# algbio/SBWT

Measured on AMD Instinct MI355X. Metric: k-mers/sec (whole node), plain-matrix k=30 streaming search, higher is better.
Workload: dtype u64

## Files before the change

### include/sbwtgpu.h

```cpp
#ifndef SBWTGPU_H
#define SBWTGPU_H

#include <stdint.h>
#include <stddef.h>

#ifdef __cplusplus
extern "C" {
#endif

#define SBWTGPU_OK                      0
#define SBWTGPU_ERR_INVALID_ARG        -1
#define SBWTGPU_ERR_NO_DEVICE          -2
#define SBWTGPU_ERR_HIP                -3
#define SBWTGPU_ERR_NO_STREAMING       -4
#define SBWTGPU_ERR_PRECALC_TOO_LONG   -5
#define SBWTGPU_ERR_PRECALC_GT_K       -6
#define SBWTGPU_ERR_NOT_SINGLETON      -7
#define SBWTGPU_ERR_OOM                -8
#define SBWTGPU_ERR_READ_TOO_LONG      -9
#define SBWTGPU_ERR_STALLED           -10

typedef struct sbwtgpu_index sbwtgpu_index;

typedef struct {
    int64_t         n_nodes;
    const uint64_t *A_bits;
    const uint64_t *C_bits;
    const uint64_t *G_bits;
    const uint64_t *T_bits;
    const uint64_t *suffix_group_starts;
    int64_t         k;
    int64_t         n_kmers;
    int64_t         precalc_k;
    const int64_t  *precalc;
} sbwtgpu_index_desc;

typedef struct {
    int64_t n_nodes, n_kmers, k, precalc_k;
    int64_t C[4];
    int32_t has_streaming_support;
    int32_t device;
    int64_t device_precalc_k;
    int64_t blob_bytes;
    int64_t image_level;
    int64_t n_paths;
    int64_t n_branch;
    int64_t default_search_variant;
} sbwtgpu_index_info;

const char *sbwtgpu_version(void);
const char *sbwtgpu_last_error(void);
int         sbwtgpu_device_count(int *count);
int         sbwtgpu_set_tuning(const char *key, int64_t value);

int  sbwtgpu_index_create(const sbwtgpu_index_desc *desc, int device, sbwtgpu_index **out);
void sbwtgpu_index_destroy(sbwtgpu_index *idx);
int  sbwtgpu_index_get_info(const sbwtgpu_index *idx, sbwtgpu_index_info *info);
int  sbwtgpu_index_get_precalc(const sbwtgpu_index *idx, int64_t *out_pairs);

typedef struct {
    int64_t   n_nodes, n_kmers, k;
    uint64_t *A_bits, *C_bits, *G_bits, *T_bits;
    uint64_t *suffix_group_starts;
} sbwtgpu_plain_matrix_bits;
int  sbwtgpu_build_plain_matrix(const char *const *seqs, const int64_t *seq_len, int64_t n_seqs, int64_t k,
                                int add_revcomp, int build_streaming_support, int device,
                                sbwtgpu_plain_matrix_bits *out);
void sbwtgpu_free_plain_matrix(sbwtgpu_plain_matrix_bits *bits);

int  sbwtgpu_index_export_header(const sbwtgpu_index *idx, void *header_out, int64_t header_cap,
                                 int64_t *header_bytes);
int  sbwtgpu_index_blob(const sbwtgpu_index *idx, void **dev_ptr, int64_t *bytes);
int  sbwtgpu_index_copy_blob(const sbwtgpu_index *idx, void *dst_dev, int64_t bytes, void *stream);
int  sbwtgpu_index_adopt(const void *header, int64_t header_bytes, void *dev_blob, int64_t blob_bytes,
                         int device, sbwtgpu_index **out);
int  sbwtgpu_index_bcast(sbwtgpu_index *root, int n_dev, const int *devs, sbwtgpu_index **out);

int  sbwtgpu_rank_batch(const sbwtgpu_index *idx, const int64_t *pos, const char *sym, int64_t n,
                        int64_t *out);
int  sbwtgpu_streaming_search_batch(const sbwtgpu_index *idx, const char *bases, const int64_t *read_off,
                                    int64_t n_reads, int64_t *out, const int64_t *out_off);
int  sbwtgpu_search_batch(const sbwtgpu_index *idx, const char *bases, const int64_t *read_off,
                          int64_t n_reads, int64_t *out, const int64_t *out_off);
int  sbwtgpu_streaming_search_batch_i32(const sbwtgpu_index *idx, const char *bases, const int64_t *read_off,
                                        int64_t n_reads, int32_t *out, const int64_t *out_off);
int  sbwtgpu_search_batch_i32(const sbwtgpu_index *idx, const char *bases, const int64_t *read_off,
                              int64_t n_reads, int32_t *out, const int64_t *out_off);
int  sbwtgpu_update_interval_batch(const sbwtgpu_index *idx, const char *bases, const int64_t *off,
                                   int64_t n, int64_t *first, int64_t *second);
int  sbwtgpu_forward_batch(const sbwtgpu_index *idx, const int64_t *node, const char *sym, int64_t n,
                           int64_t *out);
int  sbwtgpu_partial_search_batch(const sbwtgpu_index *idx, const char *bases, const int64_t *off, int64_t n,
                                  int64_t *first, int64_t *second, int64_t *matched);
int  sbwtgpu_get_kmer_batch(const sbwtgpu_index *idx, const int64_t *colex_rank, int64_t n, char *out);
int  sbwtgpu_select_batch(const sbwtgpu_index *idx, const int64_t *j, const char *sym, int64_t n, int64_t *out);

int64_t sbwtgpu_search_workspace_bytes(int64_t total_bases);
int  sbwtgpu_streaming_search_dev(const sbwtgpu_index *idx, const char *d_bases, int64_t total_bases,
                                  const int64_t *d_read_off, int64_t n_reads, int64_t *d_out,
                                  const int64_t *d_out_off, void *d_workspace, int64_t workspace_bytes,
                                  void *stream);
int  sbwtgpu_search_dev(const sbwtgpu_index *idx, const char *d_bases, int64_t total_bases,
                        const int64_t *d_read_off, int64_t n_reads, int64_t *d_out,
                        const int64_t *d_out_off, void *d_workspace, int64_t workspace_bytes,
                        void *stream);
int  sbwtgpu_streaming_search_dev_i32(const sbwtgpu_index *idx, const char *d_bases, int64_t total_bases,
                                      const int64_t *d_read_off, int64_t n_reads, int32_t *d_out,
                                      const int64_t *d_out_off, void *d_workspace, int64_t workspace_bytes,
                                      void *stream);
int  sbwtgpu_search_dev_i32(const sbwtgpu_index *idx, const char *d_bases, int64_t total_bases,
                            const int64_t *d_read_off, int64_t n_reads, int32_t *d_out,
                            const int64_t *d_out_off, void *d_workspace, int64_t workspace_bytes,
                            void *stream);
int  sbwtgpu_rank_dev(const sbwtgpu_index *idx, const int64_t *d_pos, const char *d_sym, int64_t n,
                      int64_t *d_out, void *stream);
int  sbwtgpu_encode_bases_dev(const sbwtgpu_index *idx, const char *d_bases, int64_t total_bases,
                              void *d_workspace, int64_t workspace_bytes, void *stream);
int  sbwtgpu_search_encoded_dev(const sbwtgpu_index *idx, int64_t total_bases, const int64_t *d_read_off,
                                int64_t n_reads, int64_t *d_out, const int64_t *d_out_off,
                                void *d_workspace, int64_t workspace_bytes, int streaming, void *stream);
int  sbwtgpu_workspace_status(const void *d_workspace, void *stream, int *status);
int  sbwtgpu_workspace_stats(const void *d_workspace, void *stream, int64_t stats[8]);
int  sbwtgpu_kernel_times(double *ms, int64_t cap, int64_t *n);

int64_t sbwtgpu_format_text_bound(const sbwtgpu_index *idx, int64_t n_values, int64_t n_reads);
int64_t sbwtgpu_format_scratch_bytes(int64_t n_reads);
int  sbwtgpu_format_results_dev(const sbwtgpu_index *idx, const int64_t *d_values, const int64_t *d_out_off,
                                int64_t n_reads, int64_t n_values, char *d_text, int64_t text_cap,
                                int64_t *d_line_off, void *d_scratch, int64_t scratch_bytes, void *stream);
int  sbwtgpu_search_text_batch(const sbwtgpu_index *idx, const char *bases, const int64_t *read_off,
                               int64_t n_reads, int streaming, char **text, int64_t *text_bytes,
                               int64_t *n_queries);
typedef int (*sbwtgpu_text_sink)(void *ctx, const char *text, int64_t bytes);
int  sbwtgpu_search_text_stream(const sbwtgpu_index *idx, const char *bases, const int64_t *read_off,
                                int64_t n_reads, int streaming, sbwtgpu_text_sink sink, void *sink_ctx,
                                int64_t *n_queries);
void sbwtgpu_free_host(void *p);
void sbwtgpu_release_cached_buffers(void);

int  sbwtgpu_index_build_lcs(sbwtgpu_index *idx);
int  sbwtgpu_index_get_lcs(const sbwtgpu_index *idx, uint8_t *out);
int  sbwtgpu_matching_statistics_batch(const sbwtgpu_index *idx, const char *bases, const int64_t *read_off,
                                       int64_t n_reads, uint8_t *len, int64_t *first, int64_t *second);
int64_t sbwtgpu_ms_workspace_bytes(int64_t total_bases);
int  sbwtgpu_matching_statistics_dev(const sbwtgpu_index *idx, const char *d_bases, int64_t total_bases,
                                     const int64_t *d_read_off, int64_t n_reads, uint8_t *d_len, int64_t *d_first,
                                     int64_t *d_second, void *d_workspace, int64_t workspace_bytes, void *stream);
int  sbwtgpu_ms_workspace_stats(const void *d_workspace, void *stream, int64_t stats[5]);

typedef struct sbwtgpu_unitigs sbwtgpu_unitigs;
int  sbwtgpu_unitigs_create(const sbwtgpu_index *idx, sbwtgpu_unitigs **out);
int  sbwtgpu_unitigs_info(const sbwtgpu_unitigs *u, int64_t *n_unitigs, int64_t *total_bases, int64_t *n_kmers);
int  sbwtgpu_unitigs_dev(const sbwtgpu_unitigs *u, const char **d_bases, const int64_t **d_off ,
                         const int64_t **d_first_col );
int  sbwtgpu_unitigs_copy(const sbwtgpu_unitigs *u, char *bases, int64_t *off, int64_t *first_col );
int  sbwtgpu_unitigs_stats(const sbwtgpu_unitigs *u, double pass_ms[6], int64_t *jump_rounds);
void sbwtgpu_unitigs_destroy(sbwtgpu_unitigs *u);

#define SBWTGPU_SETOP_UNION 0
#define SBWTGPU_SETOP_INTERSECTION 1
#define SBWTGPU_SETOP_DIFFERENCE 2
#define SBWTGPU_SETOP_SYMMETRIC_DIFFERENCE 3
typedef struct {
    int64_t n_a, n_b, n_both, n_either;
    int64_t n_result, n_nopred;
    double  pass_ms[4];
} sbwtgpu_setop_info;
int  sbwtgpu_index_setop(const sbwtgpu_index *a, const sbwtgpu_index *b, int op, int build_streaming_support,
                         sbwtgpu_plain_matrix_bits *out, sbwtgpu_setop_info *info );
int  sbwtgpu_index_setop_counts(const sbwtgpu_index *a, const sbwtgpu_index *b, sbwtgpu_setop_info *info);
int  sbwtgpu_index_kmer_keys(const sbwtgpu_index *idx, void *out_keys, int64_t cap_bytes, int64_t *n_keys, int *key_bytes);

typedef struct { int32_t n_kmers, n_found, covered_bases, longest_run; } sbwtgpu_read_hits;
int     sbwtgpu_read_hits_batch(const sbwtgpu_index *idx, const char *bases, const int64_t *read_off, int64_t n_reads,
                                int strands, sbwtgpu_read_hits *out);
int64_t sbwtgpu_read_hits_workspace_bytes(int64_t total_bases, int64_t n_reads, int strands);
int     sbwtgpu_read_hits_dev(const sbwtgpu_index *idx, const char *d_bases, int64_t total_bases, const int64_t *d_read_off,
                              int64_t n_reads, int strands, sbwtgpu_read_hits *d_out, void *d_workspace,
                              int64_t workspace_bytes, void *stream);

#ifdef __cplusplus
}
#endif
#endif
```

### sbwt_amd/capi.py

```python
from __future__ import annotations

import ctypes as C
import os
from typing import Optional, Sequence

import numpy as np

_HERE = os.path.dirname(os.path.abspath(__file__))
LIB_PATH = os.environ.get("SBWTGPU_LIB", os.path.join(_HERE, "lib", "libsbwtgpu.so"))

OK = 0
ERR_INVALID_ARG = -1
ERR_NO_DEVICE = -2
ERR_HIP = -3
ERR_NO_STREAMING = -4
ERR_PRECALC_TOO_LONG = -5
ERR_PRECALC_GT_K = -6
ERR_NOT_SINGLETON = -7
ERR_OOM = -8
ERR_READ_TOO_LONG = -9
ERR_STALLED = -10

EXPORTED_SYMBOLS = [
    "sbwtgpu_version", "sbwtgpu_last_error", "sbwtgpu_device_count", "sbwtgpu_set_tuning",
    "sbwtgpu_index_create", "sbwtgpu_index_destroy", "sbwtgpu_index_get_info", "sbwtgpu_index_get_precalc",
    "sbwtgpu_index_export_header", "sbwtgpu_index_blob", "sbwtgpu_index_copy_blob", "sbwtgpu_index_adopt", "sbwtgpu_index_bcast",
    "sbwtgpu_rank_batch", "sbwtgpu_streaming_search_batch", "sbwtgpu_search_batch",
    "sbwtgpu_streaming_search_batch_i32", "sbwtgpu_search_batch_i32",
    "sbwtgpu_update_interval_batch", "sbwtgpu_forward_batch",
    "sbwtgpu_build_plain_matrix", "sbwtgpu_free_plain_matrix",
    "sbwtgpu_partial_search_batch", "sbwtgpu_get_kmer_batch", "sbwtgpu_select_batch",
    "sbwtgpu_search_workspace_bytes", "sbwtgpu_streaming_search_dev", "sbwtgpu_search_dev",
    "sbwtgpu_streaming_search_dev_i32", "sbwtgpu_search_dev_i32",
    "sbwtgpu_rank_dev", "sbwtgpu_encode_bases_dev", "sbwtgpu_search_encoded_dev",
    "sbwtgpu_workspace_status", "sbwtgpu_workspace_stats", "sbwtgpu_kernel_times",
    "sbwtgpu_format_text_bound", "sbwtgpu_format_scratch_bytes", "sbwtgpu_format_results_dev",
    "sbwtgpu_search_text_batch", "sbwtgpu_search_text_stream", "sbwtgpu_free_host", "sbwtgpu_release_cached_buffers",
    "sbwtgpu_index_build_lcs", "sbwtgpu_index_get_lcs", "sbwtgpu_matching_statistics_batch", "sbwtgpu_ms_workspace_bytes",
    "sbwtgpu_matching_statistics_dev", "sbwtgpu_ms_workspace_stats",
    "sbwtgpu_unitigs_create", "sbwtgpu_unitigs_info", "sbwtgpu_unitigs_dev", "sbwtgpu_unitigs_copy", "sbwtgpu_unitigs_stats",
    "sbwtgpu_unitigs_destroy",
    "sbwtgpu_index_setop", "sbwtgpu_index_setop_counts", "sbwtgpu_index_kmer_keys",
    "sbwtgpu_read_hits_batch", "sbwtgpu_read_hits_workspace_bytes", "sbwtgpu_read_hits_dev",
]

SETOP_UNION, SETOP_INTERSECTION, SETOP_DIFFERENCE, SETOP_SYMMETRIC_DIFFERENCE = 0, 1, 2, 3
SETOPS = {"union": SETOP_UNION, "intersection": SETOP_INTERSECTION, "difference": SETOP_DIFFERENCE,
          "symmetric-difference": SETOP_SYMMETRIC_DIFFERENCE}


class SbwtGpuError(RuntimeError):
    def __init__(self, code: int, msg: str):
        super().__init__(f"sbwtgpu error {code}: {msg}")
        self.code = code
        self.msg = msg


class IndexDesc(C.Structure):
    _fields_ = [
        ("n_nodes", C.c_int64),
        ("A_bits", C.c_void_p), ("C_bits", C.c_void_p), ("G_bits", C.c_void_p), ("T_bits", C.c_void_p),
        ("suffix_group_starts", C.c_void_p),
        ("k", C.c_int64), ("n_kmers", C.c_int64), ("precalc_k", C.c_int64),
        ("precalc", C.c_void_p),
    ]


class IndexInfo(C.Structure):
    _fields_ = [
        ("n_nodes", C.c_int64), ("n_kmers", C.c_int64), ("k", C.c_int64), ("precalc_k", C.c_int64),
        ("C", C.c_int64 * 4),
        ("has_streaming_support", C.c_int32), ("device", C.c_int32),
        ("device_precalc_k", C.c_int64), ("blob_bytes", C.c_int64), ("image_level", C.c_int64),
        ("n_paths", C.c_int64), ("n_branch", C.c_int64), ("default_search_variant", C.c_int64),
    ]


class ImageHeader(C.Structure):
    _fields_ = [
        ("magic", C.c_uint64),
        ("n_nodes", C.c_int64), ("n_kmers", C.c_int64), ("k", C.c_int64), ("p_file", C.c_int64), ("p_dev", C.c_int64),
        ("C", C.c_int64 * 4),
        ("n_blocks", C.c_int64), ("n_mega", C.c_int64),
        ("off_blocks", C.c_int64), ("off_ptab", C.c_int64), ("off_ftab", C.c_int64), ("off_mega", C.c_int64),
        ("blob_bytes", C.c_int64),
        ("has_ssup", C.c_int32), ("rank_only", C.c_int32), ("ssup_derived", C.c_int32), ("p_sparse", C.c_int32),
        ("off_stab", C.c_int64),
        ("big_layout", C.c_int32), ("has_path", C.c_int32),
        ("off_col", C.c_int64), ("off_pos", C.c_int64), ("off_pq", C.c_int64), ("off_trans", C.c_int64),
        ("stab_pos", C.c_int32), ("p_filter", C.c_int32),
        ("off_pfil", C.c_int64),
        ("log2f", C.c_int32), ("has_safe", C.c_int32), ("force_mega", C.c_int32),
        ("n_tslots", C.c_int64), ("n_sb", C.c_int64), ("n_pos", C.c_int64), ("n_trans", C.c_int64),
        ("n_paths", C.c_int64), ("n_branch", C.c_int64), ("image_level", C.c_int64),
        ("row_ones", C.c_int64 * 4),
        ("log2b2_unused", C.c_int32),
        ("n_sb2", C.c_int64), ("off_stab2", C.c_int64), ("path_lookahead", C.c_int64),
    ]


class PlainMatrixBitsC(C.Structure):
    _fields_ = [("n_nodes", C.c_int64), ("n_kmers", C.c_int64), ("k", C.c_int64),
                ("A_bits", C.c_void_p), ("C_bits", C.c_void_p), ("G_bits", C.c_void_p), ("T_bits", C.c_void_p),
                ("suffix_group_starts", C.c_void_p)]


class SetopInfoC(C.Structure):
    _fields_ = [("n_a", C.c_int64), ("n_b", C.c_int64), ("n_both", C.c_int64), ("n_either", C.c_int64),
                ("n_result", C.c_int64), ("n_nopred", C.c_int64), ("pass_ms", C.c_double * 4)]

    def as_dict(self) -> dict:
        d = {f: int(getattr(self, f)) for f in ("n_a", "n_b", "n_both", "n_either", "n_result", "n_nopred")}
        d["pass_ms"] = dict(zip(("keys_a", "keys_b", "merge_select", "tail_columns"), (float(x) for x in self.pass_ms)))
        return d


_lib: Optional[C.CDLL] = None


def lib() -> C.CDLL:
    global _lib
    if _lib is not None:
        return _lib
    if not os.path.exists(LIB_PATH):
        raise ImportError(f"{LIB_PATH} is missing: build it with `python -m sbwt_amd.build` "
                          "(there is no CPU fallback for the GPU search path)")
    L = C.CDLL(LIB_PATH, mode=C.RTLD_GLOBAL)
    vp, i64, ci = C.c_void_p, C.c_int64, C.c_int
    L.sbwtgpu_version.restype = C.c_char_p
    L.sbwtgpu_last_error.restype = C.c_char_p
    L.sbwtgpu_device_count.argtypes = [C.POINTER(ci)]
    L.sbwtgpu_set_tuning.argtypes = [C.c_char_p, i64]
    L.sbwtgpu_index_create.argtypes = [C.POINTER(IndexDesc), ci, C.POINTER(vp)]
    L.sbwtgpu_index_destroy.argtypes = [vp]
    L.sbwtgpu_index_destroy.restype = None
    L.sbwtgpu_index_get_info.argtypes = [vp, C.POINTER(IndexInfo)]
    L.sbwtgpu_index_get_precalc.argtypes = [vp, vp]
    L.sbwtgpu_index_export_header.argtypes = [vp, vp, i64, C.POINTER(i64)]
    L.sbwtgpu_index_blob.argtypes = [vp, C.POINTER(vp), C.POINTER(i64)]
    L.sbwtgpu_index_copy_blob.argtypes = [vp, vp, i64, vp]
    L.sbwtgpu_index_adopt.argtypes = [vp, i64, vp, i64, ci, C.POINTER(vp)]
    L.sbwtgpu_index_bcast.argtypes = [vp, ci, C.POINTER(ci), C.POINTER(vp)]
    L.sbwtgpu_rank_batch.argtypes = [vp, vp, vp, i64, vp]
    L.sbwtgpu_streaming_search_batch.argtypes = [vp, vp, vp, i64, vp, vp]
    L.sbwtgpu_search_batch.argtypes = [vp, vp, vp, i64, vp, vp]
    try:
        L.sbwtgpu_streaming_search_batch_i32.argtypes = [vp, vp, vp, i64, vp, vp]
        L.sbwtgpu_search_batch_i32.argtypes = [vp, vp, vp, i64, vp, vp]
    except AttributeError:
        if "SBWTGPU_LIB" not in os.environ:
            raise
    L.sbwtgpu_update_interval_batch.argtypes = [vp, vp, vp, i64, vp, vp]
    L.sbwtgpu_forward_batch.argtypes = [vp, vp, vp, i64, vp]
    L.sbwtgpu_build_plain_matrix.argtypes = [C.POINTER(C.c_char_p), vp, i64, i64, ci, ci, ci, C.POINTER(PlainMatrixBitsC)]
    L.sbwtgpu_free_plain_matrix.argtypes = [C.POINTER(PlainMatrixBitsC)]
    L.sbwtgpu_free_plain_matrix.restype = None
    L.sbwtgpu_partial_search_batch.argtypes = [vp, vp, vp, i64, vp, vp, vp]
    L.sbwtgpu_get_kmer_batch.argtypes = [vp, vp, i64, vp]
    L.sbwtgpu_select_batch.argtypes = [vp, vp, vp, i64, vp]
    L.sbwtgpu_search_workspace_bytes.argtypes = [i64]
    L.sbwtgpu_search_workspace_bytes.restype = i64
    L.sbwtgpu_streaming_search_dev.argtypes = [vp, vp, i64, vp, i64, vp, vp, vp, i64, vp]
    L.sbwtgpu_search_dev.argtypes = [vp, vp, i64, vp, i64, vp, vp, vp, i64, vp]
    try:
        L.sbwtgpu_streaming_search_dev_i32.argtypes = [vp, vp, i64, vp, i64, vp, vp, vp, i64, vp]
        L.sbwtgpu_search_dev_i32.argtypes = [vp, vp, i64, vp, i64, vp, vp, vp, i64, vp]
    except AttributeError:
        if not os.environ.get("SBWTGPU_LIB"):
            raise
    L.sbwtgpu_rank_dev.argtypes = [vp, vp, vp, i64, vp, vp]
    L.sbwtgpu_workspace_status.argtypes = [vp, vp, C.POINTER(ci)]
    L.sbwtgpu_encode_bases_dev.argtypes = [vp, vp, i64, vp, i64, vp]
    L.sbwtgpu_search_encoded_dev.argtypes = [vp, i64, vp, i64, vp, vp, vp, i64, ci, vp]
    L.sbwtgpu_workspace_stats.argtypes = [vp, vp, C.POINTER(i64)]
    L.sbwtgpu_kernel_times.argtypes = [vp, i64, C.POINTER(i64)]
    L.sbwtgpu_format_text_bound.argtypes = [vp, i64, i64]
    L.sbwtgpu_format_text_bound.restype = i64
    L.sbwtgpu_format_scratch_bytes.argtypes = [i64]
    L.sbwtgpu_format_scratch_bytes.restype = i64
    L.sbwtgpu_format_results_dev.argtypes = [vp, vp, vp, i64, i64, vp, i64, vp, vp, i64, vp]
    L.sbwtgpu_search_text_batch.argtypes = [vp, vp, vp, i64, ci, C.POINTER(vp), C.POINTER(i64), C.POINTER(i64)]
    L.sbwtgpu_free_host.argtypes = [vp]
    L.sbwtgpu_free_host.restype = None
    L.sbwtgpu_release_cached_buffers.restype = None
    try:
        L.sbwtgpu_index_build_lcs.argtypes = [vp]
        L.sbwtgpu_index_get_lcs.argtypes = [vp, vp]
        L.sbwtgpu_matching_statistics_batch.argtypes = [vp, vp, vp, i64, vp, vp, vp]
        L.sbwtgpu_ms_workspace_bytes.argtypes = [i64]
        L.sbwtgpu_ms_workspace_bytes.restype = i64
        L.sbwtgpu_matching_statistics_dev.argtypes = [vp, vp, i64, vp, i64, vp, vp, vp, vp, i64, vp]
        L.sbwtgpu_ms_workspace_stats.argtypes = [vp, vp, C.POINTER(i64)]
        L.sbwtgpu_unitigs_create.argtypes = [vp, C.POINTER(vp)]
        L.sbwtgpu_unitigs_info.argtypes = [vp, C.POINTER(i64), C.POINTER(i64), C.POINTER(i64)]
        L.sbwtgpu_unitigs_dev.argtypes = [vp, C.POINTER(vp), C.POINTER(vp), C.POINTER(vp)]
        L.sbwtgpu_unitigs_copy.argtypes = [vp, vp, vp, vp]
        L.sbwtgpu_unitigs_stats.argtypes = [vp, C.POINTER(C.c_double), C.POINTER(i64)]
        L.sbwtgpu_unitigs_destroy.argtypes = [vp]
        L.sbwtgpu_unitigs_destroy.restype = None
        L.sbwtgpu_index_setop.argtypes = [vp, vp, ci, ci, C.POINTER(PlainMatrixBitsC), C.POINTER(SetopInfoC)]
        L.sbwtgpu_index_setop_counts.argtypes = [vp, vp, C.POINTER(SetopInfoC)]
        L.sbwtgpu_index_kmer_keys.argtypes = [vp, vp, i64, C.POINTER(i64), C.POINTER(ci)]
        L.sbwtgpu_read_hits_batch.argtypes = [vp, vp, vp, i64, ci, vp]
        L.sbwtgpu_read_hits_workspace_bytes.argtypes = [i64, i64, ci]
        L.sbwtgpu_read_hits_workspace_bytes.restype = i64
        L.sbwtgpu_read_hits_dev.argtypes = [vp, vp, i64, vp, i64, ci, vp, vp, i64, vp]
    except AttributeError:
        if not os.environ.get("SBWTGPU_LIB"):
            raise
    _lib = L
    return L


def _check(rc: int) -> None:
    if rc != OK:
        raise SbwtGpuError(rc, lib().sbwtgpu_last_error().decode(errors="replace"))


def set_tuning(key: str, value: int) -> None:
    _check(lib().sbwtgpu_set_tuning(key.encode(), value))


def device_count() -> int:
    n = C.c_int(0)
    rc = lib().sbwtgpu_device_count(C.byref(n))
    return n.value if rc == OK else 0


def _words(a) -> np.ndarray:
    a = np.ascontiguousarray(a, dtype=np.uint64)
    return a


def concat_reads(reads: Sequence[bytes]):
    lens = np.fromiter((len(r) for r in reads), dtype=np.int64, count=len(reads))
    off = np.zeros(len(reads) + 1, dtype=np.int64)
    np.cumsum(lens, out=off[1:])
    bases = np.frombuffer(b"".join(reads), dtype=np.uint8).copy() if len(reads) else np.zeros(0, np.uint8)
    return bases, off


def out_offsets(read_off: np.ndarray, k: int) -> np.ndarray:
    lens = np.diff(read_off)
    m = np.maximum(lens - k + 1, 0)
    off = np.zeros(len(read_off), dtype=np.int64)
    np.cumsum(m, out=off[1:])
    return off


class BuiltBits:

    def __init__(self, cols, ssup, n_nodes, n_kmers, k):
        self.cols, self.ssup, self.n_nodes, self.n_kmers, self.k = cols, ssup, n_nodes, n_kmers, k


def _take_bits(out: PlainMatrixBitsC) -> BuiltBits:
    try:
        nw = (out.n_nodes + 63) // 64

        def words(p):
            return np.ctypeslib.as_array(C.cast(p, C.POINTER(C.c_uint64)), shape=(nw,)).copy()
        cols = [words(out.A_bits), words(out.C_bits), words(out.G_bits), words(out.T_bits)]
        ssup = words(out.suffix_group_starts) if out.suffix_group_starts else None
        return BuiltBits(cols, ssup, out.n_nodes, out.n_kmers, out.k)
    finally:
        lib().sbwtgpu_free_plain_matrix(C.byref(out))


def build_bits_gpu(seqs: Sequence[bytes], k: int, add_revcomp: bool = False, streaming_support: bool = True,
                   device: int = 0) -> BuiltBits:
    arr = (C.c_char_p * len(seqs))(*[bytes(s) for s in seqs])
    lens = np.array([len(s) for s in seqs], dtype=np.int64)
    out = PlainMatrixBitsC()
    _check(lib().sbwtgpu_build_plain_matrix(arr, lens.ctypes.data, len(seqs), k, int(add_revcomp), int(streaming_support),
                                            device, C.byref(out)))
    return _take_bits(out)


class Index:

    def __init__(self, handle: int, keepalive=None):
        self._h = C.c_void_p(handle)
        self._keep = keepalive
        info = IndexInfo()
        _check(lib().sbwtgpu_index_get_info(self._h, C.byref(info)))
        self.n_nodes, self.n_kmers, self.k = info.n_nodes, info.n_kmers, info.k
        self.precalc_k = info.precalc_k
        self.C = [info.C[i] for i in range(4)]
        self.has_streaming_support = bool(info.has_streaming_support)
        self.device = info.device
        self.device_precalc_k = info.device_precalc_k
        self.blob_bytes = info.blob_bytes
        self.image_level = info.image_level
        self.n_paths, self.n_branch, self.default_search_variant = info.n_paths, info.n_branch, info.default_search_variant

    @property
    def handle(self) -> C.c_void_p:
        return self._h

    @classmethod
    def create(cls, A, Cb, G, T, ssup, n_nodes: int, k: int, n_kmers: int = 0, precalc_k: int = 0,
               precalc=None, device: int = 0) -> "Index":
        A, Cb, G, T = _words(A), _words(Cb), _words(G), _words(T)
        s = _words(ssup) if ssup is not None else None
        pc = np.ascontiguousarray(precalc, dtype=np.int64) if precalc is not None else None
        d = IndexDesc(n_nodes, A.ctypes.data, Cb.ctypes.data, G.ctypes.data, T.ctypes.data,
                      s.ctypes.data if s is not None else None, k, n_kmers, precalc_k,
                      pc.ctypes.data if pc is not None else None)
        h = C.c_void_p()
        _check(lib().sbwtgpu_index_create(C.byref(d), device, C.byref(h)))
        return cls(h.value)

    @classmethod
    def adopt(cls, header: bytes, dev_ptr: int, blob_bytes: int, device: int, keepalive=None) -> "Index":
        h = C.c_void_p()
        buf = C.create_string_buffer(header, len(header))
        _check(lib().sbwtgpu_index_adopt(buf, len(header), C.c_void_p(dev_ptr), blob_bytes, device, C.byref(h)))
        return cls(h.value, keepalive=keepalive)

    def close(self) -> None:
        if self._h:
            lib().sbwtgpu_index_destroy(self._h)
            self._h = C.c_void_p()

    def __del__(self):
        try:
            self.close()
        except Exception:
            pass

    def export_header(self) -> bytes:
        n = C.c_int64(0)
        _check(lib().sbwtgpu_index_export_header(self._h, None, 0, C.byref(n)))
        buf = C.create_string_buffer(n.value)
        _check(lib().sbwtgpu_index_export_header(self._h, buf, n.value, C.byref(n)))
# ... 3 lines not shown
        raw = self.export_header()
        if len(raw) != C.sizeof(ImageHeader):
            raise SbwtGpuError(ERR_INVALID_ARG, "ImageHeader has %d bytes, the library's header %d" % (C.sizeof(ImageHeader), len(raw)))
        return ImageHeader.from_buffer_copy(raw)

    def blob(self):
        p, n = C.c_void_p(), C.c_int64(0)
        _check(lib().sbwtgpu_index_blob(self._h, C.byref(p), C.byref(n)))
        return p.value, n.value

    def blob_tensor(self):
        import torch
        ptr, n = self.blob()

        class _Alias:
            __cuda_array_interface__ = {"shape": (n,), "typestr": "|u1", "data": (ptr, False), "version": 3, "strides": None}
        t = torch.as_tensor(_Alias(), device=torch.device("cuda", self.device))
        t._sbwt_owner = self
        return t

    def copy_blob(self, dst_dev_ptr: int, nbytes: int, stream: int = 0) -> None:
        _check(lib().sbwtgpu_index_copy_blob(self._h, dst_dev_ptr, nbytes, stream))

    def get_precalc(self) -> np.ndarray:
        out = np.zeros((4 ** self.precalc_k if self.precalc_k else 0, 2), dtype=np.int64)
        if self.precalc_k:
            _check(lib().sbwtgpu_index_get_precalc(self._h, out.ctypes.data))
        return out

    def rank(self, pos, sym) -> np.ndarray:
        pos = np.ascontiguousarray(pos, dtype=np.int64)
        sym = np.ascontiguousarray(sym, dtype=np.uint8)
        out = np.empty(len(pos), dtype=np.int64)
        _check(lib().sbwtgpu_rank_batch(self._h, pos.ctypes.data, sym.ctypes.data, len(pos), out.ctypes.data))
        return out

    def _search(self, fn, bases, read_off, out_off=None):
        bases = np.ascontiguousarray(bases, dtype=np.uint8)
        read_off = np.ascontiguousarray(read_off, dtype=np.int64)
        if out_off is None:
            out_off = out_offsets(read_off, self.k)
        out_off = np.ascontiguousarray(out_off, dtype=np.int64)
        out = np.full(int(out_off[-1]) if len(out_off) else 0, -12345, dtype=np.int64)
        _check(fn(self._h, bases.ctypes.data, read_off.ctypes.data, len(read_off) - 1, out.ctypes.data,
                  out_off.ctypes.data))
        return out, out_off

    def streaming_search(self, bases, read_off, out_off=None):
        return self._search(lib().sbwtgpu_streaming_search_batch, bases, read_off, out_off)

    def search(self, bases, read_off, out_off=None):
        return self._search(lib().sbwtgpu_search_batch, bases, read_off, out_off)

    def search_i32(self, bases, read_off, streaming: bool = True, out_off=None):
        bases = np.ascontiguousarray(bases, dtype=np.uint8)
        read_off = np.ascontiguousarray(read_off, dtype=np.int64)
        if out_off is None:
            out_off = out_offsets(read_off, self.k)
        out_off = np.ascontiguousarray(out_off, dtype=np.int64)
        out = np.full(int(out_off[-1]) if len(out_off) else 0, -12345, dtype=np.int32)
        fn = lib().sbwtgpu_streaming_search_batch_i32 if streaming else lib().sbwtgpu_search_batch_i32
        _check(fn(self._h, bases.ctypes.data, read_off.ctypes.data, len(read_off) - 1, out.ctypes.data, out_off.ctypes.data))
        return out, out_off

    def streaming_search_reads(self, reads: Sequence[bytes]):
        bases, off = concat_reads(reads)
        out, oo = self.streaming_search(bases, off)
        return [out[oo[i]:oo[i + 1]] for i in range(len(reads))]

    def search_reads(self, reads: Sequence[bytes]):
        bases, off = concat_reads(reads)
        out, oo = self.search(bases, off)
        return [out[oo[i]:oo[i + 1]] for i in range(len(reads))]

    def search_text(self, bases, read_off, streaming: bool = True):
        bases = np.ascontiguousarray(bases, dtype=np.uint8)
        read_off = np.ascontiguousarray(read_off, dtype=np.int64)
        p, n, q = C.c_void_p(), C.c_int64(0), C.c_int64(0)
        _check(lib().sbwtgpu_search_text_batch(self._h, bases.ctypes.data, read_off.ctypes.data, len(read_off) - 1,
                                               int(streaming), C.byref(p), C.byref(n), C.byref(q)))
        try:
            return C.string_at(p.value, n.value), q.value
        finally:
            lib().sbwtgpu_free_host(p)

    def update_interval(self, bases, off, first, second):
        bases = np.ascontiguousarray(bases, dtype=np.uint8)
        off = np.ascontiguousarray(off, dtype=np.int64)
        first = np.array(first, dtype=np.int64)
        second = np.array(second, dtype=np.int64)
        _check(lib().sbwtgpu_update_interval_batch(self._h, bases.ctypes.data, off.ctypes.data, len(first),
                                                   first.ctypes.data, second.ctypes.data))
        return first, second

    def forward(self, node, sym) -> np.ndarray:
        node = np.ascontiguousarray(node, dtype=np.int64)
        sym = np.ascontiguousarray(sym, dtype=np.uint8)
        out = np.empty(len(node), dtype=np.int64)
        _check(lib().sbwtgpu_forward_batch(self._h, node.ctypes.data, sym.ctypes.data, len(node), out.ctypes.data))
        return out

    def partial_search(self, bases, off):
        bases = np.ascontiguousarray(bases, dtype=np.uint8)
        off = np.ascontiguousarray(off, dtype=np.int64)
        n = len(off) - 1
        first, second, matched = (np.empty(n, dtype=np.int64) for _ in range(3))
        _check(lib().sbwtgpu_partial_search_batch(self._h, bases.ctypes.data, off.ctypes.data, n, first.ctypes.data,
                                                  second.ctypes.data, matched.ctypes.data))
        return first, second, matched

    def get_kmers(self, colex_ranks) -> np.ndarray:
        cr = np.ascontiguousarray(colex_ranks, dtype=np.int64)
        out = np.empty((len(cr), self.k), dtype=np.uint8)
        _check(lib().sbwtgpu_get_kmer_batch(self._h, cr.ctypes.data, len(cr), out.ctypes.data))
        return out

    def select(self, j, sym) -> np.ndarray:
        j = np.ascontiguousarray(j, dtype=np.int64)
        sym = np.ascontiguousarray(sym, dtype=np.uint8)
        out = np.empty(len(j), dtype=np.int64)
        _check(lib().sbwtgpu_select_batch(self._h, j.ctypes.data, sym.ctypes.data, len(j), out.ctypes.data))
        return out

    def streaming_search_dev(self, d_bases: int, total_bases: int, d_read_off: int, n_reads: int, d_out: int,
                             d_out_off: int, d_ws: int, ws_bytes: int, stream: int = 0, streaming: bool = True):
        fn = lib().sbwtgpu_streaming_search_dev if streaming else lib().sbwtgpu_search_dev
        _check(fn(self._h, d_bases, total_bases, d_read_off, n_reads, d_out, d_out_off, d_ws, ws_bytes, stream))

    def streaming_search_dev_i32(self, d_bases: int, total_bases: int, d_read_off: int, n_reads: int, d_out32: int,
                                 d_out_off: int, d_ws: int, ws_bytes: int, stream: int = 0, streaming: bool = True):
        fn = lib().sbwtgpu_streaming_search_dev_i32 if streaming else lib().sbwtgpu_search_dev_i32
        _check(fn(self._h, d_bases, total_bases, d_read_off, n_reads, d_out32, d_out_off, d_ws, ws_bytes, stream))

    def encode_bases_dev(self, d_bases: int, total_bases: int, d_ws: int, ws_bytes: int, stream: int = 0):
        _check(lib().sbwtgpu_encode_bases_dev(self._h, d_bases, total_bases, d_ws, ws_bytes, stream))

    def search_encoded_dev(self, total_bases: int, d_read_off: int, n_reads: int, d_out: int, d_out_off: int,
                           d_ws: int, ws_bytes: int, streaming: bool = True, stream: int = 0):
        _check(lib().sbwtgpu_search_encoded_dev(self._h, total_bases, d_read_off, n_reads, d_out, d_out_off, d_ws,
                                                ws_bytes, int(streaming), stream))

    def workspace_stats(self, d_ws: int, stream: int = 0):
        st = (C.c_int64 * 8)()
        _check(lib().sbwtgpu_workspace_stats(d_ws, stream, st))
        return tuple(int(x) for x in st[:5])

    def workspace_bridges(self, d_ws: int, stream: int = 0) -> int:
        st = (C.c_int64 * 8)()
        _check(lib().sbwtgpu_workspace_stats(d_ws, stream, st))
        return int(st[5])

    def build_lcs(self) -> None:
        _check(lib().sbwtgpu_index_build_lcs(self._h))

    def lcs(self) -> np.ndarray:
        out = np.empty(self.n_nodes, dtype=np.uint8)
        _check(lib().sbwtgpu_index_get_lcs(self._h, out.ctypes.data))
        return out

    def matching_statistics(self, bases, read_off, intervals: bool = True):
        bases = np.ascontiguousarray(bases, dtype=np.uint8)
        read_off = np.ascontiguousarray(read_off, dtype=np.int64)
        n = int(read_off[-1]) if len(read_off) else 0
        ln = np.zeros(n, dtype=np.uint8)
        first = np.full(n, -12345, dtype=np.int64) if intervals else None
        second = np.full(n, -12345, dtype=np.int64) if intervals else None
        _check(lib().sbwtgpu_matching_statistics_batch(self._h, bases.ctypes.data, read_off.ctypes.data, max(len(read_off) - 1, 0),
                                                       ln.ctypes.data, first.ctypes.data if intervals else None,
                                                       second.ctypes.data if intervals else None))
        return (ln, first, second) if intervals else ln

    def matching_statistics_reads(self, reads: Sequence[bytes], intervals: bool = True):
        bases, off = concat_reads(reads)
        res = self.matching_statistics(bases, off, intervals)
        if not intervals:
            return [res[off[i]:off[i + 1]] for i in range(len(reads))]
        return [tuple(a[off[i]:off[i + 1]] for a in res) for i in range(len(reads))]

    def matching_statistics_dev(self, d_bases: int, total_bases: int, d_read_off: int, n_reads: int, d_len: int,
                                d_first: int, d_second: int, d_ws: int, ws_bytes: int, stream: int = 0):
        _check(lib().sbwtgpu_matching_statistics_dev(self._h, d_bases, total_bases, d_read_off, n_reads, d_len,
                                                     d_first or None, d_second or None, d_ws, ws_bytes, stream))

    def ms_workspace_stats(self, d_ws: int, stream: int = 0) -> dict:
        st = (C.c_int64 * 5)()
        _check(lib().sbwtgpu_ms_workspace_stats(d_ws, stream, st))
        return dict(zip(("positions", "walked", "full", "contractions", "recomputes"), (int(x) for x in st)))

    def unitigs_dev(self) -> "Unitigs":
        h = C.c_void_p()
        _check(lib().sbwtgpu_unitigs_create(self._h, C.byref(h)))
        return Unitigs(h)

    def unitigs(self):
        with self.unitigs_dev() as u:
            return u.copy()

    def setop(self, other: "Index", op, streaming_support: bool = True):
        out, info = PlainMatrixBitsC(), SetopInfoC()
        rc = lib().sbwtgpu_index_setop(self._h, other._h, SETOPS.get(op, op), int(streaming_support), C.byref(out), C.byref(info))
        if rc != OK:
            err = SbwtGpuError(rc, lib().sbwtgpu_last_error().decode(errors="replace"))
            err.info = info.as_dict()
            raise err
        return _take_bits(out), info.as_dict()

    def setop_counts(self, other: "Index") -> dict:
        info = SetopInfoC()
        _check(lib().sbwtgpu_index_setop_counts(self._h, other._h, C.byref(info)))
        d = info.as_dict()
        d["jaccard"] = d["n_both"] / d["n_either"] if d["n_either"] else 1.0
        d["containment"] = d["n_both"] / d["n_a"] if d["n_a"] else 1.0
        return d

    def kmer_keys(self) -> np.ndarray:
        n, kb = C.c_int64(0), C.c_int(0)
        cap = max(self.n_kmers, 0) * (8 if self.k <= 32 else 16)
        out = np.empty(cap // 8, dtype=np.uint64)
        rc = lib().sbwtgpu_index_kmer_keys(self._h, out.ctypes.data if cap else None, cap, C.byref(n), C.byref(kb))
        if rc in (OK, ERR_INVALID_ARG) and n.value * kb.value > cap:
            cap = n.value * kb.value
            out = np.empty(cap // 8, dtype=np.uint64)
            rc = lib().sbwtgpu_index_kmer_keys(self._h, out.ctypes.data, cap, C.byref(n), C.byref(kb))
        _check(rc)
        out = out[: n.value * kb.value // 8]
        return out if kb.value == 8 else out.reshape(n.value, 2)

    def read_hits(self, bases, read_off, both_strands: bool = False) -> np.ndarray:
        bases = np.ascontiguousarray(bases, dtype=np.uint8)
        read_off = np.ascontiguousarray(read_off, dtype=np.int64)
        n = max(len(read_off) - 1, 0)
        out = np.full((n, 4), -12345, dtype=np.int32)
        _check(lib().sbwtgpu_read_hits_batch(self._h, bases.ctypes.data, read_off.ctypes.data, n, 2 if both_strands else 1,
                                             out.ctypes.data))
        return out

    def read_hits_reads(self, reads: Sequence[bytes], both_strands: bool = False) -> np.ndarray:
        bases, off = concat_reads(reads)
        return self.read_hits(bases, off, both_strands)

    def read_hits_dev(self, d_bases: int, total_bases: int, d_read_off: int, n_reads: int, d_out: int, d_ws: int, ws_bytes: int,
                      both_strands: bool = False, stream: int = 0):
        _check(lib().sbwtgpu_read_hits_dev(self._h, d_bases, total_bases, d_read_off, n_reads, 2 if both_strands else 1, d_out,
                                           d_ws, ws_bytes, stream))

    def workspace_status(self, d_ws: int, stream: int = 0) -> int:
        st = C.c_int(0)
        _check(lib().sbwtgpu_workspace_status(d_ws, stream, C.byref(st)))
        return st.value


class Unitigs:

    def __init__(self, handle):
        self._h = handle
        n, total, nk = C.c_int64(0), C.c_int64(0), C.c_int64(0)
        _check(lib().sbwtgpu_unitigs_info(self._h, C.byref(n), C.byref(total), C.byref(nk)))
        self.n_unitigs, self.total_bases, self.n_kmers = n.value, total.value, nk.value

    def __enter__(self):
        return self

    def __exit__(self, *exc):
        self.close()

    def close(self) -> None:
        if self._h:
            lib().sbwtgpu_unitigs_destroy(self._h)
            self._h = None

    def __del__(self):
        try:
            self.close()
        except Exception:
            pass

    def dev_ptrs(self):
        b, o, f = C.c_void_p(), C.c_void_p(), C.c_void_p()
        _check(lib().sbwtgpu_unitigs_dev(self._h, C.byref(b), C.byref(o), C.byref(f)))
        return b.value or 0, o.value or 0, f.value or 0

    def copy(self):
        bases = np.empty(self.total_bases, dtype=np.uint8)
        off = np.empty(self.n_unitigs + 1, dtype=np.int64)
        first_col = np.empty(self.n_unitigs, dtype=np.int64)
        _check(lib().sbwtgpu_unitigs_copy(self._h, bases.ctypes.data, off.ctypes.data, first_col.ctypes.data))
        return bases, off, first_col

    def stats(self) -> dict:
        ms = (C.c_double * 6)()
        r = C.c_int64(0)
        _check(lib().sbwtgpu_unitigs_stats(self._h, ms, C.byref(r)))
        names = ("pred_marks", "real_flags", "internal_edges", "pointer_jumping", "ids_offsets", "bases")
        return {"pass_ms": dict(zip(names, (float(x) for x in ms))), "jump_rounds": int(r.value)}


def kernel_times() -> list:
    buf = (C.c_double * 256)()
    n = C.c_int64(0)
    _check(lib().sbwtgpu_kernel_times(buf, 256, C.byref(n)))
    return [float(buf[i]) for i in range(n.value)]


def search_workspace_bytes(total_bases: int) -> int:
    return int(lib().sbwtgpu_search_workspace_bytes(total_bases))


def ms_workspace_bytes(total_bases: int) -> int:
    return int(lib().sbwtgpu_ms_workspace_bytes(total_bases))


def read_hits_workspace_bytes(total_bases: int, n_reads: int, both_strands: bool = False) -> int:
    return int(lib().sbwtgpu_read_hits_workspace_bytes(total_bases, n_reads, 2 if both_strands else 1))
```

### sbwt_amd/csrc/sbwt_device.h

```cpp
#pragma once
#include <stdint.h>

#ifndef SBWT_MEGA_SHIFT
#define SBWT_MEGA_SHIFT 31
#endif
static_assert(SBWT_MEGA_SHIFT >= 7 && SBWT_MEGA_SHIFT <= 31, "a mega block holds 2 .. 2^25 whole 64-column blocks, and its relative counts fit 32 bits");
#define SBWT_GROUP_BASES 32

#ifndef SBWT_FUSED_SORT_DEFAULT
#define SBWT_FUSED_SORT_DEFAULT 3632
#endif
struct SbwtIndexView {
    const uint4 *blocks;
    const longlong2 *ptab;
    const unsigned long long *mega;
    long long n_nodes;
    long long n_pos;
    long long C[4];
    int k;
    int p_dev;
    int n_mega;
    int has_ssup;
    int probe_len;
    const uint4 *stab;
    int p_sparse;
    unsigned n_sb;
    const unsigned *col, *pos;
    const uint4 *pq;
    int has_safe;
    const uint4 *stab2;
    unsigned n_sb2;
    const uint4 *pfil;
    int p_filter, log2f;
    const uint4 *trans;
    unsigned n_tslots;
    int stab_pos;
    int debug;
    int out32 = 0;
    int big = 0;
    int fused_sort = 0;
    int force_mega;
};

struct SbwtBlobHeader {
    uint64_t magic;
    int64_t n_nodes, n_kmers, k, p_file, p_dev;
    int64_t C[4];
    int64_t n_blocks, n_mega;
    int64_t off_blocks, off_ptab, off_ftab, off_mega, blob_bytes;
    int32_t has_ssup;
    int32_t rank_only;
    int32_t ssup_derived;
    int32_t p_sparse;
    int64_t off_stab;
    int32_t big_layout;
    int32_t has_path;
    int64_t off_col, off_pos, off_pq, off_trans;
    int32_t stab_pos;
    int32_t p_filter;
    int64_t off_pfil;
    int32_t log2f;
    int32_t has_safe;
    int32_t force_mega;
    int64_t n_tslots;
    int64_t n_sb;
    int64_t n_pos;
    int64_t n_trans;
    int64_t n_paths;
    int64_t n_branch;
    int64_t image_level;
    int64_t row_ones[4];
    int32_t log2b2_unused;
    int64_t n_sb2;
    int64_t off_stab2;
    int64_t path_lookahead;
};
#define SBWT_BLOB_MAGIC 0x3355504754574253ull

#define SBWT_SP_EMPTY (1ull << 63)
#define SBWT_SP_OVERFLOW (1ull << 62)
#define SBWT_SP_UNIQ 0x80000000u
#define SBWT_SP_MAX_DEPTH 31
#define SBWT_SP_HASH 0x9E3779B97F4A7C15ull
static __host__ __device__ inline unsigned long long sp2_hash(unsigned origin, unsigned long long key2) {
    unsigned long long h = (key2 ^ ((unsigned long long)origin << 17)) * SBWT_SP_HASH;
    h ^= h >> 31;
    return (h + origin) * 0xD6E8FEB86659FD93ull;
}
#define SBWT_SP2_USED 0x80000000u
#define SBWT_SP2_OVERFLOW 0x80000000u
static __host__ __device__ inline unsigned long long sbwt_pf_hash(unsigned long long key) { return key * SBWT_SP_HASH; }
static __host__ __device__ inline unsigned sbwt_pf_bits(unsigned long long h) { return (unsigned)(h >> 24) ^ (unsigned)(h >> 41); }

struct SbwtWorkHeader {
    unsigned long long ticket;
    int status;
    int rg_sample;
    unsigned long long n_stream;
    unsigned long long n_search;
    unsigned long long n_lf;
    unsigned long long n_tab_hit;
    unsigned long long n_ext;
    unsigned long long n_bridge;
    unsigned long long u_bad;
    long long u_read0, u_len, u_out0, u_stride;
    unsigned long long n_deferred;
    unsigned long long ticket2;
    unsigned long long n_pieces;
    unsigned long long pad[15];
    unsigned long long rg_long;
    unsigned long long n_ftick;
    unsigned long long ftick_over;
    unsigned long long pad2[5];
    unsigned long long hint;
};
#define SBWT_WS_CLEAR_BYTES (sizeof(SbwtWorkHeader) - 8)

#define SBWT_PIECE 1024
struct SbwtPieceTab {
    uint4 *pairs = nullptr;
    uint4 *outs = nullptr;
    long long cap = 0;
    int piece = SBWT_PIECE;
};
static_assert(sizeof(SbwtWorkHeader) == 320, "workspace header is 320 bytes");
struct SbwtTickTab {
    uint4 *tick = nullptr;
    unsigned *tick_read = nullptr;
    unsigned *defer_bits = nullptr;
    long long cap = 0;
};
#define SBWT_HINT_MAGIC 0x5B377A00u
#define SBWT_HINT_RATIO 12
#define SBWT_HINT_CALLS 2

void sbwt_launch_encode(const char *d_bases, long long total_bases, uint4 *d_packed, SbwtWorkHeader *ws,
                        hipStream_t stream);
void sbwt_launch_search(const SbwtIndexView &ix, const uint4 *d_packed, const long long *d_read_off,
                        const long long *d_out_off, long long *d_out, long long n_reads, SbwtWorkHeader *ws,
                        int streaming, hipStream_t stream, int variant, long long total_groups, void *d_sort_scratch,
                        long long sort_scratch_bytes, int sort_key_bits, SbwtPieceTab pt);
void sbwt_launch_search_fused(const SbwtIndexView &ix, const char *d_bases, long long total_bases, uint4 *d_packed,
                              const long long *d_read_off, const long long *d_out_off, long long *d_out, long long n_reads,
                              SbwtWorkHeader *ws, int streaming, hipStream_t stream, unsigned *d_defer,
                              hipEvent_t ev_begin, hipEvent_t ev_end, SbwtPieceTab pt, int ragged_ok, SbwtTickTab tt = SbwtTickTab());
void sbwt_launch_encode_chained(const char *d_bases, long long total_bases, uint4 *d_packed, SbwtWorkHeader *ws,
                                const unsigned *d_defer, const long long *d_read_off, int k, hipStream_t stream);
void sbwt_launch_search_chained(const SbwtIndexView &ix, const uint4 *d_packed, const long long *d_read_off,
                                const long long *d_out_off, long long *d_out, long long n_reads, SbwtWorkHeader *ws,
                                int streaming, hipStream_t stream, const unsigned *d_defer, SbwtPieceTab pt);
void sbwt_launch_piece_bounds_tt(const uint4 *d_packed, const long long *d_read_off, const long long *d_out_off, int k,
                                 SbwtWorkHeader *ws, SbwtPieceTab pt, int behind_fused, hipStream_t stream, const unsigned *defer_bits);
void sbwt_launch_piece_bounds(const uint4 *d_packed, const long long *d_read_off, const long long *d_out_off, int k,
                              SbwtWorkHeader *ws, SbwtPieceTab pt, int behind_fused, hipStream_t stream);
long long sbwt_sort_scratch_bytes(long long n_reads, int key_bits);
const unsigned *sbwt_launch_sort_reads(const SbwtIndexView &ix, const uint4 *d_packed, const long long *d_read_off,
                                       long long n_reads, const SbwtWorkHeader *ws, void *d_scratch, long long scratch_bytes,
                                       int key_bits, hipStream_t stream);
void sbwt_launch_rank(const SbwtIndexView &ix, const long long *d_pos, const char *d_sym, long long n,
                      long long *d_out, hipStream_t stream);
void sbwt_launch_precalc(const SbwtIndexView &ix, int p, longlong2 *d_table, hipStream_t stream);
void sbwt_launch_update_interval(const SbwtIndexView &ix, const char *d_bases, const long long *d_off, long long n,
                                 long long *d_first, long long *d_second, hipStream_t stream);
void sbwt_launch_forward(const SbwtIndexView &ix, const long long *d_node, const char *d_sym, long long n,
                         long long *d_out, hipStream_t stream);
void sbwt_launch_partial_search(const SbwtIndexView &ix, const char *d_bases, const long long *d_off, long long n,
                                long long *d_first, long long *d_second, long long *d_matched, hipStream_t stream);
void sbwt_launch_get_kmer(const SbwtIndexView &ix, const long long *d_colex, long long n, char *d_out,
                          hipStream_t stream);
void sbwt_launch_select(const SbwtIndexView &ix, const long long *d_j, const char *d_sym, long long n,
                        const long long row_ones[4], long long *d_out, hipStream_t stream);
long long sbwt_format_scratch_bytes(long long n_reads);
void sbwt_launch_format(const long long *d_vals, const long long *d_out_off, long long n_reads, char *d_text,
                        long long *d_line_off, void *d_scratch, hipStream_t stream);
long long sbwt_blocks_scratch_bytes(long long n_nodes);
int sbwt_blocks_count(const unsigned long long *d_bits, long long n_nodes, void *d_scratch, long long totals[5], hipStream_t st);
void sbwt_blocks_fill(const unsigned long long *d_bits, const unsigned long long *d_ssup, long long n_nodes, void *d_scratch,
                      const long long C[4], int use_mega, int n_mega, uint4 *d_blocks, unsigned long long *d_mega, hipStream_t st);
long long sbwt_derive_scratch_bytes(long long n_nodes);
void sbwt_launch_derive_marks(const SbwtIndexView &ix, uint4 *d_blocks, void *d_scratch, hipStream_t stream);
long long sbwt_sparse_scratch_bytes(long long n_nodes);
long long sbwt_path_scratch_bytes(long long n_nodes);
long long sbwt_path_quads(long long n_nodes);
long long sbwt_count_paths(const SbwtIndexView &ix, hipStream_t stream);
void sbwt_launch_path_safe(const SbwtIndexView &ix, uint4 *d_pq, int rule, void *d_hlab, unsigned char *d_alt_safe,
                           hipStream_t stream);
long long sbwt_path_safe_scratch_bytes(long long n_pos, int k);
long long sbwt_launch_path_oth(const SbwtIndexView &ix, uint4 *d_pq, long long *n_branch, hipStream_t stream, int count_only = 0);
void sbwt_launch_trans_insert(const SbwtIndexView &ix, uint4 *d_trans, long long n_slots, const unsigned char *d_alt_safe,
                              hipStream_t stream);
int sbwt_launch_build_path(const SbwtIndexView &ix, unsigned *d_col, unsigned *d_pos, uint4 *d_pq, long long pos_cap,
                           long long *n_pos, int stitch, int min_copy, void *d_scratch, int lookahead, hipStream_t stream);
int sbwt_launch_build_sparse(const SbwtIndexView &ix, int p_dense, int p_sparse, long long n_buckets, uint4 *d_table,
                             void *d_scratch, const unsigned *d_pos, int p_filter, int log2f, uint4 *d_filter,
                             long long n_entries2, uint4 *d_table2, hipStream_t stream);

struct SbwtBuildState {
    int k = 0, rc = 0, ssup = 0;
    int key_bytes = 8;
    long long n_text = 0, nk = 0, ng = 0, n_nopred = 0;
    void *km = nullptr;
    unsigned *edges = nullptr;
    void *nopred_keys = nullptr;
};
int sbwt_build_phase_a(const char *h_text, long long n_text, int k, int rc, SbwtBuildState *S, hipStream_t st);
int sbwt_build_from_keys(void *d_km, long long nk, int k, SbwtBuildState *S, hipStream_t st);
int sbwt_build_copy_nopred(const SbwtBuildState *S, void *h_keys);
int sbwt_build_phase_b(SbwtBuildState *S, const void *h_ddata, const unsigned *h_dedges, long long nd, int ssup,
                       unsigned long long *h_rows, hipStream_t st);
void sbwt_build_release(SbwtBuildState *S);
```

### sbwt_amd/csrc/sbwt_kernels_common.h

```cpp
#pragma once
#include <hip/hip_runtime.h>
#include <cstdio>
#include <cstdlib>
#include "sbwt_device.h"

typedef unsigned long long u64;
typedef long long i64;

#define SBWT_ERR_NOT_SINGLETON (-7)
#define SBWT_ERR_STALLED (-10)

__device__ __forceinline__ unsigned dna_code(unsigned b) { return ((b >> 1) & 3u) ^ ((b >> 2) & 1u); }
__device__ __forceinline__ bool is_ACGT(unsigned b) { return b == 'A' || b == 'C' || b == 'G' || b == 'T'; }
__device__ __forceinline__ u64 quad_bits(const uint4 &q) { return (u64)q.x | ((u64)q.y << 32); }
__device__ __forceinline__ u64 low_mask(int n) { return (1ull << n) - 1ull; }

__device__ __forceinline__ unsigned uniform32(unsigned v) { return (unsigned)__builtin_amdgcn_readfirstlane((int)v); }
__device__ __forceinline__ u64 uniform64(u64 v) {
    return (u64)(unsigned)__builtin_amdgcn_readfirstlane((int)(unsigned)v) |
           ((u64)(unsigned)__builtin_amdgcn_readfirstlane((int)(unsigned)(v >> 32)) << 32);
}

typedef unsigned u32x4 __attribute__((ext_vector_type(4)));
#ifdef SBWT_PLAIN_STORES
#define SBWT_NT_STORE(v, p) (*(p) = (v))
#else
#define SBWT_NT_STORE(v, p) __builtin_nontemporal_store(v, p)
#endif
__device__ __forceinline__ void st_stream(i64 *p, i64 v) { SBWT_NT_STORE(v, p); }
typedef i64 i64x2_a8 __attribute__((ext_vector_type(2), aligned(8)));
typedef unsigned u32x2_a4 __attribute__((ext_vector_type(2), aligned(4)));
__device__ __forceinline__ void st_stream2(i64 *p, i64 a, i64 b) {
    i64x2_a8 v = {a, b};
    SBWT_NT_STORE(v, reinterpret_cast<i64x2_a8 *>(p));
}
typedef int i32x2_a4 __attribute__((ext_vector_type(2), aligned(4)));
__device__ __forceinline__ void st_res(i64 *out, i64 at, i64 v, int o32) {
    if (o32) SBWT_NT_STORE((int)v, reinterpret_cast<int *>(out) + at);
    else st_stream(out + at, v);
}
__device__ __forceinline__ void st_res2(i64 *out, i64 at, i64 a, i64 b, int o32) {
    if (o32) {
        i32x2_a4 v = {(int)a, (int)b};
        SBWT_NT_STORE(v, reinterpret_cast<i32x2_a4 *>(reinterpret_cast<int *>(out) + at));
    } else {
        st_stream2(out + at, a, b);
    }
}
__device__ __forceinline__ uint4 ld_stream(const uint4 *p) {
    u32x4 v = __builtin_nontemporal_load(reinterpret_cast<const u32x4 *>(p));
    return make_uint4(v.x, v.y, v.z, v.w);
}

template <bool MEGA>
__device__ __forceinline__ u64 quad_rank(const SbwtIndexView &ix, const uint4 &q, i64 pos, int c) {
    u64 v = (u64)q.z + (u64)__popcll(quad_bits(q) & low_mask((int)(pos & 63)));
    if (MEGA) v += ix.mega[(i64)c * ix.n_mega + (pos >> SBWT_MEGA_SHIFT)];
    return v;
}

template <bool MEGA>
__device__ __forceinline__ u64 block_count(const SbwtIndexView &ix, i64 blk, int c, uint4 *q) {
    *q = ix.blocks[(blk << 2) + c];
    u64 v = (u64)q->z;
    if (MEGA) v += ix.mega[(i64)c * ix.n_mega + (blk >> (SBWT_MEGA_SHIFT - 6))];
    return v;
}

template <bool MEGA>
__device__ __forceinline__ i64 select_in_row(const SbwtIndexView &ix, int c, i64 target_i, i64 row_ones) {
    const u64 target = (u64)target_i;
    const i64 n_blocks = ix.n_nodes / 64 + 1;
    i64 g = row_ones > 0 ? (i64)((double)(target_i - ix.C[c]) / (double)row_ones * (double)n_blocks) : 0;
    if (g < 0) g = 0;
    if (g > n_blocks - 1) g = n_blocks - 1;
    uint4 q;
    i64 lo, hi;
    if (block_count<MEGA>(ix, g, c, &q) <= target) {
        lo = g;
        i64 step = 1;
        hi = g + step;
        while (hi < n_blocks && block_count<MEGA>(ix, hi, c, &q) <= target) { lo = hi; step <<= 1; hi = lo + step; }
        if (hi > n_blocks) hi = n_blocks;
    } else {
        hi = g;
        i64 step = 1;
        lo = g - step;
        while (lo > 0 && block_count<MEGA>(ix, lo, c, &q) > target) { hi = lo; step <<= 1; lo = hi - step; }
        if (lo < 0) lo = 0;
    }
    while (hi - lo > 1) {
        const i64 mid = lo + ((hi - lo) >> 1);
        if (block_count<MEGA>(ix, mid, c, &q) <= target) lo = mid; else hi = mid;
    }
    const u64 cnt = block_count<MEGA>(ix, lo, c, &q);
    u64 bits = quad_bits(q);
    const int skip = (int)(target - cnt);
    for (int s = 0; s < skip; s++) bits &= bits - 1;
    return (lo << 6) + (bits ? (__ffsll((i64)bits) - 1) : 0);
}


#define PS_NONE 0
#define PS_TRANS 1
#define PS_BRIDGE 2
#define PS_ABSENT 3
__device__ __forceinline__ int path_stop_kind(bool mismatch, unsigned sA, unsigned sB, bool has_safe) {
    if (!mismatch || !sB) return PS_TRANS;
    return (sA && has_safe) ? PS_BRIDGE : PS_ABSENT;
}
#define SBWT_TRANS_NEG 0x100u
#define SBWT_TRANS_NEG_SAFE 0x200u
__device__ __forceinline__ unsigned sbwt_sp_bucket(u64 key, unsigned n_buckets, unsigned j) {
    unsigned b = (unsigned)__umul64hi(key * SBWT_SP_HASH, (u64)n_buckets) + j;
    while (b >= n_buckets) b -= n_buckets;
    return b;
}
__device__ __forceinline__ unsigned sbwt_sp2_entry(unsigned origin, u64 key2, unsigned n_entries, unsigned j) {
    unsigned e = (unsigned)__umul64hi(sp2_hash(origin, key2), (u64)n_entries) + j;
    while (e >= n_entries) e -= n_entries;
    return e;
}
__device__ __forceinline__ unsigned sbwt_trans_slot(unsigned t, unsigned c, unsigned n_slots, unsigned j) {
    const u64 h = ((u64)t * 4ull + c) * SBWT_SP_HASH;
    unsigned s = (unsigned)__umul64hi(h, (u64)n_slots) + j;
    while (s >= n_slots) s -= n_slots;
    return s;
}

#define SBWT_FUSED_MAXG 5
#define SBWT_FUSED_MAXLEN (32 * SBWT_FUSED_MAXG)
#define SBWT_FUSED_MAXP 3
__device__ __forceinline__ long long sbwt_fused_limit(int P, int k) {
    const int kpp = SBWT_FUSED_MAXLEN - k + 1;
    return (P <= 1 || kpp < 64) ? (long long)SBWT_FUSED_MAXLEN : (long long)P * kpp + k - 1;
}
__device__ __forceinline__ int sbwt_fused_pieces(const SbwtWorkHeader *ws, int k) {
    const int sample = ws->rg_sample & 0xFFFF;
    int maxp = ws->rg_sample >> 16;
    if (maxp < 1) maxp = 1;
    if (maxp > SBWT_FUSED_MAXP) maxp = SBWT_FUSED_MAXP;
    if (ws->u_bad == 0) {
        for (int P = 1; P <= maxp; P++)
            if (ws->u_len <= sbwt_fused_limit(P, k)) return P;
        return 0;
    }
    if (sample <= 0) return 0;
    for (int P = 1; P <= maxp; P++) {
        const unsigned long long longer = (ws->rg_long >> (20 * (P - 1))) & 0xFFFFFull;
        if (longer * 8ull <= (unsigned long long)sample && (P == 1 || sbwt_fused_limit(P, k) > SBWT_FUSED_MAXLEN)) return P;
    }
    return 0;
}
__device__ __forceinline__ int sbwt_fused_mode(const SbwtWorkHeader *ws, int k) {
    const long long len = ws->u_len;
    const int pieces = sbwt_fused_pieces(ws, k);
    if (ws->u_bad == 0 && pieces > 0) return (len >= 32 && len >= k) ? 1 : 0;
    if (ws->u_bad != 0 && pieces > 0) return 2;
    return (ws->n_ftick > 0 && ws->ftick_over == 0) ? 3 : 0;
}
__device__ __forceinline__ bool sbwt_fused_wants_table(const SbwtWorkHeader *ws, int k) {
    return (ws->rg_sample & 0xFFFF) > 0 && sbwt_fused_pieces(ws, k) == 0;
}
#define SBWT_RG_SAMPLE 4096
__device__ __forceinline__ void fused_sample_of_wave(i64 t, i64 len, bool valid, i64 n_reads, int rg_enable, int k, SbwtWorkHeader *ws) {
    if (t == 0) ws->rg_sample = ((rg_enable & 1) ? (int)(n_reads < SBWT_RG_SAMPLE ? n_reads : SBWT_RG_SAMPLE) : 0) | ((rg_enable >> 8) << 16);
    if (t - (threadIdx.x & 63) >= SBWT_RG_SAMPLE) return;
    const bool in = valid && t < SBWT_RG_SAMPLE;
    const u64 l1 = __ballot(in && len > sbwt_fused_limit(1, k)), l2 = __ballot(in && len > sbwt_fused_limit(2, k)),
              l3 = __ballot(in && len > sbwt_fused_limit(3, k));
    if (l1 && (threadIdx.x & 63) == 0)
        atomicAdd(&ws->rg_long, (unsigned long long)__popcll(l1) | ((unsigned long long)__popcll(l2) << 20) |
                                    ((unsigned long long)__popcll(l3) << 40));
}

__device__ __forceinline__ bool piece_read_is_cut(i64 m, int piece) {
    return m > 2 * (i64)piece && m > (i64)SBWT_FUSED_MAXP * SBWT_FUSED_MAXLEN;
}
__device__ __forceinline__ void piece_zones_of_wave(i64 r, i64 len, bool valid, int k, SbwtWorkHeader *ws, const SbwtPieceTab &pt) {
    const i64 m = len - k + 1;
    const bool isl = valid && pt.pairs != nullptr && piece_read_is_cut(m, pt.piece);
    u64 mask = __ballot(isl);
    if (!mask) return;
    const i64 nz = isl ? m / pt.piece : 0;
    const i64 base = isl ? (i64)atomicAdd(&ws->n_pieces, (unsigned long long)nz) : 0;
    const int lane = threadIdx.x & 63;
    while (mask) {
        const int src = __ffsll((i64)mask) - 1;
        mask &= mask - 1;
        const i64 rr = __shfl(r, src), bb = __shfl(base, src), nn = __shfl(nz, src);
        for (i64 j = lane; j < nn && bb + j < pt.cap; j += 64)
            pt.outs[bb + j] = make_uint4((unsigned)rr, (unsigned)((u64)rr >> 32), (unsigned)j, (unsigned)nn);
    }
}

static inline unsigned grid_for(i64 n) {
    if (n + 255 >= ((i64)1 << 32)) {
        fprintf(stderr, "sbwtgpu: internal error: a launch of %lld threads exceeds the 2^32 work-items of one dispatch\n", (long long)n);
        abort();
    }
    return (unsigned)((n + 255) / 256);
}
```

### sbwt_amd/csrc/sbwt_search.hip

```cpp
#include "sbwt_kernels_common.h"

__device__ __forceinline__ uint4 encode_group(const unsigned char *__restrict__ bases, i64 total, i64 g, int aligned16) {
    i64 base = g * SBWT_GROUP_BASES;
    u64 codes = 0;
    unsigned vu = 0, vr = 0;
    if (aligned16 && base + SBWT_GROUP_BASES <= total) {
        const uint4 *src = reinterpret_cast<const uint4 *>(bases + base);
        uint4 x0 = ld_stream(src), x1 = ld_stream(src + 1);
        unsigned w[8] = {x0.x, x0.y, x0.z, x0.w, x1.x, x1.y, x1.z, x1.w};
#pragma unroll
        for (int d = 0; d < 8; d++) {
            const unsigned up = w[d] & 0xDFDFDFDFu;
            const unsigned t = ((up >> 1) & 0x03030303u) ^ ((up >> 2) & 0x01010101u);
            const unsigned c8 = (t * 0x01041040u) >> 24;
            auto nz = [](unsigned v) { return ((v & 0x7F7F7F7Fu) + 0x7F7F7F7Fu) | v; };
            const unsigned none = nz(up ^ 0x41414141u) & nz(up ^ 0x43434343u) & nz(up ^ 0x47474747u) & nz(up ^ 0x54545454u);
            const unsigned isl = (~none >> 7) & 0x01010101u;
            const unsigned u4 = (isl * 0x10204080u) >> 28;
            const unsigned low4 = (((w[d] >> 5) & 0x01010101u) * 0x10204080u) >> 28;
            codes |= (u64)c8 << (8 * d);
            vu |= u4 << (4 * d);
            vr |= (u4 & ~low4) << (4 * d);
        }
    } else {
        for (int pos = 0; pos < SBWT_GROUP_BASES; pos++) {
            if (base + pos < total) {
                unsigned b = bases[base + pos];
                unsigned up = b & 0xDFu;
                codes |= (u64)dna_code(up) << (2 * pos);
                vu |= (unsigned)is_ACGT(up) << pos;
                vr |= (unsigned)is_ACGT(b) << pos;
            }
        }
    }
    return make_uint4((unsigned)codes, (unsigned)(codes >> 32), vu, vr);
}

__global__ void __launch_bounds__(256) k_encode(const unsigned char *__restrict__ bases, i64 total,
                                                uint4 *__restrict__ packed, i64 n_groups,
                                                SbwtWorkHeader *ws, int aligned16) {
    i64 g = (i64)blockIdx.x * 256 + threadIdx.x;
    if (g == 0) { ws->ticket = 0; ws->status = 0; ws->n_stream = 0; ws->n_search = 0; ws->n_lf = 0; ws->n_tab_hit = 0; ws->n_ext = 0; ws->n_bridge = 0; }
    if (g >= n_groups) return;
    packed[g] = encode_group(bases, total, g, aligned16);
}

__global__ void __launch_bounds__(256) k_encode_chained(const unsigned char *__restrict__ bases, i64 total,
                                                        uint4 *__restrict__ packed, i64 n_groups, const SbwtWorkHeader *ws,
                                                        const unsigned *__restrict__ defer_list,
                                                        const i64 *__restrict__ read_off, int k, int aligned16) {
    const i64 t0 = (i64)blockIdx.x * 256 + threadIdx.x, stride = (i64)gridDim.x * 256;
    const int fmode = sbwt_fused_mode(ws, k);
    if (fmode == 0) {
        for (i64 g = t0; g < n_groups; g += stride) packed[g] = encode_group(bases, total, g, aligned16);
        return;
    }
    if (fmode >= 2) {
        const i64 nd = (i64)ws->n_deferred, nw = stride >> 6;
        const int lane = threadIdx.x & 63;
        for (i64 d = t0 >> 6; d < nd; d += nw) {
            const i64 r = (i64)defer_list[d], P0 = read_off[r], P1 = read_off[r + 1];
            if (P1 <= P0) continue;
            for (i64 g = (P0 >> 5) + lane; g <= ((P1 - 1) >> 5) && g < n_groups; g += 64)
                packed[g] = encode_group(bases, total, g, aligned16);
        }
        return;
    }
    const i64 nd = (i64)ws->n_deferred, len = ws->u_len, r0 = ws->u_read0;
    const i64 GP = (len + 31) / 32 + 1;
    for (i64 t = t0; t < nd * GP; t += stride) {
        const i64 P0 = r0 + (i64)defer_list[t / GP] * len;
        const i64 g = (P0 >> 5) + (t % GP);
        if (g <= ((P0 + len - 1) >> 5) && g < n_groups) packed[g] = encode_group(bases, total, g, aligned16);
    }
}

#define M_IDLE 0
#define M_STREAM 1
#define M_INIT 2
#define M_STEP 3
#define M_DEAD 4

template <bool MEGA>
__global__ void __launch_bounds__(256) k_search(SbwtIndexView ix, const uint4 *__restrict__ packed,
                                                const i64 *__restrict__ read_off,
                                                const i64 *__restrict__ out_off, i64 *__restrict__ out,
                                                i64 n_reads, SbwtWorkHeader *ws, int streaming) {
    const int lane = threadIdx.x & 63;
    const int k = ix.k, p = ix.p_dev;
    const i64 last_node = ix.n_nodes - 1;

    int mode = M_IDLE;
    bool dead = false;
    i64 P0 = 0, obase = 0;
    int m = 0, i = 0, j = 0;
    i64 a = -1, l = 0, r = 0;
    i64 tag = -1;
    uint4 g0 = make_uint4(0, 0, 0, 0), g1 = make_uint4(0, 0, 0, 0);
    unsigned c_stream = 0, c_search = 0, c_lf = 0, c_tab = 0;

    for (;;) {
        bool want = (mode == M_IDLE) && !dead;
        u64 need = __ballot(want);
        if (need) {
            int leader = __ffsll((i64)need) - 1;
            u64 first = 0;
            if (lane == leader) first = atomicAdd(&ws->ticket, (u64)__popcll(need));
            first = __shfl(first, leader);
            if (want) {
                u64 rd = first + (u64)__popcll(need & low_mask(lane));
                if (rd < (u64)n_reads) {
                    i64 s = read_off[rd], e = read_off[rd + 1];
                    P0 = s;
                    obase = out_off[rd];
                    m = (int)(e - s) - k + 1;
                    i = 0;
                    if (m > 0) {
                        if (p > 0) mode = M_INIT;
                        else { mode = M_STEP; l = 0; r = last_node; j = 0; c_search++; }
                    }
                } else {
                    dead = true;
                }
            }
        }
        if (__ballot(!dead) == 0) break;

        const bool act = (mode != M_IDLE);
        const int q = (mode == M_STREAM) ? (i + k - 1) : ((mode == M_INIT) ? i : (i + j));
        const i64 P = P0 + q;
        if (act && (P >> 5) != tag) {
            tag = P >> 5;
            g0 = packed[tag];
            g1 = packed[tag + 1];
        }
        const int s = (int)(P & 31);
        const u64 codes0 = quad_bits(g0);
        const int c = (int)((codes0 >> (2 * s)) & 3ull);

        const uint4 *a1 = nullptr, *a2 = nullptr;
        bool emit = false;
        i64 res = -1;
        if (mode == M_STREAM) {
            c_stream++;
            if ((g0.z >> s) & 1u) {
                a1 = ix.blocks + (((a >> 6) << 2) + (c & 2));
                a2 = a1 + 1;
            } else {
                emit = true;
            }
        } else if (mode == M_INIT) {
            c_search++;
            u64 w = codes0 >> (2 * s);
            if (s) w |= quad_bits(g1) << (64 - 2 * s);
            u64 vr = (((u64)g1.w << 32) | (u64)g0.w) >> s;
            u64 vm = low_mask(p);
            if ((vr & vm) == vm) a1 = reinterpret_cast<const uint4 *>(ix.ptab + (w & low_mask(2 * p)));
            else emit = true;
        } else if (mode == M_STEP) {
            if ((g0.w >> s) & 1u) {
                a1 = ix.blocks + (((l >> 6) << 2) + c);
                const uint4 *t = ix.blocks + ((((r + 1) >> 6) << 2) + c);
                if (t != a1) a2 = t;
            } else {
                emit = true;
            }
        }

        uint4 v1 = make_uint4(0, 0, 0, 0), v2 = make_uint4(0, 0, 0, 0);
        if (a1) v1 = *a1;
        if (a2) v2 = *a2;

        if (a1) {
            if (mode == M_STREAM) {
                u64 ss = (u64)v1.w | ((u64)v2.w << 32);
                uint4 mine = (c & 1) ? v2 : v1;
                const int b = (int)(a & 63);
                u64 msk = ss & ((2ull << b) - 1ull);
                i64 blk = a >> 6;
                while (msk == 0) {
                    if (blk == 0) { msk = 1; break; }
                    blk--;
                    const uint4 *pa = ix.blocks + ((blk << 2) + (c & 2));
                    uint4 e = pa[0], o = pa[1];
                    msk = (u64)e.w | ((u64)o.w << 32);
                    mine = (c & 1) ? o : e;
                }
                const int gb = 63 - __clzll((i64)msk);
                const u64 bits = quad_bits(mine);
                u64 val = (u64)mine.z + (u64)__popcll(bits & low_mask(gb));
                if (MEGA) val += ix.mega[(i64)c * ix.n_mega + (((blk << 6) | gb) >> SBWT_MEGA_SHIFT)];
                res = ((bits >> gb) & 1ull) ? (i64)val : -1;
                emit = true;
            } else if (mode == M_INIT) {
                l = (i64)quad_bits(v1);
                r = (i64)((u64)v1.z | ((u64)v1.w << 32));
                c_tab += (l != -1);
                if (l == -1) {
                    emit = true;
                } else if (p == k) {
                    emit = true;
                    res = l;
                    if (l != r) ws->status = SBWT_ERR_NOT_SINGLETON;
                } else {
                    j = p;
                    mode = M_STEP;
                }
            } else {
                if (!a2) v2 = v1;
                c_lf++;
                u64 va = quad_rank<MEGA>(ix, v1, l, c);
                u64 vb = quad_rank<MEGA>(ix, v2, r + 1, c);
                l = (i64)va;
                r = (i64)vb - 1;
                if (l > r) {
                    emit = true;
                } else if (++j == k) {
                    emit = true;
                    res = l;
                    if (l != r) ws->status = SBWT_ERR_NOT_SINGLETON;
                }
            }
        }

        if (emit) {
            if (ix.out32) reinterpret_cast<int *>(out)[obase + i] = (int)res;
            else out[obase + i] = res;
            i++;
            if (i == m) {
                mode = M_IDLE;
            } else if (streaming && res != -1) {
                mode = M_STREAM;
                a = res;
            } else if (p > 0) {
                mode = M_INIT;
            } else {
                mode = M_STEP; l = 0; r = last_node; j = 0;
                c_search++;
            }
        }
    }

    u64 t0 = c_stream, t1 = c_search, t2 = c_lf, t3 = c_tab;
#pragma unroll
    for (int off = 32; off > 0; off >>= 1) {
        t0 += __shfl_down(t0, off);
        t1 += __shfl_down(t1, off);
        t2 += __shfl_down(t2, off);
        t3 += __shfl_down(t3, off);
    }
    if (lane == 0) {
        atomicAdd(&ws->n_stream, t0);
        atomicAdd(&ws->n_search, t1);
        atomicAdd(&ws->n_lf, t2);
        atomicAdd(&ws->n_tab_hit, t3);
    }
}

#define M_FETCH 5
#define M_BACK 6
#define M_EXT 7
#define M_TRANS 8
#define M_POS 9
#define M_BRIDGE 10
#define EV_NONE 0
#define EV_EMIT1 1
#define EV_FAIL 2
#define EV_END 3
#define EV_PRES 4
#define K_NONE 0
#define K_FETCH 1
#define K_RELOAD 2
#define K_MODE 3
#define STAGE_DEPTH 8
#ifndef SBWT_COPY_PIPE
#define SBWT_COPY_PIPE 4
#endif

template <bool WIDE> struct SearchTypes;
template <> struct SearchTypes<false> { typedef int pos_t; typedef unsigned stage_t; static constexpr int DEPTH = 16; };
template <> struct SearchTypes<true> { typedef i64 pos_t; typedef u64 stage_t; static constexpr int DEPTH = 8; };

template <bool WIDE>
__device__ __forceinline__ typename SearchTypes<WIDE>::pos_t quad_rank_t(const SbwtIndexView &ix, const uint4 &q,
                                                                        typename SearchTypes<WIDE>::pos_t pos, int c) {
    typedef typename SearchTypes<WIDE>::pos_t pos_t;
    pos_t v = (pos_t)q.z + (pos_t)__popcll(quad_bits(q) & low_mask((int)(pos & 63)));
    if (WIDE) v += (pos_t)ix.mega[(i64)c * ix.n_mega + ((i64)pos >> SBWT_MEGA_SHIFT)];
    return v;
}

#define SBWT_NSEG 12
template <bool WIDE, int WPS, bool PATH>
__global__ void __launch_bounds__(256, WPS) k_search_cert(SbwtIndexView ix, const uint4 *__restrict__ packed,
                                                        const i64 *__restrict__ read_off,
                                                        const i64 *__restrict__ out_off, i64 *__restrict__ out,
                                                        i64 n_reads, SbwtWorkHeader *ws, int streaming,
                                                        const unsigned *__restrict__ perm,
                                                        const unsigned *__restrict__ defer_list, SbwtPieceTab pt) {
    unsigned long long *const ticket = defer_list ? &ws->ticket2 : &ws->ticket;
    if (defer_list && sbwt_fused_mode(ws, ix.k)) {
        n_reads = (i64)ws->n_deferred;
        perm = defer_list;
        if (n_reads == 0) return;
    }
    const bool cut = pt.pairs != nullptr;
    i64 n_tickets = n_reads;
    if (cut) {
        const i64 np = (i64)ws->n_pieces;
        n_tickets += np < pt.cap ? np : pt.cap;
    }
    typedef typename SearchTypes<WIDE>::pos_t pos_t;
    typedef typename SearchTypes<WIDE>::stage_t stage_t;
    constexpr int DEPTH = SearchTypes<WIDE>::DEPTH;
    constexpr bool SEG = PATH;
    static_assert(!PATH || !WIDE, "path order: 32-bit indexes only");
    constexpr bool G3 = SEG;
    __shared__ stage_t stage[SEG ? 1 : DEPTH][SEG ? 1 : 256];
    __shared__ uint2 segs[SEG ? SBWT_NSEG : 1][SEG ? 256 : 1];
    const int tid = threadIdx.x, lane = tid & 63;
    int nseg = 0, i0 = 0, last_start = 0;
    unsigned last_src = 0, emit_pos = 0;
    const int k = ix.k, p = ix.p_dev, L0 = ix.probe_len;
    const int ps = WIDE ? 0 : ix.p_sparse;
    const bool pfon = ix.pfil && ix.p_filter == L0 && L0 > p;
    const u64 m2 = (k - ps >= 32) ? ~0ull : low_mask(2 * ((k - ps) & 31));
    const int pw = pfon ? L0 : p;
    const pos_t last_node = (pos_t)(ix.n_nodes - 1);

    int wk = 0;
    u64 hk = 0;
    int blo = -1;
    unsigned mz = 0;
    int mode = M_IDLE;
    i64 obase = 0;
    int pgrp = 0, poff = 0;
    int m = 0, i = 0, j = 0, b = -1, wstart = 0, cnt = 0;
    pos_t l = 0, r = 0;
    i64 rd = 0;
    bool rdok = true;
    int tag = -2;
    bool g1ok = false, g2ok = false;
    const bool uni = PATH && ws->u_bad == 0 && ws->u_len > 0;
    const i64 u_read0 = ws->u_read0, u_len = ws->u_len, u_out0 = ws->u_out0, u_stride = ws->u_stride;
    unsigned c_ext = 0;
    unsigned c_brg = 0;
    uint4 g0 = make_uint4(0, 0, 0, 0), g1 = make_uint4(0, 0, 0, 0), g2 = make_uint4(0, 0, 0, 0);
    u64 pool_next = 0, pool_end = 0;
    unsigned c_stream = 0, c_search = 0, c_lf = 0, c_tab = 0;

    for (;;) {
        const u64 need = __ballot(mode == M_IDLE);
        if (need) {
            if (pool_next == pool_end) {
// ... 452 lines not shown
                }
            } else {
                l = quad_rank_t<WIDE>(ix, v1, l, c);
                r = quad_rank_t<WIDE>(ix, v2, r + 1, c) - 1;
                if (l > r) {
                    ev = EV_FAIL;
                    tfail = wstart + j;
                } else if (wstart + (++j) == i + k) {
                    ev = EV_END;
                }
            }
        }
        c_tab = uniform32(c_tab + (unsigned)__popcll(__ballot(tabhit)));
        c_stream = uniform32(c_stream + (unsigned)__popcll(__ballot(ev == EV_EMIT1 && (strm || trn))));

        int burst_hi = -1;
        if (ev == EV_END) {
            if (wstart == i) {
                res = l;
                if (l != r) ws->status = SBWT_ERR_NOT_SINGLETON;
                if (PATH && tpos >= 0) { r = tpos; rknown = true; emit_pos = (unsigned)tpos; }
                ev = EV_EMIT1;
                b = -1;
                mz = 0;
            } else {
                do_plan = true;
                force = true;
            }
        } else if (ev == EV_FAIL) {
            burst_hi = (wstart < m - 1) ? wstart : (m - 1);
            if (burst_to >= 0) {
                burst_hi = burst_to;
                b = -1;
            } else if (wk == 3) {
                if (wstart >= b) b = -1;
                else if (blo < wstart + 1) blo = wstart + 1;
            } else if (imprecise && !(wstart == b && blo >= b)) {
                blo = wstart;
                b = tfail;
            } else {
                if (wstart == b) b = -1;
                else if (!(b > wstart && b <= tfail)) b = tfail;
                blo = b;
            }
            if (burst_hi > i || wk == 2 || wk == 3) mz = 0;
            else if (wstart == i && (mz & 3u) < 2u) mz = (mz & 4u) ? (mz & 3u) + 1u : 0u;
            mz &= ~4u;
            if (burst_hi == i) { ev = EV_EMIT1; burst_hi = -1; }
        }
        if (ev == EV_PRES) {
            const int lo = blo > i ? blo : i;
            if (wstart > lo) b = wstart - 1;
            else blo = wstart + pw;
            if (blo > b) b = -1;
            do_plan = true;
        }
        if (ev == EV_EMIT1 && !SEG) {
            stage[cnt][tid] = (stage_t)res;
            cnt++;
            i++;
        }
        if (SEG) {
            auto append = [&](int at, unsigned src) {
                const bool merge = nseg > 0 && ((src == 0xFFFFFFFFu && last_src == 0xFFFFFFFFu) ||
                                                (!(src >> 31) && !(last_src >> 31) && last_src + (unsigned)(at - last_start) == src));
                if (!merge) {
                    segs[nseg][tid] = make_uint2(src, (unsigned)at);
                    nseg++;
                    last_src = src;
                    last_start = at;
                }
            };
            if (ev == EV_EMIT1) {
                append(i, res == -1 ? 0xFFFFFFFFu : (rknown ? emit_pos : (0x80000000u | (unsigned)res)));
                i++;
            }
            {
                const int nleft = (burst_hi >= 0) ? (burst_hi - i + 1) : seg_n;
                if (nleft > 0) {
                    append(i, (burst_hi >= 0) ? 0xFFFFFFFFu : seg_src);
                    i += nleft;
                }
                if (ext_absent) {
                    append(i, 0xFFFFFFFFu);
                    b = blo = i + k - 1;
                    i++;
                    if (i == m) mode = M_IDLE;
                    else do_plan = true;
                }
            }
            u64 fm = __ballot(nseg > 0 && (i == m || nseg > SBWT_NSEG - 2));
            while (fm) {
                constexpr int FP = 4;
                int fL[FP], fe[FP], fj[FP], w0[FP], w1[FP];
                i64 fob[FP];
                unsigned x0[FP], x1[FP];
                bool long_read = false;
#pragma unroll
                for (int u = 0; u < FP; u++) {
                    fL[u] = -1; fe[u] = 0; fj[u] = 0; fob[u] = 0; x0[u] = x1[u] = 0xFFFFFFFFu; w0[u] = w1[u] = 0;
                    if (fm == 0) continue;
                    const int L = __ffsll((i64)fm) - 1;
                    fm &= fm - 1;
                    const int ns = __builtin_amdgcn_readlane(nseg, L), a = __builtin_amdgcn_readlane(i0, L), e = __builtin_amdgcn_readlane(i, L);
                    fL[u] = L;
                    fe[u] = e;
                    fob[u] = (i64)((u64)(unsigned)__builtin_amdgcn_readlane((int)(unsigned)(u64)obase, L) |
                                   ((u64)(unsigned)__builtin_amdgcn_readlane((int)(unsigned)((u64)obase >> 32), L) << 32));
                    long_read = long_read || (e - a > 128);
                    const int tl = (tid & ~63) + L;
                    const int j0 = a + 2 * lane, j1 = j0 + 1;
                    fj[u] = j0;
                    const int my_at = (int)segs[lane < SBWT_NSEG ? lane : SBWT_NSEG - 1][tl].y;
                    int idx = 0;
                    for (int t = 1; t < ns; t++) idx += (__builtin_amdgcn_readlane(my_at, t) <= j0) ? 1 : 0;
                    const uint2 c0 = segs[idx][tl];
                    const uint2 nx = segs[idx + 1 < SBWT_NSEG ? idx + 1 : SBWT_NSEG - 1][tl];
                    const uint2 c1 = (idx + 1 < ns && (int)nx.y <= j1) ? nx : c0;
                    x0[u] = c0.x;
                    x1[u] = c1.x;
                    const unsigned p0 = (j0 < e && !(c0.x >> 31)) ? c0.x + (unsigned)(j0 - (int)c0.y) : 0u;
                    const unsigned p1 = (j1 < e && !(c1.x >> 31)) ? c1.x + (unsigned)(j1 - (int)c1.y) : 0u;
                    w0[u] = (int)ix.col[p0];
                    w1[u] = (int)ix.col[p1];
                }
                int v0[FP], v1[FP];
#pragma unroll
                for (int u = 0; u < FP; u++) {
                    v0[u] = (x0[u] >> 31) ? ((x0[u] == 0xFFFFFFFFu) ? -1 : (int)(x0[u] & 0x7FFFFFFFu)) : w0[u];
                    v1[u] = (x1[u] >> 31) ? ((x1[u] == 0xFFFFFFFFu) ? -1 : (int)(x1[u] & 0x7FFFFFFFu)) : w1[u];
                }
#pragma unroll
                for (int u = 0; u < FP; u++) asm volatile("" : "+v"(v0[u]), "+v"(v1[u]));
                if (!(ix.debug & 1)) {
#pragma unroll
                    for (int u = 0; u < FP; u++) {
                        if (fj[u] + 1 < fe[u]) st_res2(out, fob[u] + fj[u], (i64)v0[u], (i64)v1[u], ix.out32);
                        else if (fj[u] < fe[u]) st_res(out, fob[u] + fj[u], (i64)v0[u], ix.out32);
                    }
                }
                if (long_read) {
#pragma unroll
                    for (int u = 0; u < FP; u++) {
                        if (fL[u] < 0) continue;
                        const int L = fL[u], ns = __shfl(nseg, L), a = __shfl(i0, L), e = fe[u];
                        const int tl = (tid & ~63) + L;
                        for (int base = a + 128; base < e; base += 128) {
                            const int j0 = base + 2 * lane, j1 = j0 + 1;
                            uint2 c0 = segs[0][tl], c1 = c0;
                            for (int sx = 1; sx < ns; sx++) {
                                const uint2 sg = segs[sx][tl];
                                if ((int)sg.y <= j0) c0 = sg;
                                if ((int)sg.y <= j1) c1 = sg;
                            }
                            const unsigned p0 = (j0 < e && !(c0.x >> 31)) ? c0.x + (unsigned)(j0 - (int)c0.y) : 0u;
                            const unsigned p1 = (j1 < e && !(c1.x >> 31)) ? c1.x + (unsigned)(j1 - (int)c1.y) : 0u;
                            const int q0 = (int)ix.col[p0], q1 = (int)ix.col[p1];
                            const int v0 = (c0.x >> 31) ? ((c0.x == 0xFFFFFFFFu) ? -1 : (int)(c0.x & 0x7FFFFFFFu)) : q0;
                            const int v1 = (c1.x >> 31) ? ((c1.x == 0xFFFFFFFFu) ? -1 : (int)(c1.x & 0x7FFFFFFFu)) : q1;
                            if (!(ix.debug & 1)) {
                                if (j1 < e) st_res2(out, fob[u] + j0, (i64)v0, (i64)v1, ix.out32);
                                else if (j0 < e) st_res(out, fob[u] + j0, (i64)v0, ix.out32);
                            }
                        }
                    }
                }
#pragma unroll
                for (int u = 0; u < FP; u++)
                    if (lane == fL[u]) { nseg = 0; i0 = i; }
            }
        } else
        {
            const bool fl = (cnt > 0) && (burst_hi >= 0 || seg_n > 0 || i == m || (((unsigned)obase + (unsigned)i) & (DEPTH - 1)) == 0);
            i64 dst = obase + (i - cnt);
            int nrun = fl ? cnt : 0;
            u64 fm = __ballot(fl);
            const int sub = lane & (DEPTH - 1), grpl = lane / DEPTH;
            constexpr int NG = 64 / DEPTH;
            while (fm) {
                int src = -1;
#pragma unroll
                for (int g = 0; g < NG; g++) {
                    int f = fm ? (__ffsll((i64)fm) - 1) : -1;
                    fm &= fm - 1;
                    src = (grpl == g) ? f : src;
                }
                const int srcl = src < 0 ? 0 : src;
                const i64 d = __shfl(dst, srcl);
                const int nn = __shfl(nrun, srcl);
                if (src >= 0 && sub < nn && !(ix.debug & 1)) {
                    const i64 val = (i64)(pos_t)stage[sub][(tid & ~63) + src];
                    if ((ix.debug & 2) && !ix.out32) out[d + sub] = val;
                    else st_res(out, d + sub, val, ix.out32);
                }
            }
            if (fl) cnt = 0;
            dst = obase + i;
            nrun = (burst_hi >= 0) ? (burst_hi - i + 1) : 0;
            fm = __ballot(nrun > 0);
            while (fm) {
                int src = -1;
                u64 served = 0;
#pragma unroll
                for (int g = 0; g < NG; g++) {
                    int f = fm ? (__ffsll((i64)fm) - 1) : -1;
                    if (f >= 0) served |= 1ull << f;
                    fm &= fm - 1;
                    src = (grpl == g) ? f : src;
                }
                const int srcl = src < 0 ? 0 : src;
                const i64 d = __shfl(dst, srcl);
                const int nn = __shfl(nrun, srcl);
                if (src >= 0 && sub < nn && !(ix.debug & 1)) {
                    if ((ix.debug & 2) && !ix.out32) out[d + sub] = -1;
                    else st_res(out, d + sub, -1, ix.out32);
                }
                if ((served >> lane) & 1ull) { dst += DEPTH; nrun -= DEPTH; }
                fm = __ballot(nrun > 0);
            }
            if (burst_hi >= 0) i = burst_hi + 1;
        }
        if (ev == EV_EMIT1 || burst_hi >= 0) {
            if (i == m) {
                mode = M_IDLE;
            } else if (ev == EV_EMIT1 && res != -1 && streaming) {
                mode = PATH ? (rknown ? tnext : M_POS) : M_STREAM;
                l = res;
                if (PATH) j = 0;
            } else if (PATH && bridged) {
                mode = M_EXT;
                r += (pos_t)k;
            } else {
                do_plan = true;
            }
        }
        if (do_plan) {
            int s0 = i, nwk = (ps > 0) ? 1 : 0;
            if ((mz & 3u) >= 2u) force = true;
            if (!force && L0 > 0 && b >= i && b <= i + k - 1) {
                const int lo = blo > i ? blo : i;
                if (lo < b && p > 0 && k - pw >= 1) {
                    int x = lo + ((b - lo + 1) >> 1);
                    if (x > i + k - pw) x = i + k - pw;
                    if (x <= i) x = i + 1;
                    s0 = x;
                    nwk = 3;
                } else {
                    s0 = (b - i >= L0 - 1) ? (b - L0 + 1) : b;
                    if (pfon && s0 == b && b + L0 - 1 > i + k - 1 && k > L0) s0 = i + k - L0;
                    if (s0 + p - 1 > i + k - 1) s0 = i;
                    if (s0 != i) nwk = (pfon && s0 + L0 - 1 <= i + k - 1) ? 2 : 0;
                }
            }
            wstart = s0;
            j = 0;
            wk = nwk;
            if (p > 0) mode = M_INIT;
            else { mode = M_STEP; l = 0; r = last_node; }
        }
    }

    if (PATH) {
        u64 e = c_ext, eb = c_brg;
#pragma unroll
        for (int off = 32; off > 0; off >>= 1) { e += __shfl_down(e, off); eb += __shfl_down(eb, off); }
        if (lane == 0) { if (e) atomicAdd(&ws->n_ext, e); if (eb) atomicAdd(&ws->n_bridge, eb); }
    }
    if (lane == 0) {
        if (c_stream) atomicAdd(&ws->n_stream, (u64)c_stream);
        if (c_search) atomicAdd(&ws->n_search, (u64)c_search);
        if (c_lf) atomicAdd(&ws->n_lf, (u64)c_lf);
        if (c_tab) atomicAdd(&ws->n_tab_hit, (u64)c_tab);
    }
}

__global__ void __launch_bounds__(256) k_check_uniform(const i64 *__restrict__ read_off, const i64 *__restrict__ out_off,
                                                       i64 n_reads, SbwtWorkHeader *ws, int k, SbwtPieceTab pt) {
    const i64 t = (i64)blockIdx.x * 256 + threadIdx.x;
    const i64 len = read_off[1] - read_off[0], stride = (n_reads > 1) ? out_off[1] - out_off[0] : 0;
    if (t == 0) { ws->u_read0 = read_off[0]; ws->u_len = len; ws->u_out0 = out_off[0]; ws->u_stride = stride; }
    const bool valid = t < n_reads;
    const i64 mylen = valid ? read_off[t + 1] - read_off[t] : 0;
    piece_zones_of_wave(t, mylen, valid, k, ws, pt);
    if (!valid) return;
    const bool bad = (mylen != len) || (t + 1 < n_reads && out_off[t + 1] - out_off[t] != stride);
    if (__ballot(bad) != 0 && (threadIdx.x & 63) == 0) ws->u_bad = 1ull;
}

__device__ static i64 piece_adjust(const uint4 *__restrict__ packed, i64 P0, i64 x, i64 m, int k) {
    i64 cand = x, gi = -1;
    unsigned low = 0;
    for (i64 t = x; cand < m; t++) {
        if (t - cand >= k) return cand;
        const i64 g = (P0 + t) >> 5;
        if (g != gi) { const uint4 q = packed[g]; low = q.z & ~q.w; gi = g; }
        if ((low >> ((P0 + t) & 31)) & 1u) cand = t + 1;
    }
    return m;
}
__global__ void __launch_bounds__(256) k_piece_bounds(const uint4 *__restrict__ packed, const i64 *__restrict__ read_off,
                                                      const i64 *__restrict__ out_off, int k, const SbwtWorkHeader *ws,
                                                      SbwtPieceTab pt, int behind_fused, const unsigned *__restrict__ defer_bits) {
    if (behind_fused && sbwt_fused_mode(ws, k) == 1 && !piece_read_is_cut(ws->u_len - k + 1, pt.piece)) return;
    const i64 z = (i64)blockIdx.x * 256 + threadIdx.x;
    const i64 np = (i64)ws->n_pieces < pt.cap ? (i64)ws->n_pieces : pt.cap;
    if (z >= np) return;
    const uint4 d = pt.outs[z];
    const i64 r = (i64)(((u64)d.y << 32) | (u64)d.x), j = (i64)d.z, nz = (i64)d.w;
    if (behind_fused && defer_bits && sbwt_fused_mode(ws, k) == 3 && !((defer_bits[r >> 5] >> (r & 31)) & 1u)) {
        const i64 P0e = read_off[r];
        pt.pairs[z] = make_uint4((unsigned)P0e, (unsigned)((u64)P0e >> 32), (unsigned)P0e, (unsigned)((u64)P0e >> 32));
        pt.outs[z] = make_uint4(0u, 0u, 0u, 0u);
        return;
    }
    const i64 P0 = read_off[r], m = read_off[r + 1] - P0 - k + 1, ob = out_off[r];
    const i64 s = j ? piece_adjust(packed, P0, j * pt.piece, m, k) : 0;
    const i64 e = (j + 1 == nz) ? m : piece_adjust(packed, P0, (j + 1) * pt.piece, m, k);
    const i64 b0 = P0 + (e > s ? s : 0), b1 = e > s ? P0 + e + k - 1 : P0;
    const i64 o0 = ob + (e > s ? s : 0);
    pt.pairs[z] = make_uint4((unsigned)b0, (unsigned)((u64)b0 >> 32), (unsigned)b1, (unsigned)((u64)b1 >> 32));
    pt.outs[z] = make_uint4((unsigned)o0, (unsigned)((u64)o0 >> 32), 0u, 0u);
}

void sbwt_launch_encode(const char *d_bases, long long total_bases, uint4 *d_packed, SbwtWorkHeader *ws,
                        hipStream_t stream) {
    i64 n_groups = (total_bases + SBWT_GROUP_BASES - 1) / SBWT_GROUP_BASES + 2;
    int aligned = ((uintptr_t)d_bases & 15) == 0;
    hipLaunchKernelGGL(k_encode, dim3(grid_for(n_groups)), dim3(256), 0, stream,
                       reinterpret_cast<const unsigned char *>(d_bases), (i64)total_bases, d_packed, n_groups, ws,
                       aligned);
}

void sbwt_launch_encode_chained(const char *d_bases, long long total_bases, uint4 *d_packed, SbwtWorkHeader *ws,
                                const unsigned *d_defer, const long long *d_read_off, int k, hipStream_t stream) {
    i64 n_groups = (total_bases + SBWT_GROUP_BASES - 1) / SBWT_GROUP_BASES + 2;
    int aligned = ((uintptr_t)d_bases & 15) == 0;
    const i64 want = (n_groups + 255) / 256;
    hipLaunchKernelGGL(k_encode_chained, dim3((unsigned)(want < 4096 ? want : 4096)), dim3(256), 0, stream,
                       reinterpret_cast<const unsigned char *>(d_bases), (i64)total_bases, d_packed, n_groups, ws, d_defer, d_read_off, k,
                       aligned);
}

static inline bool view_is_big(const SbwtIndexView &ix) { return ix.big || ix.n_mega > 1 || ix.n_nodes >= ((1ll << 31) - 128); }
static inline SbwtIndexView general_view(const SbwtIndexView &ix) {
    SbwtIndexView v = ix;
    if (v.k > 32) v.has_safe = 0;
    if (view_is_big(v)) {
        v.stab = nullptr; v.p_sparse = 0; v.n_sb = 0; v.stab_pos = 0;
        v.stab2 = nullptr; v.n_sb2 = 0;
        v.pfil = nullptr; v.p_filter = 0; v.log2f = 0;
        v.col = v.pos = nullptr; v.pq = nullptr; v.trans = nullptr; v.n_tslots = 0; v.has_safe = 0;
        v.n_pos = v.n_nodes;
    }
    return v;
}

void sbwt_launch_search_chained(const SbwtIndexView &ix_in, const uint4 *d_packed, const long long *d_read_off,
                                const long long *d_out_off, long long *d_out, long long n_reads, SbwtWorkHeader *ws,
                                int streaming, hipStream_t stream, const unsigned *d_defer, SbwtPieceTab pt) {
    const i64 want1 = (n_reads + pt.cap + 255) / 256;
    const SbwtIndexView ix = general_view(ix_in);
    const unsigned cap = (ix.debug >> 8) ? (unsigned)(ix.debug >> 8) : 1280u;
    const unsigned g = (unsigned)(want1 < (i64)cap ? want1 : (i64)cap);
    if (view_is_big(ix))
        hipLaunchKernelGGL((k_search_cert<true, 4, false>), dim3(g), dim3(256), 0, stream, ix, d_packed, d_read_off,
                           d_out_off, d_out, (i64)n_reads, ws, streaming, (const unsigned *)nullptr, d_defer, pt);
    else
        hipLaunchKernelGGL((k_search_cert<false, 4, true>), dim3(g), dim3(256), 0, stream, ix, d_packed, d_read_off,
                           d_out_off, d_out, (i64)n_reads, ws, streaming, (const unsigned *)nullptr, d_defer, pt);
}

void sbwt_launch_piece_bounds_tt(const uint4 *d_packed, const long long *d_read_off, const long long *d_out_off, int k,
                                 SbwtWorkHeader *ws, SbwtPieceTab pt, int behind_fused, hipStream_t stream, const unsigned *defer_bits) {
    if (!pt.pairs || pt.cap <= 0) return;
    hipLaunchKernelGGL(k_piece_bounds, dim3(grid_for(pt.cap)), dim3(256), 0, stream, d_packed, d_read_off, d_out_off, k, ws, pt,
                       behind_fused, defer_bits);
}
void sbwt_launch_piece_bounds(const uint4 *d_packed, const long long *d_read_off, const long long *d_out_off, int k,
                              SbwtWorkHeader *ws, SbwtPieceTab pt, int behind_fused, hipStream_t stream) {
    sbwt_launch_piece_bounds_tt(d_packed, d_read_off, d_out_off, k, ws, pt, behind_fused, stream, nullptr);
}

void sbwt_launch_search(const SbwtIndexView &ix_in, const uint4 *d_packed, const long long *d_read_off,
                        const long long *d_out_off, long long *d_out, long long n_reads, SbwtWorkHeader *ws,
                        int streaming, hipStream_t stream, int variant, long long total_groups, void *d_sort_scratch,
                        long long sort_scratch_bytes, int sort_key_bits, SbwtPieceTab pt) {
    if (n_reads <= 0) return;
    const SbwtIndexView ix = general_view(ix_in);
    const unsigned *d_perm = nullptr;
    if (variant >= 1) {
        if (d_sort_scratch) pt = SbwtPieceTab();
        i64 want1 = (n_reads + pt.cap + 255) / 256;
        if (!(ix.debug & 8) || pt.pairs)
            hipLaunchKernelGGL(k_check_uniform, dim3(grid_for(n_reads)), dim3(256), 0, stream, d_read_off, d_out_off,
                               (i64)n_reads, ws, ix.k, pt);
        if (ix.debug & 8) (void)hipMemsetAsync(&ws->u_bad, 0xFF, 8, stream);
        sbwt_launch_piece_bounds(d_packed, d_read_off, d_out_off, ix.k, ws, pt, 0, stream);
        unsigned grid1 = (unsigned)(want1 < 2048 ? want1 : 2048);
        const bool wide = view_is_big(ix) || total_groups >= (1ll << 31) - 4 || (ix.debug & 16);
        unsigned cap = (ix.debug >> 8) ? (unsigned)(ix.debug >> 8) : (variant >= 2 ? 1280u : 1024u);
        unsigned g = grid1 < cap ? grid1 : cap;
        if (wide)
            hipLaunchKernelGGL((k_search_cert<true, 4, false>), dim3(g), dim3(256), 0, stream, ix, d_packed, d_read_off,
                               d_out_off, d_out, (i64)n_reads, ws, streaming, d_perm, (const unsigned *)nullptr, pt);
        else if (variant >= 2 && ix.col && streaming) {
            if (d_sort_scratch)
                d_perm = sbwt_launch_sort_reads(ix, d_packed, d_read_off, n_reads, ws, d_sort_scratch, sort_scratch_bytes,
                                                sort_key_bits, stream);
            hipLaunchKernelGGL((k_search_cert<false, 4, true>), dim3(g), dim3(256), 0, stream, ix, d_packed, d_read_off,
                               d_out_off, d_out, (i64)n_reads, ws, streaming, d_perm, (const unsigned *)nullptr, pt);
        } else
            hipLaunchKernelGGL((k_search_cert<false, 4, false>), dim3(g), dim3(256), 0, stream, ix, d_packed, d_read_off,
                               d_out_off, d_out, (i64)n_reads, ws, streaming, d_perm, (const unsigned *)nullptr, pt);
        return;
    }
    i64 want = (n_reads + 255) / 256;
    unsigned grid = (unsigned)(want < 2048 ? want : 2048);
    if (ix.n_mega > 1)
        hipLaunchKernelGGL(k_search<true>, dim3(grid), dim3(256), 0, stream, ix, d_packed, d_read_off, d_out_off,
                           d_out, (i64)n_reads, ws, streaming == 1 ? 1 : 0);
    else
        hipLaunchKernelGGL(k_search<false>, dim3(grid), dim3(256), 0, stream, ix, d_packed, d_read_off, d_out_off,
                           d_out, (i64)n_reads, ws, streaming == 1 ? 1 : 0);
}
```

### sbwt_amd/csrc/sbwt_search_fused.hip

```cpp
#include "sbwt_kernels_common.h"

#define F_IDLE 0
#define F_INIT 2
#define F_STEP 3
#define F_DEAD 4
#define F_EXT 7
#define F_TRANS 8
#define F_POS 9
#define F_BRIDGE 10
#define F_CMP 11
#define F_PLAN 12
#define FE_NONE 0
#define FE_EMIT1 1
#define FE_FAIL 2
#define FE_END 3
#define FE_PRES 4
#define FE_ANCH 5
#ifndef FZ_ANCHORS
#define FZ_ANCHORS 3
#endif
#ifndef FZ_ALIGNS
#define FZ_ALIGNS 7
#endif
#define CF_S1 1u
#define CF_A1 2u
#define CF_B1 4u
#define CF_S2 8u
#define CF_A2 16u
#define CF_B2 32u
#define CF_ONP 64u
#define CF_ALIGNED 128u
#define CF_ANCH 256u
#define CF_SEED 512u
#define CA_GOON 0
#define CA_DONE 1
#define CA_CERT 2
#define CA_TRANS 3
#define CA_ABSENT 4
#define CA_LOST 5
#define CF_MISS 1024u
#define CF_MISS_MASK 3072u
#define CF_WIN31 8192u
#define CF_SEED2 16384u
#define CF_NOCERT 4096u
#define CF_FORCE (1u << 30)
#define CF_ANC_LEFT(f) (((f) >> 16) & 3u)
#define CF_CMP_LEFT(f) (((f) >> 18) & 7u)
#define CF_ANC_TRIED(f) ((int)(((f) >> 21) & 511u) - 1)
#define CF_SET_TRIED(f, a) ((f) = ((f) & ~(511u << 21)) | ((((unsigned)((a) + 1)) & 511u) << 21))
#define CF_BUDGETS (((unsigned)FZ_ANCHORS << 16) | ((unsigned)FZ_ALIGNS << 18))
#define CF_M1 (CF_S1 | CF_A1 | CF_B1)
#define CF_M2 (CF_S2 | CF_A2 | CF_B2)

#ifndef FZ_SPLIT_MIN
#define FZ_SPLIT_MIN 16
#endif
#define FZ_NSEG 9

typedef unsigned fz_u32x4 __attribute__((ext_vector_type(4)));

#ifdef SBWT_STATS
#ifndef SBWT_SLOW_LO
#define SBWT_SLOW_LO 100
#define SBWT_SLOW_HI 100000
#endif
__device__ unsigned long long g_iter_hist[64];
__device__ unsigned long long g_tail_prof[192];
extern "C" int sbwtgpu_debug_tail_prof(unsigned long long *out, int reset) {
    if (out && hipMemcpyFromSymbol(out, HIP_SYMBOL(g_tail_prof), sizeof(g_tail_prof)) != hipSuccess) return -1;
    if (reset) {
        unsigned long long z[192] = {0};
        if (hipMemcpyToSymbol(HIP_SYMBOL(g_tail_prof), z, sizeof(z)) != hipSuccess) return -1;
    }
    return 0;
}
__device__ unsigned long long g_iter_max[8];
extern "C" int sbwtgpu_debug_iter_hist(unsigned long long *out, int reset) {
    if (out && hipMemcpyFromSymbol(out, HIP_SYMBOL(g_iter_hist), sizeof(g_iter_hist)) != hipSuccess) return -1;
    if (reset) {
        unsigned long long z[64] = {0};
        if (hipMemcpyToSymbol(HIP_SYMBOL(g_iter_hist), z, sizeof(z)) != hipSuccess) return -1;
    }
    return 0;
}
extern "C" int sbwtgpu_debug_iter_max(unsigned long long *out, int reset) {
    if (out && hipMemcpyFromSymbol(out, HIP_SYMBOL(g_iter_max), sizeof(g_iter_max)) != hipSuccess) return -1;
    if (reset) {
        unsigned long long z[8] = {0};
        if (hipMemcpyToSymbol(HIP_SYMBOL(g_iter_max), z, sizeof(z)) != hipSuccess) return -1;
    }
    return 0;
}
__device__ unsigned long long g_fz_why[24];
extern "C" int sbwtgpu_debug_why(unsigned long long *out, int reset) {
    if (out && hipMemcpyFromSymbol(out, HIP_SYMBOL(g_fz_why), sizeof(g_fz_why)) != hipSuccess) return -1;
    if (reset) {
        unsigned long long z[24] = {0};
        if (hipMemcpyToSymbol(HIP_SYMBOL(g_fz_why), z, sizeof(z)) != hipSuccess) return -1;
    }
    return 0;
}
__device__ unsigned long long g_sort_stats[16];
extern "C" int sbwtgpu_debug_sort_stats(unsigned long long *out, int reset) {
    if (out && hipMemcpyFromSymbol(out, HIP_SYMBOL(g_sort_stats), sizeof(g_sort_stats)) != hipSuccess) return -1;
    if (reset) {
        unsigned long long z[16] = {0};
        if (hipMemcpyToSymbol(HIP_SYMBOL(g_sort_stats), z, sizeof(z)) != hipSuccess) return -1;
    }
    return 0;
}
#define FZ_SORT_STAT(q, val) do { const unsigned long long v_ = (unsigned long long)(val); if (lane == 0 && v_) atomicAdd(&g_sort_stats[q], v_); } while (0)
#define FZ_WHY(q, cond) do { const unsigned long long n_ = __popcll(__ballot(cond)); if (lane == 0 && n_) atomicAdd(&g_fz_why[q], n_); } while (0)
__device__ unsigned long long g_fz_plan[48];
extern "C" int sbwtgpu_debug_plan(unsigned long long *out, int reset) {
    if (out && hipMemcpyFromSymbol(out, HIP_SYMBOL(g_fz_plan), sizeof(g_fz_plan)) != hipSuccess) return -1;
    if (reset) {
        unsigned long long z[48] = {0};
        if (hipMemcpyToSymbol(HIP_SYMBOL(g_fz_plan), z, sizeof(z)) != hipSuccess) return -1;
    }
    return 0;
}
#define FZ_PLAN(q, cond) do { const unsigned long long n_ = __popcll(__ballot(cond)); if (lane == 0 && n_) atomicAdd(&g_fz_plan[q], n_); } while (0)
#define FZ_PLAN_SUM(q, val) do { unsigned long long v_ = (unsigned long long)(val); for (int o_ = 32; o_ > 0; o_ >>= 1) v_ += __shfl_down(v_, o_); if (lane == 0 && v_) atomicAdd(&g_fz_plan[q], v_); } while (0)
#define FZ_HIST_FLUSH() do { if (it_cnt) { atomicAdd(&g_iter_hist[(it_cnt >> 1) < 63 ? (it_cnt >> 1) : 63], 1ull); \
    if (it_cnt >= SBWT_SLOW_LO && it_cnt < SBWT_SLOW_HI) atomicMax(&g_iter_max[it_cnt & 7u], ((unsigned long long)it_cnt << 32) | rd); it_cnt = 0; } } while (0)
#else
#define FZ_SORT_STAT(q, val) do { } while (0)
#define FZ_HIST_FLUSH() do { } while (0)
#define FZ_WHY(q, cond) do { } while (0)
#define FZ_PLAN(q, cond) do { } while (0)
#define FZ_PLAN_SUM(q, val) do { } while (0)
#endif

#ifdef SBWT_TIMELINE
__device__ unsigned long long g_fz_tl[8];
__device__ unsigned long long g_fz_tl_hist[1024];
extern "C" int sbwtgpu_debug_timeline(unsigned long long *out, int reset) {
    if (out && (hipMemcpyFromSymbol(out, HIP_SYMBOL(g_fz_tl), sizeof(g_fz_tl)) != hipSuccess ||
                hipMemcpyFromSymbol(out + 8, HIP_SYMBOL(g_fz_tl_hist), sizeof(g_fz_tl_hist)) != hipSuccess)) return -1;
    if (reset) {
        static unsigned long long z[1024];
        unsigned long long t0[8] = {~0ull, ~0ull, 0, 0, 0, 0, 0, 0};
        if (hipMemcpyToSymbol(HIP_SYMBOL(g_fz_tl), t0, sizeof(t0)) != hipSuccess ||
            hipMemcpyToSymbol(HIP_SYMBOL(g_fz_tl_hist), z, sizeof(g_fz_tl_hist)) != hipSuccess) return -1;
    }
    return 0;
}
#endif

__device__ __forceinline__ u64 fz_encode32(const unsigned w[8], const unsigned tm[8], unsigned &bad) {
    u64 codes = 0;
#pragma unroll
    for (int d = 0; d < 8; d++) {
        const unsigned x = w[d];
        const unsigned t = ((x >> 1) & 0x03030303u) ^ ((x >> 2) & 0x01010101u);
        const unsigned c8 = (t * 0x01041040u) >> 24;
        const unsigned letters = __builtin_amdgcn_perm(0x54474341u, 0x54474341u, t);
        bad |= (letters ^ x) & tm[d];
        codes |= (u64)c8 << (8 * d);
    }
    return codes;
}

#ifdef FZ_SORT_WG5
#define FZ_SLOTS 256
#define FZ_RING 256
#define FZ_SORT_WGS 5
#else
#define FZ_SLOTS 320
#define FZ_RING 512
#define FZ_SORT_WGS 4
#endif
template <bool WIDE, bool O32, bool BIG = false, bool UNI = false, bool SORT = false, bool TAB = false>
__global__ void __launch_bounds__(256, SORT ? FZ_SORT_WGS : 5) k_search_fused(SbwtIndexView ix, const unsigned char *__restrict__ bases,
                                                          i64 total_bases, i64 *__restrict__ out, i64 n_reads,
                                                          SbwtWorkHeader *ws, unsigned *__restrict__ defer_list,
                                                          const i64 *__restrict__ read_off, const i64 *__restrict__ out_off,
                                                          SbwtTickTab tt) {
    static_assert(!SORT || (!WIDE && !BIG), "lanes sorted by state: k <= 31, fewer than 2^31 columns (so far)");
    __shared__ u64 pool_codes[SBWT_FUSED_MAXG][SORT ? 128 : 256];
    constexpr int NSLOT = SORT ? FZ_SLOTS : 256;
    __shared__ u64 cur_codes[SBWT_FUSED_MAXG][NSLOT];
    __shared__ unsigned seg_src[FZ_NSEG][NSLOT];
    __shared__ unsigned char seg_at[FZ_NSEG][NSLOT];
    __shared__ unsigned st_w[SORT ? 4 : 1][SORT ? FZ_SLOTS : 1];
    __shared__ unsigned short q_ring[SORT ? 2 : 1][SORT ? FZ_RING : 1];
    __shared__ unsigned q_ctl[8];
    const int fmode = sbwt_fused_mode(ws, ix.k);
    if (fmode == 0) return;
    const int P_batch = sbwt_fused_pieces(ws, ix.k);
    if (UNI != (fmode == 1 && P_batch == 1 && !(ix.debug & 128))) return;
    const bool ragged = !UNI && fmode == 2;
    static_assert(!TAB || !UNI, "the ticket table's instantiation is a general one");
    const bool table = TAB && fmode == 3 && tt.tick != nullptr;
    if (TAB != (fmode == 3)) return;
    if (!WIDE && !BIG && ix.fused_sort > 0) {
        const bool sorted_call = (ix.fused_sort & 4096) ||
                                 (ws->hint == (unsigned long long)(SBWT_HINT_MAGIC | (unsigned)SBWT_HINT_CALLS) && (UNI || TAB || P_batch == 1));
        if (SORT != sorted_call) return;
    } else if (SORT) return;
    const int tid = threadIdx.x, lane = tid & 63, wbase = tid & ~63;
    const bool follower_wave = SORT && __builtin_amdgcn_readfirstlane(tid) >= 128;
    int slot = SORT ? (follower_wave ? -1 : tid) : tid;
    if (SORT) {
        if (tid < 8) q_ctl[tid] = (tid == 2) ? (unsigned)(FZ_SLOTS - 128) : 0u;
        for (int q = tid; q < (SORT ? FZ_RING : 0); q += 256) {
            q_ring[0][SORT ? q : 0] = q < FZ_SLOTS - 128 ? (unsigned short)(128 + q + 1) : (unsigned short)0;
            q_ring[SORT ? 1 : 0][SORT ? q : 0] = 0;
        }
        for (int q = 128 + tid; q < (SORT ? FZ_SLOTS : 0); q += 256) st_w[SORT ? 2 : 0][SORT ? q : 0] = 0u;
        __syncthreads();
    }
#define FZ_LDS32(p) (*(__attribute__((address_space(3))) volatile unsigned *)(p))
#define FZ_LDS16(p) (*(__attribute__((address_space(3))) volatile unsigned short *)(p))
    auto ring_push = [&](const u64 mask, const int ring, const int s) {
        unsigned base = 0;
        if (lane == 0) base = __hip_atomic_fetch_add(&q_ctl[2 + ring], (unsigned)__popcll(mask), __ATOMIC_RELAXED, __HIP_MEMORY_SCOPE_WORKGROUP);
        base = uniform32(base);
        if ((mask >> lane) & 1ull) {
            const unsigned at = (base + (unsigned)__popcll(mask & low_mask(lane))) & (unsigned)(FZ_RING - 1);
            asm volatile("s_waitcnt lgkmcnt(0)" ::: "memory");
            FZ_LDS16(&q_ring[SORT ? ring : 0][SORT ? at : 0]) = (unsigned short)(s + 1);
        }
    };
    const int k = ix.k, p = ix.p_dev, L0 = ix.probe_len, ps = ix.p_sparse;
    const int P = (UNI || table) ? 1 : P_batch, kpp = SBWT_FUSED_MAXLEN - k + 1;
    const bool varlen = ragged || table || P > 1;
    const i64 n_tickets = table ? (i64)ws->n_ftick : n_reads * P;
    const int ulen = (ragged || table) ? SBWT_FUSED_MAXLEN : (int)ws->u_len, m = ulen - k + 1, G = varlen ? SBWT_FUSED_MAXG : ((ulen + 31) >> 5);
    const i64 u_read0 = ws->u_read0, u_out0 = ws->u_out0, u_stride = ws->u_stride;
    const bool pfon = ix.pfil && ix.p_filter == L0 && L0 > p;
    const u64 mk2 = (k - ps >= 32) ? ~0ull : low_mask(2 * ((k - ps) & 31));
    const int pw = pfon ? L0 : p;
    const int last_node = (int)(ix.n_nodes - 1);
    static_assert(!BIG || !O32, "2^31 columns and more: int64 results");
    auto zx = [](int v) -> i64 { return BIG ? (i64)(unsigned)v : (i64)v; };
    auto is_run = [](unsigned src) -> bool { return BIG ? src != 0xFFFFFFFFu : !(src >> 31); };

    int nseg = 0, i0 = 0, last_start = 0;
    unsigned sort_spins = 0;
    unsigned sort_seen = 0;
    unsigned sort_waits = 0;
#ifdef SBWT_SORT_COUNTERS
    unsigned c_iter = 0;
    unsigned long long c_busy = 0;
    unsigned c_lists = 0, c_part = 0;
#endif
    const int sort_thr = (SORT && (ix.fused_sort & 255) > 1) ? ((ix.fused_sort & 255) < 64 ? (ix.fused_sort & 255) : 64) : 0;
    const int sort_ship = SORT ? ((ix.fused_sort >> 8) & 15) : 0;
    u64 fm_pend = 0;
    int pend = 0;
    unsigned pend_rd = 0;
    unsigned last_src = 0, emit_pos = 0;
    int wk = 0;
    u64 hk = 0;
    int blo = -1;
    int co = 0, cP = 0, m1 = -1;
    unsigned fl = 0;
    const bool wide_k = WIDE && ((ix.stab2 != nullptr && ps < k) || (ix.stab_pos && ps == k)) && !(ix.debug & 32);
    const bool anch_ok = wide_k;
    const bool seed_ok = wide_k && ps < k && !BIG;
    int bnext = -1;
    int mode = F_IDLE;
    unsigned rd = 0;
    int i = 0, j = 0, b = -1, wstart = 0;
    int mend = 0;
    bool drained = false;
    int l = 0, r = 0;
    unsigned c_ext = 0;
    constexpr bool LSEG_LDS = SORT || !UNI;
    u64 pool_next = 0, pool_end = 0, pool_bad = 0;
    int pool_len = 0;
    unsigned c_stream = 0, c_search = 0, c_lf = 0, c_tab = 0;
#ifdef SBWT_STATS
    unsigned it_cnt = 0, tail_it = 0;
#endif
#ifdef SBWT_TIMELINE
    const u64 tl_start = wall_clock64();
    u64 tl_drain = 0;
    unsigned tl_n = 0;
    if (lane == 0) atomicMin(&g_fz_tl[0], tl_start);
#endif

    if (SORT && follower_wave) {
        constexpr bool isP = true;
        constexpr bool runS = !SORT || !isP, runP = !SORT || isP;
        constexpr int qc = isP ? 1 : 0;
#include "sbwt_search_fused_loop.inc"
    } else {
        constexpr bool isP = false;
        constexpr bool runS = !SORT || !isP, runP = !SORT || isP;
        constexpr int qc = isP ? 1 : 0;
#include "sbwt_search_fused_loop.inc"
    }

    FZ_HIST_FLUSH();
#ifdef SBWT_TIMELINE
    if (lane == 0) {
        const u64 tl_exit = wall_clock64(), t0 = g_fz_tl[0];
        atomicMin(&g_fz_tl[1], tl_drain); atomicMax(&g_fz_tl[2], tl_drain); atomicMax(&g_fz_tl[3], tl_exit);
        atomicAdd(&g_fz_tl[4], 1ull); atomicAdd(&g_fz_tl[5], tl_exit - tl_drain); atomicAdd(&g_fz_tl[6], tl_exit - tl_start);
        atomicAdd(&g_fz_tl[7], (unsigned long long)tl_n);
        const u64 bk = (tl_exit - t0) / 1000ull;
        atomicAdd(&g_fz_tl_hist[bk < 1023 ? bk : 1023], 1ull);
    }
#endif
    {
        u64 e = c_ext & 0xFFFFFu, eb = c_ext >> 20;
#pragma unroll
        for (int off = 32; off > 0; off >>= 1) { e += __shfl_down(e, off); eb += __shfl_down(eb, off); }
        if (lane == 0) { if (e) atomicAdd(&ws->n_ext, e); if (eb) atomicAdd(&ws->n_bridge, eb); }
    }
#if defined(SBWT_SORT_COUNTERS) && !defined(SBWT_STATS)
    if (SORT && lane == 0) {
        atomicAdd(&ws->pad[follower_wave ? 13 : 11], (unsigned long long)c_iter);
        atomicAdd(&ws->pad[follower_wave ? 14 : 12], c_busy);
        atomicAdd(&ws->pad[9], (unsigned long long)c_lists);
        atomicAdd(&ws->pad[10], (unsigned long long)c_part);
    }
#endif
    if (lane == 0) {
        if (c_stream) atomicAdd(&ws->n_stream, (u64)c_stream);
        if (c_search) atomicAdd(&ws->n_search, (u64)c_search);
        if (c_lf) atomicAdd(&ws->n_lf, (u64)c_lf);
        if (c_tab) atomicAdd(&ws->n_tab_hit, (u64)c_tab);
    }
}

__global__ void __launch_bounds__(256) k_fused_tickets(const i64 *__restrict__ read_off, const i64 *__restrict__ out_off, i64 n_reads,
                                                       SbwtWorkHeader *ws, int k, SbwtTickTab tt) {
    if (!sbwt_fused_wants_table(ws, k)) return;
    const int lane = threadIdx.x & 63;
    const int kpp = SBWT_FUSED_MAXLEN - k + 1;
    const i64 stride = (i64)gridDim.x * 256;
    for (i64 r0 = (i64)blockIdx.x * 256 + (threadIdx.x & ~63); r0 < n_reads; r0 += stride) {
        const i64 r = r0 + lane;
        const bool valid = r < n_reads;
        const i64 P0 = valid ? read_off[r] : 0, len = valid ? read_off[r + 1] - P0 : 0, ob = valid ? out_off[r] : 0;
        const i64 m = len - k + 1;
        const u64 np = m > 0 ? (u64)((m + kpp - 1) / kpp) : 0ull;
        u64 incl = np;
#pragma unroll
        for (int o = 1; o < 64; o <<= 1) { const u64 v = __shfl_up(incl, o); if (lane >= o) incl += v; }
        const u64 total = __shfl(incl, 63);
        if (total == 0) continue;
        u64 base = 0;
        if (lane == 0) base = atomicAdd(&ws->n_ftick, (unsigned long long)total);
        base = uniform64(base);
        if (base + total > (u64)tt.cap) {
            if (lane == 0) ws->ftick_over = 1ull;
            continue;
        }
        const u64 first = base + incl - np;
        auto entry = [&](i64 rr, i64 p0, i64 ln, i64 o0, u64 t0, u64 j) {
            const i64 b = p0 + (i64)j * kpp, left = ln - (i64)j * kpp;
            const unsigned nb = (unsigned)(left > SBWT_FUSED_MAXLEN ? SBWT_FUSED_MAXLEN : left);
            const i64 o = o0 + (i64)j * kpp;
            tt.tick[t0 + j] = make_uint4((unsigned)b, ((unsigned)((u64)b >> 32) & 0xFFFFu) | (nb << 16), (unsigned)o, (unsigned)((u64)o >> 32));
            tt.tick_read[t0 + j] = (unsigned)rr;
        };
        for (u64 j = 0; j < np && j < 4; j++) entry(r, P0, len, ob, first, j);
        u64 big = __ballot(np > 4);
        while (big) {
            const int src = __ffsll((i64)big) - 1;
            big &= big - 1;
            const i64 rr = __shfl(r, src), p0 = __shfl(P0, src), ln = __shfl(len, src), o0 = __shfl(ob, src);
            const u64 t0 = __shfl(first, src), nn = __shfl(np, src);
            for (u64 j = 4 + (u64)lane; j < nn; j += 64) entry(rr, p0, ln, o0, t0, j);
        }
    }
}

__global__ void k_fused_hint(SbwtWorkHeader *ws, int k) {
    if (threadIdx.x != 0 || sbwt_fused_mode(ws, k) == 0) return;
    const unsigned long long ext = ws->n_ext, walks = ws->n_search, prev = ws->hint;
    const bool fits = walks > 0 && ext >= (unsigned long long)SBWT_HINT_RATIO * walks;
    const unsigned run = ((prev & ~0xFFull) == (unsigned long long)SBWT_HINT_MAGIC) ? (unsigned)(prev & 0xFFull) : 0u;
    ws->hint = (unsigned long long)(SBWT_HINT_MAGIC | (fits ? (run < SBWT_HINT_CALLS ? run + 1u : (unsigned)SBWT_HINT_CALLS) : 0u));
}

__global__ void __launch_bounds__(256) k_check_uniform2(const i64 *__restrict__ read_off, const i64 *__restrict__ out_off,
                                                        i64 n_reads, SbwtWorkHeader *ws, int k, SbwtPieceTab pt,
                                                        int rg_enable) {
    const i64 t = (i64)blockIdx.x * 256 + threadIdx.x;
    const i64 len = read_off[1] - read_off[0], stride = (n_reads > 1) ? out_off[1] - out_off[0] : 0;
    if (t == 0) { ws->u_read0 = read_off[0]; ws->u_len = len; ws->u_out0 = out_off[0]; ws->u_stride = stride; }
    const bool valid = t < n_reads;
    const i64 mylen = valid ? read_off[t + 1] - read_off[t] : 0;
    fused_sample_of_wave(t, mylen, valid, n_reads, rg_enable, k, ws);
    piece_zones_of_wave(t, mylen, valid, k, ws, pt);
    if (!valid) return;
    const bool bad = (mylen != len) || (t + 1 < n_reads && out_off[t + 1] - out_off[t] != stride);
    if (__ballot(bad) != 0 && (threadIdx.x & 63) == 0) ws->u_bad = 1ull;
}

void sbwt_launch_search_fused(const SbwtIndexView &ix, const char *d_bases, long long total_bases, uint4 *d_packed,
                              const long long *d_read_off, const long long *d_out_off, long long *d_out, long long n_reads,
                              SbwtWorkHeader *ws, int streaming, hipStream_t stream, unsigned *d_defer,
                              hipEvent_t ev_begin, hipEvent_t ev_end, SbwtPieceTab pt, int ragged_ok, SbwtTickTab tt) {
    if (n_reads <= 0) return;
    hipLaunchKernelGGL(k_check_uniform2, dim3(grid_for(n_reads)), dim3(256), 0, stream, d_read_off, d_out_off, (i64)n_reads, ws,
                       ix.k, pt, ragged_ok);
    if (tt.tick && n_reads < ((i64)1 << 32)) {
        const i64 wantt = (n_reads + 255) / 256;
        hipLaunchKernelGGL(k_fused_tickets, dim3((unsigned)(wantt < 1024 ? wantt : 1024)), dim3(256), 0, stream, d_read_off, d_out_off,
                           (i64)n_reads, ws, ix.k, tt);
    }
    const i64 want_r = (n_reads + 255) / 256, want_t = tt.tick ? (total_bases / SBWT_FUSED_MAXLEN + 255) / 256 : 0;
    const i64 want = want_r > want_t ? want_r : want_t;
    unsigned cap = 1280u;
    if (ix.debug >> 8) cap = (unsigned)(ix.debug >> 8);
    else if (total_bases < 8000000ll) cap = 256u;
    else if (total_bases < 20000000ll) cap = 384u;
    else if (total_bases < 60000000ll) cap = 512u;
    else if (total_bases < 110000000ll) cap = 640u;
    else if (total_bases < 170000000ll) cap = 768u;
    else if (total_bases < 250000000ll) cap = 896u;
    else if (total_bases < 500000000ll) cap = 1024u;
    const bool sorted = !ix.big && !(ix.n_nodes >= ((i64)1 << 31) - 64) && !((ix.stab2 != nullptr && ix.p_sparse < ix.k) || (ix.debug & 64)) && ix.fused_sort > 0;
    const unsigned cap_s = cap > 256u * FZ_SORT_WGS ? 256u * FZ_SORT_WGS : cap;
    const unsigned g = (unsigned)(want < (i64)cap ? want : (i64)cap), g_s = (unsigned)(want < (i64)cap_s ? want : (i64)cap_s);
    if (ev_begin) (void)hipEventRecord(ev_begin, stream);
    const bool wide = (ix.stab2 != nullptr && ix.p_sparse < ix.k) || (ix.debug & 64);
#define FZ_LAUNCH1(W, O, B, U) hipLaunchKernelGGL((k_search_fused<W, O, B, U>), dim3(g), dim3(256), 0, stream, ix, \
                                           reinterpret_cast<const unsigned char *>(d_bases), (i64)total_bases, d_out, (i64)n_reads, ws, d_defer, \
                                           d_read_off, d_out_off, tt)
#define FZ_LAUNCH(W, O, B) do { FZ_LAUNCH1(W, O, B, true); FZ_LAUNCH1(W, O, B, false); \
                                if (tt.tick) hipLaunchKernelGGL((k_search_fused<W, O, B, false, false, true>), dim3(g), dim3(256), 0, stream, ix, \
                                           reinterpret_cast<const unsigned char *>(d_bases), (i64)total_bases, d_out, (i64)n_reads, ws, d_defer, \
                                           d_read_off, d_out_off, tt); } while (0)
#define FZ_LAUNCH_S(O) do { hipLaunchKernelGGL((k_search_fused<false, O, false, true, true>), dim3(g_s), dim3(256), 0, stream, ix, \
                                           reinterpret_cast<const unsigned char *>(d_bases), (i64)total_bases, d_out, (i64)n_reads, ws, d_defer, \
                                           d_read_off, d_out_off, tt); \
                            hipLaunchKernelGGL((k_search_fused<false, O, false, false, true>), dim3(g_s), dim3(256), 0, stream, ix, \
                                           reinterpret_cast<const unsigned char *>(d_bases), (i64)total_bases, d_out, (i64)n_reads, ws, d_defer, \
                                           d_read_off, d_out_off, tt); \
                            if (tt.tick) hipLaunchKernelGGL((k_search_fused<false, O, false, false, true, true>), dim3(g_s), dim3(256), 0, stream, ix, \
                                           reinterpret_cast<const unsigned char *>(d_bases), (i64)total_bases, d_out, (i64)n_reads, ws, d_defer, \
                                           d_read_off, d_out_off, tt); } while (0)
    const bool big = ix.big || ix.n_nodes >= ((i64)1 << 31) - 64;
    if (big) { if (wide) FZ_LAUNCH(true, false, true); else FZ_LAUNCH(false, false, true); }
    else if (wide) { if (ix.out32) FZ_LAUNCH(true, true, false); else FZ_LAUNCH(true, false, false); }
    else {
        if (ix.out32) FZ_LAUNCH(false, true, false); else FZ_LAUNCH(false, false, false);
        if (sorted) { if (ix.out32) FZ_LAUNCH_S(true); else FZ_LAUNCH_S(false); }
    }
#undef FZ_LAUNCH_S
#undef FZ_LAUNCH
#undef FZ_LAUNCH1
    if (ev_end) (void)hipEventRecord(ev_end, stream);
    if (sorted) hipLaunchKernelGGL(k_fused_hint, dim3(1), dim3(64), 0, stream, ws, ix.k);
    sbwt_launch_encode_chained(d_bases, total_bases, d_packed, ws, d_defer, d_read_off, ix.k, stream);
    sbwt_launch_piece_bounds_tt(d_packed, d_read_off, d_out_off, ix.k, ws, pt, 1, stream, tt.defer_bits);
    sbwt_launch_search_chained(ix, d_packed, d_read_off, d_out_off, d_out, n_reads, ws, streaming, stream, d_defer, pt);
}
```

### sbwt_amd/csrc/sbwtgpu_capi.cpp

```cpp
#include <hip/hip_runtime.h>

#include <dlfcn.h>
#include <cstdarg>
#include <chrono>
#include <cstdio>
#include <cstdlib>
#include <algorithm>
#include <mutex>
#include <cstddef>
#include <cstring>
#include <new>
#include <vector>
#include <thread>

#include "../../include/sbwtgpu.h"
#include "sbwt_device.h"
#include "sbwt_ms.h"
#include "sbwt_unitigs.h"
#include "sbwt_setops.h"
#include "sbwt_readhits.h"

namespace {

thread_local char g_err[512] = "";
// ... 576 lines not shown
                                               h.p_filter > 0 ? reinterpret_cast<uint4 *>(idx->blob + h.off_pfil) : nullptr,
                                               (long long)h.n_sb2,
                                               h.n_sb2 > 0 ? reinterpret_cast<uint4 *>(idx->blob + h.off_stab2) : nullptr, 0);
            e = hipDeviceSynchronize();
            if (g_verbose >= 2) plog("  (sparse tables: built)");
            if (!use_arena) arena_drop();
            if (src == -3) { h.n_sb2 = 0; src = 0; }
            if (src < 0 && e == hipSuccess) e = hipErrorUnknown;
            if (e != hipSuccess) break;
            h.stab_pos = src > 0 ? 1 : 0;
            plog("sparse table, second level, filter");
            if (big_path && h.has_path && !(h.stab_pos || (h.n_sb2 > 0 && d->k > h.p_sparse))) { e = hipErrorOutOfMemory; break; }
            const bool whole_kmers = h.p_sparse == d->k || (h.n_sb2 > 0 && d->k > h.p_sparse);
            if (h.has_path && whole_kmers && g_path_safe) {
                SbwtIndexView v2 = idx->view();
                void *hscr = nullptr;
                const bool wide_safe = d->k > h.p_sparse;
                const size_t safe_bytes = (size_t)sbwt_path_safe_scratch_bytes(h.n_pos, (int)d->k);
                const bool hscr_in_arena = arena && arena_bytes >= safe_bytes;
                if (!hscr_in_arena) arena_drop();
                if (g_path_safe >= 2 || wide_safe) {
                    if (hscr_in_arena) hscr = arena;
                    else if (hipMalloc(&hscr, safe_bytes) != hipSuccess) {
                        (void)hipGetLastError();
                        hscr = nullptr;
                    }
                }
                if (hscr && hipMalloc((void **)&alt_safe, (size_t)h.n_pos) != hipSuccess) {
                    (void)hipGetLastError();
                    alt_safe = nullptr;
                }
                sbwt_launch_path_safe(v2, reinterpret_cast<uint4 *>(idx->blob + h.off_pq), hscr ? (wide_safe ? 2 : g_path_safe) : 1, hscr, alt_safe, 0);
                e = hipDeviceSynchronize();
                const bool had_scratch = hscr != nullptr;
                if (hscr && !hscr_in_arena) (void)hipFree(hscr);
                if (e != hipSuccess) break;
                h.has_safe = (wide_safe && !had_scratch) ? 0 : 1;
            }
        }
        plog("substitution-safe bits");
        if (h.has_path) {
            SbwtIndexView v3 = idx->view();
            long long nb = 0;
            const long long n_ent = sbwt_launch_path_oth(v3, reinterpret_cast<uint4 *>(idx->blob + h.off_pq), &nb, 0);
            if (n_ent != h.n_trans) { e = hipErrorUnknown; break; }
            const int64_t n_slots = h.n_tslots;
            plog("only-successor bits");
            sbwt_launch_trans_insert(idx->view(), reinterpret_cast<uint4 *>(idx->blob + h.off_trans), n_slots, alt_safe, 0);
            if ((e = hipDeviceSynchronize()) != hipSuccess) break;
            h.n_paths = sbwt_count_paths(idx->view(), 0);
            if (h.n_paths < 0) { e = hipErrorUnknown; break; }
            plog("transition table");
        }
        if ((e = hipGetLastError()) != hipSuccess) break;
        e = hipDeviceSynchronize();
    } while (0);
    arena_drop();
    if (alt_safe) (void)hipFree(alt_safe);
    if (e == hipErrorOutOfMemory && level < 2 && (h.has_path || h.p_sparse > 0)) {
        (void)hipGetLastError();
        (void)hipFree(idx->blob);
        delete idx;
        return retry_next_level();
    }
    if (e != hipSuccess) {
        rc = fail(SBWTGPU_ERR_HIP, "building the index image: %s", hipGetErrorString(e));
        (void)hipFree(idx->blob);
        delete idx;
        return rc;
    }
    *out = idx;
    return SBWTGPU_OK;
}

void sbwtgpu_index_destroy(sbwtgpu_index *idx) {
    if (!idx) return;
    if (idx->blob && idx->owns_blob) {
        DeviceGuard guard(idx->device);
        (void)hipFree(idx->blob);
    }
    if (idx->lcs) {
        DeviceGuard guard(idx->device);
        (void)hipFree(idx->lcs);
    }
    delete idx;
}

int sbwtgpu_index_get_info(const sbwtgpu_index *idx, sbwtgpu_index_info *info) {
    if (!idx || !info) return fail(SBWTGPU_ERR_INVALID_ARG, "idx/info is NULL");
    info->n_nodes = idx->h.n_nodes;
    info->n_kmers = idx->h.n_kmers;
    info->k = idx->h.k;
    info->precalc_k = idx->h.p_file;
    for (int i = 0; i < 4; i++) info->C[i] = idx->h.C[i];
    info->has_streaming_support = idx->h.has_ssup;
    info->device = idx->device;
    info->device_precalc_k = idx->h.p_dev;
    info->blob_bytes = idx->h.blob_bytes;
    info->image_level = idx->h.image_level;
    info->n_paths = idx->h.n_paths;
    info->n_branch = idx->h.n_branch;
    info->default_search_variant = !idx->h.has_path ? 1 : auto_variant(idx->h);
    return SBWTGPU_OK;
}

int sbwtgpu_index_get_precalc(const sbwtgpu_index *idx, int64_t *out_pairs) {
    if (!idx || !out_pairs) return fail(SBWTGPU_ERR_INVALID_ARG, "idx/out is NULL");
    if (idx->h.p_file == 0) return SBWTGPU_OK;
    DeviceGuard guard(idx->device);
    HIP_TRY(hipMemcpy(out_pairs, idx->blob + idx->h.off_ftab, (size_t)16 << (2 * idx->h.p_file),
                      hipMemcpyDeviceToHost));
    return SBWTGPU_OK;
}

int sbwtgpu_index_export_header(const sbwtgpu_index *idx, void *header_out, int64_t cap, int64_t *bytes) {
    if (!idx || !bytes) return fail(SBWTGPU_ERR_INVALID_ARG, "idx/bytes is NULL");
    *bytes = (int64_t)sizeof(SbwtBlobHeader);
    if (!header_out) return SBWTGPU_OK;
    if (cap < (int64_t)sizeof(SbwtBlobHeader)) return fail(SBWTGPU_ERR_INVALID_ARG, "header buffer too small");
    memcpy(header_out, &idx->h, sizeof(SbwtBlobHeader));
    return SBWTGPU_OK;
}

int sbwtgpu_index_blob(const sbwtgpu_index *idx, void **dev_ptr, int64_t *bytes) {
    if (!idx || !dev_ptr || !bytes) return fail(SBWTGPU_ERR_INVALID_ARG, "NULL argument");
    *dev_ptr = idx->blob;
    *bytes = idx->h.blob_bytes;
    return SBWTGPU_OK;
}

int sbwtgpu_index_copy_blob(const sbwtgpu_index *idx, void *dst_dev, int64_t bytes, void *stream) {
    if (!idx || !dst_dev) return fail(SBWTGPU_ERR_INVALID_ARG, "NULL argument");
    if (bytes != idx->h.blob_bytes) return fail(SBWTGPU_ERR_INVALID_ARG, "bytes must equal blob_bytes");
    DeviceGuard guard(idx->device);
    HIP_TRY(hipMemcpyAsync(dst_dev, idx->blob, (size_t)bytes, hipMemcpyDeviceToDevice, static_cast<hipStream_t>(stream)));
    return SBWTGPU_OK;
}

int sbwtgpu_index_adopt(const void *header, int64_t header_bytes, void *dev_blob, int64_t blob_bytes, int device,
                        sbwtgpu_index **out) {
    if (!header || !dev_blob || !out) return fail(SBWTGPU_ERR_INVALID_ARG, "NULL argument");
    if (header_bytes != (int64_t)sizeof(SbwtBlobHeader)) return fail(SBWTGPU_ERR_INVALID_ARG, "bad header size");
    SbwtBlobHeader h;
    memcpy(&h, header, sizeof(h));
    if (h.magic != SBWT_BLOB_MAGIC) return fail(SBWTGPU_ERR_INVALID_ARG, "bad header magic");
    if (h.blob_bytes != blob_bytes) return fail(SBWTGPU_ERR_INVALID_ARG, "blob size does not match its header");
    if (((uintptr_t)dev_blob & 255) != 0) return fail(SBWTGPU_ERR_INVALID_ARG, "the device image must be 256-byte aligned");
    sbwtgpu_index *idx = new (std::nothrow) sbwtgpu_index();
    if (!idx) return fail(SBWTGPU_ERR_OOM, "out of host memory");
    idx->h = h;
    idx->device = device;
    idx->blob = static_cast<char *>(dev_blob);
    idx->owns_blob = false;
    *out = idx;
    return SBWTGPU_OK;
}

int sbwtgpu_debug_bcast_plan(int n_dev, const int *devs, int root_device, int n_visible, int *uniq_out, int *slot_out, int *n_uniq,
                             int *root_rank) {
    if (n_dev <= 0 || !devs || !uniq_out || !slot_out || !n_uniq || !root_rank) return fail(SBWTGPU_ERR_INVALID_ARG, "NULL/empty argument");
    int nu = 0;
    for (int i = 0; i < n_dev; i++) {
        if (devs[i] < 0 || devs[i] >= n_visible) return fail(SBWTGPU_ERR_NO_DEVICE, "device %d out of range", devs[i]);
        int u = 0;
        while (u < nu && uniq_out[u] != devs[i]) u++;
        if (u == nu) uniq_out[nu++] = devs[i];
        slot_out[i] = u;
    }
    *n_uniq = nu;
    *root_rank = -1;
    for (int u = 0; u < nu; u++)
        if (uniq_out[u] == root_device) *root_rank = u;
    if (*root_rank < 0) return fail(SBWTGPU_ERR_INVALID_ARG, "the root's device must be in devs[]");
    return SBWTGPU_OK;
}

int sbwtgpu_index_bcast(sbwtgpu_index *root, int n_dev, const int *devs, sbwtgpu_index **out) {
    if (!root || n_dev <= 0 || !devs || !out) return fail(SBWTGPU_ERR_INVALID_ARG, "NULL/empty argument");
    int ndev = 0;
    if (hipGetDeviceCount(&ndev) != hipSuccess) ndev = 0;
    std::vector<int> uniq((size_t)n_dev, 0);
    std::vector<int> slot((size_t)n_dev, 0);
    int n_uniq = 0, root_rank = -1;
    {
        const int prc = sbwtgpu_debug_bcast_plan(n_dev, devs, root->device, ndev, uniq.data(), slot.data(), &n_uniq, &root_rank);
        if (prc != SBWTGPU_OK) return prc;
    }
    const char *nd_env = getenv("SBWTGPU_BCAST_NO_DEDUP");
    if (nd_env && *nd_env == '1' && n_dev > 1) {
        n_uniq = n_dev;
        root_rank = -1;
        for (int i = 0; i < n_dev; i++) {
            uniq[(size_t)i] = devs[i];
            slot[(size_t)i] = i;
            if (root_rank < 0 && devs[i] == root->device) root_rank = i;
        }
    }
    uniq.resize((size_t)n_uniq);
    if (uniq.size() == 1) {
        for (int i = 0; i < n_dev; i++) out[i] = root;
        return SBWTGPU_OK;
    }
    typedef void *comm_t;
    typedef int (*init_all_t)(comm_t *, int, const int *);
    typedef int (*bcast_t)(const void *, void *, size_t, int, int, comm_t, hipStream_t);
    typedef int (*grp_t)(void);
    typedef int (*destroy_t)(comm_t);
    const char *rccl_name = getenv("SBWTGPU_RCCL_LIB");
    void *lib = (rccl_name && *rccl_name) ? dlopen(rccl_name, RTLD_NOW | RTLD_GLOBAL) : dlopen("librccl.so.1", RTLD_NOW | RTLD_GLOBAL);
    if (!lib && !(rccl_name && *rccl_name)) lib = dlopen("librccl.so", RTLD_NOW | RTLD_GLOBAL);
    if (!lib) return fail(SBWTGPU_ERR_HIP, "cannot load librccl.so: %s", dlerror());
    init_all_t init_all = (init_all_t)dlsym(lib, "ncclCommInitAll");
    bcast_t bcast = (bcast_t)dlsym(lib, "ncclBroadcast");
    grp_t gstart = (grp_t)dlsym(lib, "ncclGroupStart"), gend = (grp_t)dlsym(lib, "ncclGroupEnd");
    destroy_t destroy = (destroy_t)dlsym(lib, "ncclCommDestroy");
    if (!init_all || !bcast || !gstart || !gend || !destroy) {
        dlclose(lib);
        return fail(SBWTGPU_ERR_HIP, "RCCL symbols missing");
    }
    const int nu = (int)uniq.size();
    std::vector<comm_t> comms((size_t)nu, nullptr);
    std::vector<hipStream_t> streams((size_t)nu, nullptr);
    std::vector<char> have_stream((size_t)nu, 0);
    std::vector<sbwtgpu_index *> made((size_t)nu, nullptr);
    bool have_comms = false;
    int rc = SBWTGPU_OK;
    for (int u = 0; u < nu && rc == SBWTGPU_OK; u++) {
        if (hipSetDevice(uniq[u]) != hipSuccess || hipStreamCreate(&streams[u]) != hipSuccess) {
            rc = fail(SBWTGPU_ERR_HIP, "cannot set up device %d", uniq[u]);
            break;
        }
        have_stream[u] = 1;
        if (u != root_rank) {
            sbwtgpu_index *c = new (std::nothrow) sbwtgpu_index();
            if (!c || hipMalloc((void **)&c->blob, (size_t)root->h.blob_bytes) != hipSuccess) {
                delete c;
                rc = fail(SBWTGPU_ERR_OOM, "hipMalloc on device %d", uniq[u]);
                break;
            }
            c->h = root->h;
            c->device = uniq[u];
            made[u] = c;
        }
    }
    if (rc == SBWTGPU_OK) {
        if (init_all(comms.data(), nu, uniq.data()) != 0) rc = fail(SBWTGPU_ERR_HIP, "ncclCommInitAll failed");
        else have_comms = true;
    }
    if (rc == SBWTGPU_OK) {
        gstart();
        for (int u = 0; u < nu; u++) {
            (void)hipSetDevice(uniq[u]);
            void *buf = (u == root_rank) ? (void *)root->blob : (void *)made[u]->blob;
            if (bcast(buf, buf, (size_t)root->h.blob_bytes,  0, root_rank, comms[u], streams[u]) != 0)
                rc = fail(SBWTGPU_ERR_HIP, "ncclBroadcast failed");
        }
        if (gend() != 0 && rc == SBWTGPU_OK) rc = fail(SBWTGPU_ERR_HIP, "ncclGroupEnd failed");
        for (int u = 0; u < nu; u++) {
            (void)hipSetDevice(uniq[u]);
            if (hipStreamSynchronize(streams[u]) != hipSuccess && rc == SBWTGPU_OK)
                rc = fail(SBWTGPU_ERR_HIP, "broadcast to device %d failed", uniq[u]);
        }
    }
    for (int u = 0; u < nu; u++) {
        if (!have_stream[u] && !have_comms) continue;
        (void)hipSetDevice(uniq[u]);
        if (have_comms) destroy(comms[u]);
        if (have_stream[u]) (void)hipStreamDestroy(streams[u]);
    }
    (void)hipSetDevice(root->device);
    if (rc != SBWTGPU_OK) {
        for (auto *c : made) sbwtgpu_index_destroy(c);
        dlclose(lib);
        return rc;
    }
    for (int i = 0; i < n_dev; i++) out[i] = (slot[(size_t)i] == root_rank) ? root : made[(size_t)slot[(size_t)i]];
    return SBWTGPU_OK;
}

static inline int64_t ws_packed_bytes(int64_t total_bases) {
    const int64_t groups = (total_bases + SBWT_GROUP_BASES - 1) / SBWT_GROUP_BASES + 4;
    return (int64_t)sizeof(SbwtWorkHeader) + groups * 16;
}
static inline int64_t ws_sort_capacity(int64_t total_bases) {
    return g_sort_reads > 0 ? total_bases / 32 + 4096 : 0;
}
static inline int64_t ws_defer_bytes(int64_t total_bases) { return align256(total_bases / 8 + 256); }
static inline int ws_piece_len(int64_t total_bases) {
    int piece = 128;
    while (piece < SBWT_PIECE && total_bases / piece > ((int64_t)1 << 18)) piece *= 2;
    return piece;
}
static inline int64_t ws_piece_cap(int64_t total_bases) {
    return std::max<int64_t>(total_bases / SBWT_PIECE, std::min<int64_t>(total_bases / 128, (int64_t)1 << 18)) + 2;
}
static inline int64_t ws_piece_bytes(int64_t total_bases) { return align256(ws_piece_cap(total_bases) * 32); }
static inline int64_t ws_tick_cap(int64_t total_bases) { return total_bases / 64 + 64; }
static inline int64_t ws_tick_bytes(int64_t total_bases) {
    return align256(ws_tick_cap(total_bases) * 16) + align256(ws_tick_cap(total_bases) * 4) + align256(total_bases / 256 + 64);
}
static inline int64_t ws_fixed_bytes(int64_t total_bases) {
    return align256(ws_packed_bytes(total_bases)) + ws_defer_bytes(total_bases) + ws_piece_bytes(total_bases) + ws_tick_bytes(total_bases);
}
int64_t sbwtgpu_search_workspace_bytes(int64_t total_bases) {
    if (total_bases < 0) total_bases = 0;
    const int64_t n_cap = ws_sort_capacity(total_bases);
    return ws_fixed_bytes(total_bases) + (n_cap ? 32 * n_cap + ((int64_t)16 << 20) : 0);
}
static SbwtPieceTab ws_piece_tab(void *d_ws, int64_t total_bases) {
    SbwtPieceTab pt;
    if (!g_split_long) return pt;
    char *base = static_cast<char *>(d_ws) + align256(ws_packed_bytes(total_bases)) + ws_defer_bytes(total_bases);
    pt.cap = ws_piece_cap(total_bases);
    pt.piece = ws_piece_len(total_bases);
    pt.pairs = reinterpret_cast<uint4 *>(base);
    pt.outs = pt.pairs + pt.cap;
    return pt;
}

static SbwtTickTab ws_tick_tab(void *d_ws, int64_t total_bases) {
    SbwtTickTab tt;
    char *base = static_cast<char *>(d_ws) + align256(ws_packed_bytes(total_bases)) + ws_defer_bytes(total_bases) + ws_piece_bytes(total_bases);
    tt.cap = ws_tick_cap(total_bases);
    tt.tick = reinterpret_cast<uint4 *>(base);
    tt.tick_read = reinterpret_cast<unsigned *>(base + align256(tt.cap * 16));
    tt.defer_bits = reinterpret_cast<unsigned *>(base + align256(tt.cap * 16) + align256(tt.cap * 4));
    return tt;
}

static const char *RANK_ONLY_MSG =
    "the index columns are not a valid SBWT (set bits != n_nodes - 1): only rank() is available";

static bool internal_streaming_ok(const SbwtBlobHeader &h) {
    return (h.has_ssup || h.ssup_derived) && g_derive_ssup && h.k >= 2;
}

static int search_dev_check(const sbwtgpu_index *idx, int64_t total_bases, int64_t n_reads, const void *d_ws,
                            int64_t ws_bytes, int streaming) {
    if (!idx) return fail(SBWTGPU_ERR_INVALID_ARG, "idx is NULL");
    if (idx->h.rank_only) return fail(SBWTGPU_ERR_INVALID_ARG, "%s", RANK_ONLY_MSG);
    if (streaming && !idx->h.has_ssup)
        return fail(SBWTGPU_ERR_NO_STREAMING, "Error: streaming search support not built");
    if (n_reads < 0 || total_bases < 0) return fail(SBWTGPU_ERR_INVALID_ARG, "negative size");
    if (total_bases >= ((int64_t)1 << 36))
        return fail(SBWTGPU_ERR_INVALID_ARG, "more than 2^36 bases in one call: split the batch");
    if (!d_ws) return fail(SBWTGPU_ERR_INVALID_ARG, "NULL workspace");
    if (ws_bytes < sbwtgpu_search_workspace_bytes(total_bases))
        return fail(SBWTGPU_ERR_INVALID_ARG, "workspace too small (%lld < %lld)", (long long)ws_bytes,
                    (long long)sbwtgpu_search_workspace_bytes(total_bases));
    if (((uintptr_t)d_ws & 15) != 0) return fail(SBWTGPU_ERR_INVALID_ARG, "workspace must be 16-byte aligned");
    return SBWTGPU_OK;
}

int sbwtgpu_encode_bases_dev(const sbwtgpu_index *idx, const char *d_bases, int64_t total_bases, void *d_ws,
                             int64_t ws_bytes, void *stream) {
    int rc = search_dev_check(idx, total_bases, 0, d_ws, ws_bytes, 0);
    if (rc != SBWTGPU_OK) return rc;
    if (total_bases > 0 && !d_bases) return fail(SBWTGPU_ERR_INVALID_ARG, "NULL device pointer");
    DeviceGuard guard(idx->device);
    SbwtWorkHeader *ws = static_cast<SbwtWorkHeader *>(d_ws);
    uint4 *packed = reinterpret_cast<uint4 *>(static_cast<char *>(d_ws) + sizeof(SbwtWorkHeader));
    sbwt_launch_encode(d_bases, total_bases, packed, ws, static_cast<hipStream_t>(stream));
    hipError_t e = hipGetLastError();
    if (e != hipSuccess) return fail(SBWTGPU_ERR_HIP, "kernel launch: %s", hipGetErrorString(e));
    return SBWTGPU_OK;
}

int sbwtgpu_search_encoded_dev(const sbwtgpu_index *idx, int64_t total_bases, const int64_t *d_read_off,
                               int64_t n_reads, int64_t *d_out, const int64_t *d_out_off, void *d_ws,
                               int64_t ws_bytes, int streaming, void *stream) {
    int rc = search_dev_check(idx, total_bases, n_reads, d_ws, ws_bytes, streaming);
    if (rc != SBWTGPU_OK) return rc;
    if (n_reads == 0) return SBWTGPU_OK;
    if (!d_read_off || !d_out_off) return fail(SBWTGPU_ERR_INVALID_ARG, "NULL device pointer");
    DeviceGuard guard(idx->device);
    hipStream_t st = static_cast<hipStream_t>(stream);
    SbwtWorkHeader *ws = static_cast<SbwtWorkHeader *>(d_ws);
    hipError_t e = hipMemsetAsync(ws, 0, sizeof(SbwtWorkHeader), st);
    if (e != hipSuccess) return fail(SBWTGPU_ERR_HIP, "hipMemsetAsync: %s", hipGetErrorString(e));
    const uint4 *packed = reinterpret_cast<const uint4 *>(static_cast<char *>(d_ws) + sizeof(SbwtWorkHeader));
    if (g_poison && n_reads > 0) {
        int64_t ends[2] = {0, 0};
        HIP_TRY(hipMemcpyAsync(&ends[0], d_out_off, 8, hipMemcpyDeviceToHost, st));
        HIP_TRY(hipMemcpyAsync(&ends[1], d_out_off + n_reads, 8, hipMemcpyDeviceToHost, st));
        HIP_TRY(hipStreamSynchronize(st));
        if (ends[1] > ends[0]) {
                    const size_t vb = t_out32 ? 4 : 8;
                    HIP_TRY(hipMemsetAsync(reinterpret_cast<char *>(d_out) + (size_t)ends[0] * vb, 0xA5, (size_t)(ends[1] - ends[0]) * vb, st));
                }
    }
    int variant = g_variant_override >= 0 ? g_variant_override : tuning_variant();
    if (variant < 0) variant = idx->h.has_path ? auto_variant(idx->h) : 2;
    if (variant == 5 || variant == 2 || variant == 3) variant = 4;
    const int eff_streaming = (!streaming && internal_streaming_ok(idx->h)) ? 2 : streaming;
    void *sort_scratch = nullptr;
    long long sort_bytes = 0;
    int key_bits = 1;
    while (key_bits < 32 && ((int64_t)1 << key_bits) <= idx->h.n_nodes) key_bits++;
    const bool path_kernel = variant == 4 && idx->h.has_path && eff_streaming && idx->h.stab_pos &&
                             idx->h.n_nodes < ((int64_t)1 << 31) - 128 && n_reads < ((int64_t)1 << 31);
    const bool want_sort = path_kernel && g_sort_reads > 0;
    if (want_sort) {
        const int64_t off = ws_fixed_bytes(total_bases);
        sort_bytes = sbwt_sort_scratch_bytes(n_reads, key_bits);
        if (n_reads <= ws_sort_capacity(total_bases) && off + sort_bytes <= ws_bytes) sort_scratch = static_cast<char *>(d_ws) + off;
    }
    sbwt_launch_search(idx->view(), packed, reinterpret_cast<const long long *>(d_read_off),
                       reinterpret_cast<const long long *>(d_out_off), reinterpret_cast<long long *>(d_out), n_reads,
                       ws, eff_streaming, st, variant, total_bases / SBWT_GROUP_BASES + 2, sort_scratch, sort_bytes, key_bits,
                       ws_piece_tab(d_ws, total_bases));
    e = hipGetLastError();
    if (e != hipSuccess) return fail(SBWTGPU_ERR_HIP, "kernel launch: %s", hipGetErrorString(e));
    return SBWTGPU_OK;
}

static const int EV_RING = 256;
static hipEvent_t g_ev[EV_RING][2];
static int g_ev_made = 0;

int sbwtgpu_kernel_times(double *ms, int64_t cap, int64_t *n) {
    if (!n || (cap > 0 && !ms)) return fail(SBWTGPU_ERR_INVALID_ARG, "NULL argument");
    const int64_t have = g_ev_count < EV_RING ? g_ev_count : EV_RING;
    const int64_t first = g_ev_count - have;
    int64_t w = 0;
    for (int64_t q = first; q < g_ev_count && w < cap; q++, w++) {
        hipEvent_t *e = g_ev[q % EV_RING];
        HIP_TRY(hipEventSynchronize(e[1]));
        float f = 0;
        HIP_TRY(hipEventElapsedTime(&f, e[0], e[1]));
        ms[w] = (double)f;
    }
    *n = w;
    return SBWTGPU_OK;
}

static int search_dev_common(const sbwtgpu_index *idx, const char *d_bases, int64_t total_bases,
                             const int64_t *d_read_off, int64_t n_reads, int64_t *d_out, const int64_t *d_out_off,
                             void *d_ws, int64_t ws_bytes, void *stream, int streaming) {
    int rc = search_dev_check(idx, total_bases, n_reads, d_ws, ws_bytes, streaming);
    if (rc != SBWTGPU_OK) return rc;
    if (n_reads == 0) return SBWTGPU_OK;
    {
        int variant = g_variant_override >= 0 ? g_variant_override : tuning_variant();
        if (variant < 0) variant = idx->h.has_path ? auto_variant(idx->h) : 2;
        const int eff_streaming = (!streaming && internal_streaming_ok(idx->h)) ? 2 : streaming;
        const bool big_image = idx->h.big_layout && idx->h.has_path && !t_out32 &&
                               ((idx->h.stab_pos && idx->h.p_sparse == idx->h.k) || (idx->h.n_sb2 > 0 && idx->h.k > idx->h.p_sparse));
        const bool path_kernel = idx->h.has_path && eff_streaming &&
                                 ((idx->h.n_nodes < ((int64_t)1 << 31) - 128 && !idx->h.big_layout) || big_image) && n_reads < ((int64_t)1 << 31) &&
                                 total_bases / SBWT_GROUP_BASES + 2 < ((int64_t)1 << 31) - 4;
        if (variant == 5 && path_kernel && g_sort_reads <= 0 && !(g_debug & 16)) {
            if (!d_read_off || !d_out_off) return fail(SBWTGPU_ERR_INVALID_ARG, "NULL device pointer");
            if (total_bases > 0 && !d_bases) return fail(SBWTGPU_ERR_INVALID_ARG, "NULL device pointer");
            DeviceGuard guard(idx->device);
            hipStream_t st = static_cast<hipStream_t>(stream);
            SbwtWorkHeader *ws = static_cast<SbwtWorkHeader *>(d_ws);
            HIP_TRY(hipMemsetAsync(ws, 0, SBWT_WS_CLEAR_BYTES, st));
            if (g_poison) {
                int64_t ends[2] = {0, 0};
                HIP_TRY(hipMemcpyAsync(&ends[0], d_out_off, 8, hipMemcpyDeviceToHost, st));
                HIP_TRY(hipMemcpyAsync(&ends[1], d_out_off + n_reads, 8, hipMemcpyDeviceToHost, st));
                HIP_TRY(hipStreamSynchronize(st));
                if (ends[1] > ends[0]) {
                    const size_t vb = t_out32 ? 4 : 8;
                    HIP_TRY(hipMemsetAsync(reinterpret_cast<char *>(d_out) + (size_t)ends[0] * vb, 0xA5, (size_t)(ends[1] - ends[0]) * vb, st));
                }
            }
            uint4 *packed = reinterpret_cast<uint4 *>(static_cast<char *>(d_ws) + sizeof(SbwtWorkHeader));
            unsigned *defer = reinterpret_cast<unsigned *>(static_cast<char *>(d_ws) + align256(ws_packed_bytes(total_bases)));
            const SbwtTickTab tt_of_call = ws_tick_tab(d_ws, total_bases);
            HIP_TRY(hipMemsetAsync(tt_of_call.defer_bits, 0, (size_t)(total_bases / 256 + 64), st));
            SbwtTickTab tt_for_launch = tt_of_call;
            if (!(g_fused_table && g_fused_ragged && n_reads <= total_bases / 32)) { tt_for_launch.tick = nullptr; tt_for_launch.tick_read = nullptr; }
            hipEvent_t e0 = nullptr, e1 = nullptr;
            if (g_kernel_events) {
                const int slot = (int)(g_ev_count % EV_RING);
                if (slot >= g_ev_made) {
                    HIP_TRY(hipEventCreate(&g_ev[slot][0]));
                    HIP_TRY(hipEventCreate(&g_ev[slot][1]));
                    g_ev_made = slot + 1;
                }
                e0 = g_ev[slot][0]; e1 = g_ev[slot][1];
                g_ev_count++;
            }
            sbwt_launch_search_fused(idx->view(), d_bases, total_bases, packed, reinterpret_cast<const long long *>(d_read_off),
                                     reinterpret_cast<const long long *>(d_out_off), reinterpret_cast<long long *>(d_out), n_reads,
                                     ws, eff_streaming, st, defer, e0, e1, ws_piece_tab(d_ws, total_bases),
                                     ((g_fused_ragged && n_reads <= total_bases / 32) ? 1 : 0) |
                                         ((g_fused_pieces > 0 ? g_fused_pieces : 3) << 8),
                                     tt_for_launch);
            hipError_t e = hipGetLastError();
            if (e != hipSuccess) return fail(SBWTGPU_ERR_HIP, "kernel launch: %s", hipGetErrorString(e));
            return SBWTGPU_OK;
        }
    }
    rc = sbwtgpu_encode_bases_dev(idx, d_bases, total_bases, d_ws, ws_bytes, stream);
    if (rc != SBWTGPU_OK) return rc;
    return sbwtgpu_search_encoded_dev(idx, total_bases, d_read_off, n_reads, d_out, d_out_off, d_ws, ws_bytes,
                                      streaming, stream);
}

int sbwtgpu_streaming_search_dev(const sbwtgpu_index *idx, const char *d_bases, int64_t total_bases,
                                 const int64_t *d_read_off, int64_t n_reads, int64_t *d_out,
                                 const int64_t *d_out_off, void *d_ws, int64_t ws_bytes, void *stream) {
    return search_dev_common(idx, d_bases, total_bases, d_read_off, n_reads, d_out, d_out_off, d_ws, ws_bytes, stream,
                             1);
}

int sbwtgpu_search_dev(const sbwtgpu_index *idx, const char *d_bases, int64_t total_bases, const int64_t *d_read_off,
                       int64_t n_reads, int64_t *d_out, const int64_t *d_out_off, void *d_ws, int64_t ws_bytes,
                       void *stream) {
    return search_dev_common(idx, d_bases, total_bases, d_read_off, n_reads, d_out, d_out_off, d_ws, ws_bytes, stream,
                             0);
}

static int search_dev_i32(const sbwtgpu_index *idx, const char *d_bases, int64_t total_bases, const int64_t *d_read_off,
                          int64_t n_reads, int32_t *d_out, const int64_t *d_out_off, void *d_ws, int64_t ws_bytes, void *stream,
                          int streaming) {
    if (!idx) return fail(SBWTGPU_ERR_INVALID_ARG, "idx is NULL");
    if (idx->h.n_nodes >= ((int64_t)1 << 31))
        return fail(SBWTGPU_ERR_INVALID_ARG, "int32 results need an index of fewer than 2^31 columns (this one has %lld)",
                    (long long)idx->h.n_nodes);
    t_out32 = 1;
    const int rc = search_dev_common(idx, d_bases, total_bases, d_read_off, n_reads, reinterpret_cast<int64_t *>(d_out), d_out_off,
                                     d_ws, ws_bytes, stream, streaming);
    t_out32 = 0;
    return rc;
}
int sbwtgpu_streaming_search_dev_i32(const sbwtgpu_index *idx, const char *d_bases, int64_t total_bases,
                                     const int64_t *d_read_off, int64_t n_reads, int32_t *d_out, const int64_t *d_out_off,
                                     void *d_ws, int64_t ws_bytes, void *stream) {
    return search_dev_i32(idx, d_bases, total_bases, d_read_off, n_reads, d_out, d_out_off, d_ws, ws_bytes, stream, 1);
}
int sbwtgpu_search_dev_i32(const sbwtgpu_index *idx, const char *d_bases, int64_t total_bases, const int64_t *d_read_off,
                           int64_t n_reads, int32_t *d_out, const int64_t *d_out_off, void *d_ws, int64_t ws_bytes,
                           void *stream) {
    return search_dev_i32(idx, d_bases, total_bases, d_read_off, n_reads, d_out, d_out_off, d_ws, ws_bytes, stream, 0);
}

int sbwtgpu_rank_dev(const sbwtgpu_index *idx, const int64_t *d_pos, const char *d_sym, int64_t n, int64_t *d_out,
                     void *stream) {
    if (!idx) return fail(SBWTGPU_ERR_INVALID_ARG, "idx is NULL");
    if (n < 0) return fail(SBWTGPU_ERR_INVALID_ARG, "negative size");
    if (n == 0) return SBWTGPU_OK;
    if (!d_pos || !d_sym || !d_out) return fail(SBWTGPU_ERR_INVALID_ARG, "NULL device pointer");
    DeviceGuard guard(idx->device);
    sbwt_launch_rank(idx->view(), reinterpret_cast<const long long *>(d_pos), d_sym, n,
                     reinterpret_cast<long long *>(d_out), static_cast<hipStream_t>(stream));
    hipError_t e = hipGetLastError();
    if (e != hipSuccess) return fail(SBWTGPU_ERR_HIP, "kernel launch: %s", hipGetErrorString(e));
    return SBWTGPU_OK;
}

int sbwtgpu_workspace_status(const void *d_ws, void *stream, int *status) {
    if (!d_ws || !status) return fail(SBWTGPU_ERR_INVALID_ARG, "NULL argument");
    SbwtWorkHeader hdr;
    HIP_TRY(hipMemcpyAsync(&hdr, d_ws, sizeof(hdr), hipMemcpyDeviceToHost, static_cast<hipStream_t>(stream)));
    HIP_TRY(hipStreamSynchronize(static_cast<hipStream_t>(stream)));
    *status = hdr.status;
    return SBWTGPU_OK;
}

int sbwtgpu_workspace_stats(const void *d_ws, void *stream, int64_t stats[8]) {
    if (!d_ws || !stats) return fail(SBWTGPU_ERR_INVALID_ARG, "NULL argument");
    SbwtWorkHeader hdr;
    HIP_TRY(hipMemcpyAsync(&hdr, d_ws, sizeof(hdr), hipMemcpyDeviceToHost, static_cast<hipStream_t>(stream)));
    HIP_TRY(hipStreamSynchronize(static_cast<hipStream_t>(stream)));
    stats[0] = (int64_t)hdr.n_stream;
    stats[1] = (int64_t)hdr.n_search;
    stats[2] = (int64_t)hdr.n_lf;
    stats[3] = (int64_t)hdr.n_tab_hit;
    stats[4] = (int64_t)hdr.n_ext;
    stats[5] = (int64_t)hdr.n_bridge;
    stats[6] = stats[7] = 0;
    return SBWTGPU_OK;
}

}
namespace {
struct Stream {
    hipStream_t s = nullptr;
    ~Stream() {
        if (s) (void)hipStreamDestroy(s);
    }
};

constexpr size_t SLOT_CAP = (size_t)1 << 20;
bool g_exiting = false;
struct SmallSlot {
    int device = -1;
    hipStream_t stream = nullptr;
    char *host = nullptr, *dev = nullptr;
    void release() {
        if (device < 0 || g_exiting) return;
        DeviceGuard guard(device);
        if (stream) (void)hipStreamDestroy(stream);
        if (host) (void)hipHostFree(host);
        if (dev) (void)hipFree(dev);
        stream = nullptr; host = dev = nullptr; device = -1;
    }
};
struct SlotSet {
    std::vector<SmallSlot> v;
    ~SlotSet() { for (auto &s : v) s.release(); }
};
thread_local SlotSet t_slots;
SmallSlot *small_slot(int device, size_t need) {
    if (need > SLOT_CAP) return nullptr;
    static const bool once = [] { atexit([] { g_exiting = true; }); return true; }();
    (void)once;
    for (auto &s : t_slots.v)
        if (s.device == device) return &s;
    SmallSlot s;
    if (hipStreamCreateWithFlags(&s.stream, hipStreamNonBlocking) != hipSuccess) { (void)hipGetLastError(); return nullptr; }
    if (hipHostMalloc((void **)&s.host, SLOT_CAP, hipHostMallocDefault) != hipSuccess ||
        hipMalloc((void **)&s.dev, SLOT_CAP) != hipSuccess) {
        (void)hipGetLastError();
        (void)hipStreamDestroy(s.stream);
        if (s.host) (void)hipHostFree(s.host);
        return nullptr;
    }
    s.device = device;
    t_slots.v.push_back(s);
    return &t_slots.v.back();
}

struct Staging {
    std::vector<std::vector<int64_t>> kept;
    Stream tmp_stream;
    DevBuf tmp_dev;
    SmallSlot *sl = nullptr;
    char *dev = nullptr;
    hipStream_t stream = nullptr;
    size_t in_lo = SIZE_MAX, in_hi = 0, out_lo = SIZE_MAX, out_hi = 0;
    struct Back { void *dst; size_t off, n; } back[4];
    int n_back = 0;

    int open(int device, size_t bytes) {
        sl = small_slot(device, bytes);
        if (sl) { dev = sl->dev; stream = sl->stream; return SBWTGPU_OK; }
        HIP_TRY(hipStreamCreateWithFlags(&tmp_stream.s, hipStreamNonBlocking));
        HIP_TRY(tmp_dev.alloc(bytes));
        dev = static_cast<char *>(tmp_dev.p);
        stream = tmp_stream.s;
        return SBWTGPU_OK;
    }
    template <typename T>
    T *at(size_t off) const { return reinterpret_cast<T *>(dev + off); }
    int in(size_t off, const void *src, size_t n) {
        if (n == 0) return SBWTGPU_OK;
        if (!sl) {
            HIP_TRY(hipMemcpyAsync(dev + off, src, n, hipMemcpyHostToDevice, stream));
            return SBWTGPU_OK;
        }
        if (src != sl->host + off) memcpy(sl->host + off, src, n);
        in_lo = std::min(in_lo, off);
        in_hi = std::max(in_hi, off + n);
        return SBWTGPU_OK;
    }
    int in_rebased(size_t off, const int64_t *src, int64_t n) {
        int64_t *o = nullptr;
        if (sl) {
            o = reinterpret_cast<int64_t *>(sl->host + off);
        } else {
            try {
                kept.emplace_back((size_t)n);
            } catch (const std::bad_alloc &) {
                return fail(SBWTGPU_ERR_OOM, "out of host memory");
            }
            o = kept.back().data();
        }
        for (int64_t t = 0; t < n; t++) o[t] = src[t] - src[0];
        return in(off, o, (size_t)n * 8);
    }
    int upload() {
        if (sl && in_hi > in_lo) HIP_TRY(hipMemcpyAsync(dev + in_lo, sl->host + in_lo, in_hi - in_lo, hipMemcpyHostToDevice, stream));
        return SBWTGPU_OK;
    }
    int out(size_t off, void *dst, size_t n) {
        if (n == 0) return SBWTGPU_OK;
        if (!sl) {
            HIP_TRY(hipMemcpyAsync(dst, dev + off, n, hipMemcpyDeviceToHost, stream));
            return SBWTGPU_OK;
        }
        if (n_back == (int)(sizeof(back) / sizeof(back[0]))) return fail(SBWTGPU_ERR_HIP, "internal: too many results in one staged call");
        back[n_back++] = Back{dst, off, n};
        out_lo = std::min(out_lo, off);
        out_hi = std::max(out_hi, off + n);
        return SBWTGPU_OK;
    }
    int finish() {
        if (sl && out_hi > out_lo) HIP_TRY(hipMemcpyAsync(sl->host + out_lo, dev + out_lo, out_hi - out_lo, hipMemcpyDeviceToHost, stream));
        HIP_TRY(hipStreamSynchronize(stream));
        for (int i = 0; i < n_back; i++) memcpy(back[i].dst, sl->host + back[i].off, back[i].n);
        return SBWTGPU_OK;
    }
};
#define STG_TRY(expr)                                                                          \
    do {                                                                                       \
        const int rc_ = (expr);                                                                \
        if (rc_ != SBWTGPU_OK) return rc_;                                                     \
    } while (0)
}
extern "C" {

static inline int check_read_length(const int64_t *read_off, int64_t r) {
    const int64_t len = read_off[r + 1] - read_off[r];
    if (len < 0) return fail(SBWTGPU_ERR_INVALID_ARG, "read_off is not non-decreasing at read %lld", (long long)r);
    if (len >= ((int64_t)1 << 31)) return fail(SBWTGPU_ERR_READ_TOO_LONG, "read %lld has >= 2^31 bases", (long long)r);
    return SBWTGPU_OK;
}

static int check_reads(const int64_t *read_off, const int64_t *out_off, int64_t n_reads, int64_t k, bool *any_long = nullptr) {
    int64_t longest = 0;
    for (int64_t r = 0; r < n_reads; r++) {
        const int rc = check_read_length(read_off, r);
        if (rc != SBWTGPU_OK) return rc;
        int64_t m = read_off[r + 1] - read_off[r] - k + 1;
        if (m < 0) m = 0;
        if (out_off[r + 1] - out_off[r] != m)
            return fail(SBWTGPU_ERR_INVALID_ARG, "out_off[%lld+1]-out_off[%lld] must be max(0,len-k+1) = %lld",
                        (long long)r, (long long)r, (long long)m);
        if (m > longest) longest = m;
    }
    if (any_long) *any_long = longest > 4096;
    return SBWTGPU_OK;
}


static const int64_t PIECE = 2048;
static_assert(2 * PIECE == 4096, "check_reads flags reads of more than 4096 k-mers");

static inline bool window_has_lower(const char *s, int64_t k) {
    for (int64_t t = 0; t < k; t++) {
        char ch = s[t];
        if (ch == 'a' || ch == 'c' || ch == 'g' || ch == 't') return true;
    }
    return false;
}
static int64_t append_pieces(const char *s, int64_t len, int64_t k, char *dst, std::vector<int64_t> &roff,
                             std::vector<int64_t> &ooff) {
    const int64_t m = len - k + 1;
    int64_t written = 0;
    if (m <= 2 * PIECE) {
        if (dst && len > 0) memcpy(dst, s, (size_t)len);
        roff.push_back(roff.back() + len);
        ooff.push_back(ooff.back() + (m > 0 ? m : 0));
        return len;
    }
    int64_t start = 0;
    while (start < m) {
        int64_t next = start + PIECE;
        if (m - next < PIECE) next = m;
        while (next < m && window_has_lower(s + next, k)) next++;
        const int64_t nb = (next - start) + k - 1;
        if (dst) memcpy(dst + written, s + start, (size_t)nb);
        written += nb;
        roff.push_back(roff.back() + nb);
        ooff.push_back(ooff.back() + (next - start));
        start = next;
    }
    return written;
}
static inline int64_t pieces_bases_bound(int64_t len, int64_t k) {
    const int64_t m = len - k + 1;
    if (m <= 2 * PIECE) return len > 0 ? len : 0;
    return len + (m / PIECE + 2) * (k - 1);
}

}
namespace {
struct PipeSlot {
    hipStream_t st = nullptr;
    char *h_in = nullptr, *h_out = nullptr;
// ... 1284 lines not shown
```

Baseline: 257.0 billion.

## Merge fused search variants into fewer launches and fold small kernels into neighbours

Reduces the number of stream operations per streaming search call. The separate uniform/general/table fused-search kernel launches become a single kernel with a runtime dispatch over several bodies. The defer-bits memset moves into the check-uniform kernel, and the hint-update kernel moves into the chained encode kernel. Piece-bounds and chained encode now use capped grid-stride loops, and a stream-op counter is exported for inspection. Merging the bodies can raise register and shared-memory pressure in the combined kernel, which may lower occupancy.

```diff
diff --git a/include/sbwtgpu.h b/include/sbwtgpu.h
--- a/include/sbwtgpu.h
+++ b/include/sbwtgpu.h
@@ -96,6 +96,7 @@
 int  sbwtgpu_select_batch(const sbwtgpu_index *idx, const int64_t *j, const char *sym, int64_t n, int64_t *out);
 
 int64_t sbwtgpu_search_workspace_bytes(int64_t total_bases);
+int  sbwtgpu_stream_ops(int64_t *n);
 int  sbwtgpu_streaming_search_dev(const sbwtgpu_index *idx, const char *d_bases, int64_t total_bases,
                                   const int64_t *d_read_off, int64_t n_reads, int64_t *d_out,
                                   const int64_t *d_out_off, void *d_workspace, int64_t workspace_bytes,
diff --git a/sbwt_amd/capi.py b/sbwt_amd/capi.py
--- a/sbwt_amd/capi.py
+++ b/sbwt_amd/capi.py
@@ -30,7 +30,7 @@
     "sbwtgpu_update_interval_batch", "sbwtgpu_forward_batch",
     "sbwtgpu_build_plain_matrix", "sbwtgpu_free_plain_matrix",
     "sbwtgpu_partial_search_batch", "sbwtgpu_get_kmer_batch", "sbwtgpu_select_batch",
-    "sbwtgpu_search_workspace_bytes", "sbwtgpu_streaming_search_dev", "sbwtgpu_search_dev",
+    "sbwtgpu_search_workspace_bytes", "sbwtgpu_stream_ops", "sbwtgpu_streaming_search_dev", "sbwtgpu_search_dev",
     "sbwtgpu_streaming_search_dev_i32", "sbwtgpu_search_dev_i32",
     "sbwtgpu_rank_dev", "sbwtgpu_encode_bases_dev", "sbwtgpu_search_encoded_dev",
     "sbwtgpu_workspace_status", "sbwtgpu_workspace_stats", "sbwtgpu_kernel_times",
@@ -640,6 +640,14 @@
     return [float(buf[i]) for i in range(n.value)]
 
 
+def stream_ops() -> int:
+    L = lib()
+    L.sbwtgpu_stream_ops.argtypes = [C.POINTER(C.c_int64)]
+    n = C.c_int64(0)
+    _check(L.sbwtgpu_stream_ops(C.byref(n)))
+    return int(n.value)
+
+
 def search_workspace_bytes(total_bases: int) -> int:
     return int(lib().sbwtgpu_search_workspace_bytes(total_bases))
 
diff --git a/sbwt_amd/csrc/sbwt_device.h b/sbwt_amd/csrc/sbwt_device.h
--- a/sbwt_amd/csrc/sbwt_device.h
+++ b/sbwt_amd/csrc/sbwt_device.h
@@ -134,6 +134,9 @@
 #define SBWT_HINT_RATIO 12
 #define SBWT_HINT_CALLS 2
 
+extern long long g_sbwt_stream_ops;
+static inline void sbwt_count_stream_ops(int n) { __atomic_fetch_add(&g_sbwt_stream_ops, (long long)n, __ATOMIC_RELAXED); }
+
 void sbwt_launch_encode(const char *d_bases, long long total_bases, uint4 *d_packed, SbwtWorkHeader *ws,
                         hipStream_t stream);
 void sbwt_launch_search(const SbwtIndexView &ix, const uint4 *d_packed, const long long *d_read_off,
@@ -145,7 +148,7 @@
                               SbwtWorkHeader *ws, int streaming, hipStream_t stream, unsigned *d_defer,
                               hipEvent_t ev_begin, hipEvent_t ev_end, SbwtPieceTab pt, int ragged_ok, SbwtTickTab tt = SbwtTickTab());
 void sbwt_launch_encode_chained(const char *d_bases, long long total_bases, uint4 *d_packed, SbwtWorkHeader *ws,
-                                const unsigned *d_defer, const long long *d_read_off, int k, hipStream_t stream);
+                                const unsigned *d_defer, const long long *d_read_off, int k, hipStream_t stream, int note_hint = 0);
 void sbwt_launch_search_chained(const SbwtIndexView &ix, const uint4 *d_packed, const long long *d_read_off,
                                 const long long *d_out_off, long long *d_out, long long n_reads, SbwtWorkHeader *ws,
                                 int streaming, hipStream_t stream, const unsigned *d_defer, SbwtPieceTab pt);
diff --git a/sbwt_amd/csrc/sbwt_kernels_common.h b/sbwt_amd/csrc/sbwt_kernels_common.h
--- a/sbwt_amd/csrc/sbwt_kernels_common.h
+++ b/sbwt_amd/csrc/sbwt_kernels_common.h
@@ -162,6 +162,13 @@
 __device__ __forceinline__ bool sbwt_fused_wants_table(const SbwtWorkHeader *ws, int k) {
     return (ws->rg_sample & 0xFFFF) > 0 && sbwt_fused_pieces(ws, k) == 0;
 }
+__device__ __forceinline__ void sbwt_fused_note_hint(SbwtWorkHeader *ws, int k) {
+    if (sbwt_fused_mode(ws, k) == 0) return;
+    const unsigned long long ext = ws->n_ext, walks = ws->n_search, prev = ws->hint;
+    const bool fits = walks > 0 && ext >= (unsigned long long)SBWT_HINT_RATIO * walks;
+    const unsigned run = ((prev & ~0xFFull) == (unsigned long long)SBWT_HINT_MAGIC) ? (unsigned)(prev & 0xFFull) : 0u;
+    ws->hint = (unsigned long long)(SBWT_HINT_MAGIC | (fits ? (run < SBWT_HINT_CALLS ? run + 1u : (unsigned)SBWT_HINT_CALLS) : 0u));
+}
 #define SBWT_RG_SAMPLE 4096
 __device__ __forceinline__ void fused_sample_of_wave(i64 t, i64 len, bool valid, i64 n_reads, int rg_enable, int k, SbwtWorkHeader *ws) {
     if (t == 0) ws->rg_sample = ((rg_enable & 1) ? (int)(n_reads < SBWT_RG_SAMPLE ? n_reads : SBWT_RG_SAMPLE) : 0) | ((rg_enable >> 8) << 16);
diff --git a/sbwt_amd/csrc/sbwt_search.hip b/sbwt_amd/csrc/sbwt_search.hip
--- a/sbwt_amd/csrc/sbwt_search.hip
+++ b/sbwt_amd/csrc/sbwt_search.hip
@@ -46,10 +46,11 @@
 }
 
 __global__ void __launch_bounds__(256) k_encode_chained(const unsigned char *__restrict__ bases, i64 total,
-                                                        uint4 *__restrict__ packed, i64 n_groups, const SbwtWorkHeader *ws,
+                                                        uint4 *__restrict__ packed, i64 n_groups, SbwtWorkHeader *ws,
                                                         const unsigned *__restrict__ defer_list,
-                                                        const i64 *__restrict__ read_off, int k, int aligned16) {
+                                                        const i64 *__restrict__ read_off, int k, int aligned16, int note_hint) {
     const i64 t0 = (i64)blockIdx.x * 256 + threadIdx.x, stride = (i64)gridDim.x * 256;
+    if (note_hint && t0 == 0) sbwt_fused_note_hint(ws, k);
     const int fmode = sbwt_fused_mode(ws, k);
     if (fmode == 0) {
         for (i64 g = t0; g < n_groups; g += stride) packed[g] = encode_group(bases, total, g, aligned16);
@@ -1108,24 +1109,24 @@
                                                       const i64 *__restrict__ out_off, int k, const SbwtWorkHeader *ws,
                                                       SbwtPieceTab pt, int behind_fused, const unsigned *__restrict__ defer_bits) {
     if (behind_fused && sbwt_fused_mode(ws, k) == 1 && !piece_read_is_cut(ws->u_len - k + 1, pt.piece)) return;
-    const i64 z = (i64)blockIdx.x * 256 + threadIdx.x;
     const i64 np = (i64)ws->n_pieces < pt.cap ? (i64)ws->n_pieces : pt.cap;
-    if (z >= np) return;
-    const uint4 d = pt.outs[z];
-    const i64 r = (i64)(((u64)d.y << 32) | (u64)d.x), j = (i64)d.z, nz = (i64)d.w;
-    if (behind_fused && defer_bits && sbwt_fused_mode(ws, k) == 3 && !((defer_bits[r >> 5] >> (r & 31)) & 1u)) {
-        const i64 P0e = read_off[r];
-        pt.pairs[z] = make_uint4((unsigned)P0e, (unsigned)((u64)P0e >> 32), (unsigned)P0e, (unsigned)((u64)P0e >> 32));
-        pt.outs[z] = make_uint4(0u, 0u, 0u, 0u);
-        return;
-    }
-    const i64 P0 = read_off[r], m = read_off[r + 1] - P0 - k + 1, ob = out_off[r];
-    const i64 s = j ? piece_adjust(packed, P0, j * pt.piece, m, k) : 0;
-    const i64 e = (j + 1 == nz) ? m : piece_adjust(packed, P0, (j + 1) * pt.piece, m, k);
-    const i64 b0 = P0 + (e > s ? s : 0), b1 = e > s ? P0 + e + k - 1 : P0;
-    const i64 o0 = ob + (e > s ? s : 0);
-    pt.pairs[z] = make_uint4((unsigned)b0, (unsigned)((u64)b0 >> 32), (unsigned)b1, (unsigned)((u64)b1 >> 32));
-    pt.outs[z] = make_uint4((unsigned)o0, (unsigned)((u64)o0 >> 32), 0u, 0u);
+    for (i64 z = (i64)blockIdx.x * 256 + threadIdx.x; z < np; z += (i64)gridDim.x * 256) {
+        const uint4 d = pt.outs[z];
+        const i64 r = (i64)(((u64)d.y << 32) | (u64)d.x), j = (i64)d.z, nz = (i64)d.w;
+        if (behind_fused && defer_bits && sbwt_fused_mode(ws, k) == 3 && !((defer_bits[r >> 5] >> (r & 31)) & 1u)) {
+            const i64 P0e = read_off[r];
+            pt.pairs[z] = make_uint4((unsigned)P0e, (unsigned)((u64)P0e >> 32), (unsigned)P0e, (unsigned)((u64)P0e >> 32));
+            pt.outs[z] = make_uint4(0u, 0u, 0u, 0u);
+            continue;
+        }
+        const i64 P0 = read_off[r], m = read_off[r + 1] - P0 - k + 1, ob = out_off[r];
+        const i64 s = j ? piece_adjust(packed, P0, j * pt.piece, m, k) : 0;
+        const i64 e = (j + 1 == nz) ? m : piece_adjust(packed, P0, (j + 1) * pt.piece, m, k);
+        const i64 b0 = P0 + (e > s ? s : 0), b1 = e > s ? P0 + e + k - 1 : P0;
+        const i64 o0 = ob + (e > s ? s : 0);
+        pt.pairs[z] = make_uint4((unsigned)b0, (unsigned)((u64)b0 >> 32), (unsigned)b1, (unsigned)((u64)b1 >> 32));
+        pt.outs[z] = make_uint4((unsigned)o0, (unsigned)((u64)o0 >> 32), 0u, 0u);
+    }
 }
 
 void sbwt_launch_encode(const char *d_bases, long long total_bases, uint4 *d_packed, SbwtWorkHeader *ws,
@@ -1135,16 +1136,18 @@
     hipLaunchKernelGGL(k_encode, dim3(grid_for(n_groups)), dim3(256), 0, stream,
                        reinterpret_cast<const unsigned char *>(d_bases), (i64)total_bases, d_packed, n_groups, ws,
                        aligned);
+    sbwt_count_stream_ops(1);
 }
 
 void sbwt_launch_encode_chained(const char *d_bases, long long total_bases, uint4 *d_packed, SbwtWorkHeader *ws,
-                                const unsigned *d_defer, const long long *d_read_off, int k, hipStream_t stream) {
+                                const unsigned *d_defer, const long long *d_read_off, int k, hipStream_t stream, int note_hint) {
     i64 n_groups = (total_bases + SBWT_GROUP_BASES - 1) / SBWT_GROUP_BASES + 2;
     int aligned = ((uintptr_t)d_bases & 15) == 0;
     const i64 want = (n_groups + 255) / 256;
-    hipLaunchKernelGGL(k_encode_chained, dim3((unsigned)(want < 4096 ? want : 4096)), dim3(256), 0, stream,
+    hipLaunchKernelGGL(k_encode_chained, dim3((unsigned)(want < 2048 ? want : 2048)), dim3(256), 0, stream,
                        reinterpret_cast<const unsigned char *>(d_bases), (i64)total_bases, d_packed, n_groups, ws, d_defer, d_read_off, k,
-                       aligned);
+                       aligned, note_hint);
+    sbwt_count_stream_ops(1);
 }
 
 static inline bool view_is_big(const SbwtIndexView &ix) { return ix.big || ix.n_mega > 1 || ix.n_nodes >= ((1ll << 31) - 128); }
@@ -1174,13 +1177,16 @@
     else
         hipLaunchKernelGGL((k_search_cert<false, 4, true>), dim3(g), dim3(256), 0, stream, ix, d_packed, d_read_off,
                            d_out_off, d_out, (i64)n_reads, ws, streaming, (const unsigned *)nullptr, d_defer, pt);
+    sbwt_count_stream_ops(1);
 }
 
 void sbwt_launch_piece_bounds_tt(const uint4 *d_packed, const long long *d_read_off, const long long *d_out_off, int k,
                                  SbwtWorkHeader *ws, SbwtPieceTab pt, int behind_fused, hipStream_t stream, const unsigned *defer_bits) {
     if (!pt.pairs || pt.cap <= 0) return;
-    hipLaunchKernelGGL(k_piece_bounds, dim3(grid_for(pt.cap)), dim3(256), 0, stream, d_packed, d_read_off, d_out_off, k, ws, pt,
+    const unsigned g_cap = grid_for(pt.cap);
+    hipLaunchKernelGGL(k_piece_bounds, dim3(g_cap < 1024u ? g_cap : 1024u), dim3(256), 0, stream, d_packed, d_read_off, d_out_off, k, ws, pt,
                        behind_fused, defer_bits);
+    sbwt_count_stream_ops(1);
 }
 void sbwt_launch_piece_bounds(const uint4 *d_packed, const long long *d_read_off, const long long *d_out_off, int k,
                               SbwtWorkHeader *ws, SbwtPieceTab pt, int behind_fused, hipStream_t stream) {
@@ -1197,15 +1203,18 @@
     if (variant >= 1) {
         if (d_sort_scratch) pt = SbwtPieceTab();
         i64 want1 = (n_reads + pt.cap + 255) / 256;
-        if (!(ix.debug & 8) || pt.pairs)
+        if (!(ix.debug & 8) || pt.pairs) {
             hipLaunchKernelGGL(k_check_uniform, dim3(grid_for(n_reads)), dim3(256), 0, stream, d_read_off, d_out_off,
                                (i64)n_reads, ws, ix.k, pt);
-        if (ix.debug & 8) (void)hipMemsetAsync(&ws->u_bad, 0xFF, 8, stream);
+            sbwt_count_stream_ops(1);
+        }
+        if (ix.debug & 8) { (void)hipMemsetAsync(&ws->u_bad, 0xFF, 8, stream); sbwt_count_stream_ops(1); }
         sbwt_launch_piece_bounds(d_packed, d_read_off, d_out_off, ix.k, ws, pt, 0, stream);
         unsigned grid1 = (unsigned)(want1 < 2048 ? want1 : 2048);
         const bool wide = view_is_big(ix) || total_groups >= (1ll << 31) - 4 || (ix.debug & 16);
         unsigned cap = (ix.debug >> 8) ? (unsigned)(ix.debug >> 8) : (variant >= 2 ? 1280u : 1024u);
         unsigned g = grid1 < cap ? grid1 : cap;
+        sbwt_count_stream_ops(1);
         if (wide)
             hipLaunchKernelGGL((k_search_cert<true, 4, false>), dim3(g), dim3(256), 0, stream, ix, d_packed, d_read_off,
                                d_out_off, d_out, (i64)n_reads, ws, streaming, d_perm, (const unsigned *)nullptr, pt);
@@ -1222,6 +1231,7 @@
     }
     i64 want = (n_reads + 255) / 256;
     unsigned grid = (unsigned)(want < 2048 ? want : 2048);
+    sbwt_count_stream_ops(1);
     if (ix.n_mega > 1)
         hipLaunchKernelGGL(k_search<true>, dim3(grid), dim3(256), 0, stream, ix, d_packed, d_read_off, d_out_off,
                            d_out, (i64)n_reads, ws, streaming == 1 ? 1 : 0);
diff --git a/sbwt_amd/csrc/sbwt_search_fused.hip b/sbwt_amd/csrc/sbwt_search_fused.hip
--- a/sbwt_amd/csrc/sbwt_search_fused.hip
+++ b/sbwt_amd/csrc/sbwt_search_fused.hip
@@ -171,34 +171,23 @@
 #define FZ_RING 512
 #define FZ_SORT_WGS 4
 #endif
-template <bool WIDE, bool O32, bool BIG = false, bool UNI = false, bool SORT = false, bool TAB = false>
-__global__ void __launch_bounds__(256, SORT ? FZ_SORT_WGS : 5) k_search_fused(SbwtIndexView ix, const unsigned char *__restrict__ bases,
-                                                          i64 total_bases, i64 *__restrict__ out, i64 n_reads,
-                                                          SbwtWorkHeader *ws, unsigned *__restrict__ defer_list,
-                                                          const i64 *__restrict__ read_off, const i64 *__restrict__ out_off,
-                                                          SbwtTickTab tt) {
+template <bool WIDE, bool O32, bool BIG, bool UNI, bool SORT, bool TAB>
+__device__ __forceinline__ void fz_search_body(const SbwtIndexView &ix, const unsigned char *__restrict__ bases,
+                                               i64 total_bases, i64 *__restrict__ out, i64 n_reads,
+                                               SbwtWorkHeader *ws, unsigned *__restrict__ defer_list,
+                                               const i64 *__restrict__ read_off, const i64 *__restrict__ out_off,
+                                               const SbwtTickTab &tt, const int fmode, const int P_batch,
+                                               u64 (&pool_codes)[SBWT_FUSED_MAXG][SORT ? 128 : 256],
+                                               u64 (&cur_codes)[SBWT_FUSED_MAXG][SORT ? FZ_SLOTS : 256],
+                                               unsigned (&seg_src)[FZ_NSEG][SORT ? FZ_SLOTS : 256],
+                                               unsigned char (&seg_at)[FZ_NSEG][SORT ? FZ_SLOTS : 256],
+                                               unsigned (&st_w)[SORT ? 4 : 1][SORT ? FZ_SLOTS : 1],
+                                               unsigned short (&q_ring)[SORT ? 2 : 1][SORT ? FZ_RING : 1],
+                                               unsigned (&q_ctl)[8]) {
     static_assert(!SORT || (!WIDE && !BIG), "lanes sorted by state: k <= 31, fewer than 2^31 columns (so far)");
-    __shared__ u64 pool_codes[SBWT_FUSED_MAXG][SORT ? 128 : 256];
-    constexpr int NSLOT = SORT ? FZ_SLOTS : 256;
-    __shared__ u64 cur_codes[SBWT_FUSED_MAXG][NSLOT];
-    __shared__ unsigned seg_src[FZ_NSEG][NSLOT];
-    __shared__ unsigned char seg_at[FZ_NSEG][NSLOT];
-    __shared__ unsigned st_w[SORT ? 4 : 1][SORT ? FZ_SLOTS : 1];
-    __shared__ unsigned short q_ring[SORT ? 2 : 1][SORT ? FZ_RING : 1];
-    __shared__ unsigned q_ctl[8];
-    const int fmode = sbwt_fused_mode(ws, ix.k);
-    if (fmode == 0) return;
-    const int P_batch = sbwt_fused_pieces(ws, ix.k);
-    if (UNI != (fmode == 1 && P_batch == 1 && !(ix.debug & 128))) return;
     const bool ragged = !UNI && fmode == 2;
     static_assert(!TAB || !UNI, "the ticket table's instantiation is a general one");
     const bool table = TAB && fmode == 3 && tt.tick != nullptr;
-    if (TAB != (fmode == 3)) return;
-    if (!WIDE && !BIG && ix.fused_sort > 0) {
-        const bool sorted_call = (ix.fused_sort & 4096) ||
-                                 (ws->hint == (unsigned long long)(SBWT_HINT_MAGIC | (unsigned)SBWT_HINT_CALLS) && (UNI || TAB || P_batch == 1));
-        if (SORT != sorted_call) return;
-    } else if (SORT) return;
     const int tid = threadIdx.x, lane = tid & 63, wbase = tid & ~63;
     const bool follower_wave = SORT && __builtin_amdgcn_readfirstlane(tid) >= 128;
     int slot = SORT ? (follower_wave ? -1 : tid) : tid;
@@ -325,6 +314,42 @@
         if (c_lf) atomicAdd(&ws->n_lf, (u64)c_lf);
         if (c_tab) atomicAdd(&ws->n_tab_hit, (u64)c_tab);
     }
+}
+
+#define FZ_UNI 1
+#define FZ_GEN 2
+#define FZ_TAB 4
+#define FZ_ALL (FZ_UNI | FZ_GEN | FZ_TAB)
+template <bool WIDE, bool O32, bool BIG = false, bool SORT = false, int BODIES = FZ_ALL>
+__global__ void __launch_bounds__(256, SORT ? FZ_SORT_WGS : 5) k_search_fused(SbwtIndexView ix, const unsigned char *__restrict__ bases,
+                                                          i64 total_bases, i64 *__restrict__ out, i64 n_reads,
+                                                          SbwtWorkHeader *ws, unsigned *__restrict__ defer_list,
+                                                          const i64 *__restrict__ read_off, const i64 *__restrict__ out_off,
+                                                          SbwtTickTab tt) {
+    __shared__ u64 pool_codes[SBWT_FUSED_MAXG][SORT ? 128 : 256];
+    constexpr int NSLOT = SORT ? FZ_SLOTS : 256;
+    __shared__ u64 cur_codes[SBWT_FUSED_MAXG][NSLOT];
+    __shared__ unsigned seg_src[FZ_NSEG][NSLOT];
+    __shared__ unsigned char seg_at[FZ_NSEG][NSLOT];
+    __shared__ unsigned st_w[SORT ? 4 : 1][SORT ? FZ_SLOTS : 1];
+    __shared__ unsigned short q_ring[SORT ? 2 : 1][SORT ? FZ_RING : 1];
+    __shared__ unsigned q_ctl[8];
+    const int fmode = sbwt_fused_mode(ws, ix.k);
+    if (fmode == 0) return;
+    if (fmode == 3 && tt.tick == nullptr) return;
+    const int P_batch = sbwt_fused_pieces(ws, ix.k);
+    const bool uni = fmode == 1 && P_batch == 1 && !(ix.debug & 128);
+    if (!WIDE && !BIG && ix.fused_sort > 0) {
+        const bool sorted_call = (ix.fused_sort & 4096) ||
+                                 (ws->hint == (unsigned long long)(SBWT_HINT_MAGIC | (unsigned)SBWT_HINT_CALLS) && (uni || fmode == 3 || P_batch == 1));
+        if (SORT != sorted_call) return;
+    } else if (SORT) return;
+#define FZ_BODY(U, T) fz_search_body<WIDE, O32, BIG, U, SORT, T>(ix, bases, total_bases, out, n_reads, ws, defer_list, read_off, out_off, tt, \
+                                                                  fmode, P_batch, pool_codes, cur_codes, seg_src, seg_at, st_w, q_ring, q_ctl)
+    if (fmode == 3) { if constexpr ((BODIES & FZ_TAB) != 0) FZ_BODY(false, true); }
+    else if (uni) { if constexpr ((BODIES & FZ_UNI) != 0) FZ_BODY(true, false); }
+    else { if constexpr ((BODIES & FZ_GEN) != 0) FZ_BODY(false, false); }
+#undef FZ_BODY
 }
 
 __global__ void __launch_bounds__(256) k_fused_tickets(const i64 *__restrict__ read_off, const i64 *__restrict__ out_off, i64 n_reads,
@@ -371,18 +396,11 @@
     }
 }
 
-__global__ void k_fused_hint(SbwtWorkHeader *ws, int k) {
-    if (threadIdx.x != 0 || sbwt_fused_mode(ws, k) == 0) return;
-    const unsigned long long ext = ws->n_ext, walks = ws->n_search, prev = ws->hint;
-    const bool fits = walks > 0 && ext >= (unsigned long long)SBWT_HINT_RATIO * walks;
-    const unsigned run = ((prev & ~0xFFull) == (unsigned long long)SBWT_HINT_MAGIC) ? (unsigned)(prev & 0xFFull) : 0u;
-    ws->hint = (unsigned long long)(SBWT_HINT_MAGIC | (fits ? (run < SBWT_HINT_CALLS ? run + 1u : (unsigned)SBWT_HINT_CALLS) : 0u));
-}
-
 __global__ void __launch_bounds__(256) k_check_uniform2(const i64 *__restrict__ read_off, const i64 *__restrict__ out_off,
                                                         i64 n_reads, SbwtWorkHeader *ws, int k, SbwtPieceTab pt,
-                                                        int rg_enable) {
+                                                        int rg_enable, unsigned *__restrict__ defer_bits, i64 defer_words) {
     const i64 t = (i64)blockIdx.x * 256 + threadIdx.x;
+    for (i64 w = t; w < defer_words; w += (i64)gridDim.x * 256) defer_bits[w] = 0u;
     const i64 len = read_off[1] - read_off[0], stride = (n_reads > 1) ? out_off[1] - out_off[0] : 0;
     if (t == 0) { ws->u_read0 = read_off[0]; ws->u_len = len; ws->u_out0 = out_off[0]; ws->u_stride = stride; }
     const bool valid = t < n_reads;
@@ -399,12 +417,19 @@
                               SbwtWorkHeader *ws, int streaming, hipStream_t stream, unsigned *d_defer,
                               hipEvent_t ev_begin, hipEvent_t ev_end, SbwtPieceTab pt, int ragged_ok, SbwtTickTab tt) {
     if (n_reads <= 0) return;
-    hipLaunchKernelGGL(k_check_uniform2, dim3(grid_for(n_reads)), dim3(256), 0, stream, d_read_off, d_out_off, (i64)n_reads, ws,
-                       ix.k, pt, ragged_ok);
+    {
+        const i64 defer_words = tt.defer_bits ? (total_bases / 256 + 64 + 3) / 4 : 0;
+        const i64 want_w = (defer_words + 4 * 256 - 1) / (4 * 256);
+        const unsigned g_r = grid_for(n_reads), g_w = (unsigned)(want_w < 1024 ? want_w : 1024);
+        hipLaunchKernelGGL(k_check_uniform2, dim3(g_r > g_w ? g_r : g_w), dim3(256), 0, stream, d_read_off, d_out_off, (i64)n_reads, ws,
+                           ix.k, pt, ragged_ok, tt.defer_bits, defer_words);
+        sbwt_count_stream_ops(1);
+    }
     if (tt.tick && n_reads < ((i64)1 << 32)) {
         const i64 wantt = (n_reads + 255) / 256;
         hipLaunchKernelGGL(k_fused_tickets, dim3((unsigned)(wantt < 1024 ? wantt : 1024)), dim3(256), 0, stream, d_read_off, d_out_off,
                            (i64)n_reads, ws, ix.k, tt);
+        sbwt_count_stream_ops(1);
     }
     const i64 want_r = (n_reads + 255) / 256, want_t = tt.tick ? (total_bases / SBWT_FUSED_MAXLEN + 255) / 256 : 0;
     const i64 want = want_r > want_t ? want_r : want_t;
@@ -422,35 +447,24 @@
     const unsigned g = (unsigned)(want < (i64)cap ? want : (i64)cap), g_s = (unsigned)(want < (i64)cap_s ? want : (i64)cap_s);
     if (ev_begin) (void)hipEventRecord(ev_begin, stream);
     const bool wide = (ix.stab2 != nullptr && ix.p_sparse < ix.k) || (ix.debug & 64);
-#define FZ_LAUNCH1(W, O, B, U) hipLaunchKernelGGL((k_search_fused<W, O, B, U>), dim3(g), dim3(256), 0, stream, ix, \
+#define FZ_LAUNCH(W, O, B, S, M, G) do { hipLaunchKernelGGL((k_search_fused<W, O, B, S, M>), dim3(G), dim3(256), 0, stream, ix, \
                                            reinterpret_cast<const unsigned char *>(d_bases), (i64)total_bases, d_out, (i64)n_reads, ws, d_defer, \
-                                           d_read_off, d_out_off, tt)
-#define FZ_LAUNCH(W, O, B) do { FZ_LAUNCH1(W, O, B, true); FZ_LAUNCH1(W, O, B, false); \
-                                if (tt.tick) hipLaunchKernelGGL((k_search_fused<W, O, B, false, false, true>), dim3(g), dim3(256), 0, stream, ix, \
-                                           reinterpret_cast<const unsigned char *>(d_bases), (i64)total_bases, d_out, (i64)n_reads, ws, d_defer, \
-                                           d_read_off, d_out_off, tt); } while (0)
-#define FZ_LAUNCH_S(O) do { hipLaunchKernelGGL((k_search_fused<false, O, false, true, true>), dim3(g_s), dim3(256), 0, stream, ix, \
-                                           reinterpret_cast<const unsigned char *>(d_bases), (i64)total_bases, d_out, (i64)n_reads, ws, d_defer, \
-                                           d_read_off, d_out_off, tt); \
-                            hipLaunchKernelGGL((k_search_fused<false, O, false, false, true>), dim3(g_s), dim3(256), 0, stream, ix, \
-                                           reinterpret_cast<const unsigned char *>(d_bases), (i64)total_bases, d_out, (i64)n_reads, ws, d_defer, \
-                                           d_read_off, d_out_off, tt); \
-                            if (tt.tick) hipLaunchKernelGGL((k_search_fused<false, O, false, false, true, true>), dim3(g_s), dim3(256), 0, stream, ix, \
-                                           reinterpret_cast<const unsigned char *>(d_bases), (i64)total_bases, d_out, (i64)n_reads, ws, d_defer, \
-                                           d_read_off, d_out_off, tt); } while (0)
+                                           d_read_off, d_out_off, tt); sbwt_count_stream_ops(1); } while (0)
+#define FZ_LAUNCH_APART(W, O, B, S, G) do { FZ_LAUNCH(W, O, B, S, FZ_UNI, G); FZ_LAUNCH(W, O, B, S, FZ_GEN, G); \
+                                            if (tt.tick) FZ_LAUNCH(W, O, B, S, FZ_TAB, G); } while (0)
+#define FZ_LAUNCH_WIDE(O, B) do { FZ_LAUNCH(true, O, B, false, FZ_UNI | FZ_GEN, g); if (tt.tick) FZ_LAUNCH(true, O, B, false, FZ_TAB, g); } while (0)
     const bool big = ix.big || ix.n_nodes >= ((i64)1 << 31) - 64;
-    if (big) { if (wide) FZ_LAUNCH(true, false, true); else FZ_LAUNCH(false, false, true); }
-    else if (wide) { if (ix.out32) FZ_LAUNCH(true, true, false); else FZ_LAUNCH(true, false, false); }
+    if (big) { if (wide) FZ_LAUNCH_WIDE(false, true); else FZ_LAUNCH(false, false, true, false, FZ_ALL, g); }
+    else if (wide) { if (ix.out32) FZ_LAUNCH_APART(true, true, false, false, g); else FZ_LAUNCH_WIDE(false, false); }
     else {
-        if (ix.out32) FZ_LAUNCH(false, true, false); else FZ_LAUNCH(false, false, false);
-        if (sorted) { if (ix.out32) FZ_LAUNCH_S(true); else FZ_LAUNCH_S(false); }
-    }
-#undef FZ_LAUNCH_S
+        if (ix.out32) FZ_LAUNCH_APART(false, true, false, false, g); else FZ_LAUNCH(false, false, false, false, FZ_ALL, g);
+        if (sorted) { if (ix.out32) FZ_LAUNCH_APART(false, true, false, true, g_s); else FZ_LAUNCH(false, false, false, true, FZ_ALL, g_s); }
+    }
+#undef FZ_LAUNCH_WIDE
+#undef FZ_LAUNCH_APART
 #undef FZ_LAUNCH
-#undef FZ_LAUNCH1
     if (ev_end) (void)hipEventRecord(ev_end, stream);
-    if (sorted) hipLaunchKernelGGL(k_fused_hint, dim3(1), dim3(64), 0, stream, ws, ix.k);
-    sbwt_launch_encode_chained(d_bases, total_bases, d_packed, ws, d_defer, d_read_off, ix.k, stream);
+    sbwt_launch_encode_chained(d_bases, total_bases, d_packed, ws, d_defer, d_read_off, ix.k, stream, sorted ? 1 : 0);
     sbwt_launch_piece_bounds_tt(d_packed, d_read_off, d_out_off, ix.k, ws, pt, 1, stream, tt.defer_bits);
     sbwt_launch_search_chained(ix, d_packed, d_read_off, d_out_off, d_out, n_reads, ws, streaming, stream, d_defer, pt);
 }
diff --git a/sbwt_amd/csrc/sbwtgpu_capi.cpp b/sbwt_amd/csrc/sbwtgpu_capi.cpp
--- a/sbwt_amd/csrc/sbwtgpu_capi.cpp
+++ b/sbwt_amd/csrc/sbwtgpu_capi.cpp
@@ -902,6 +902,13 @@
 static inline int64_t ws_fixed_bytes(int64_t total_bases) {
     return align256(ws_packed_bytes(total_bases)) + ws_defer_bytes(total_bases) + ws_piece_bytes(total_bases) + ws_tick_bytes(total_bases);
 }
+extern "C++" { long long g_sbwt_stream_ops = 0; }
+int sbwtgpu_stream_ops(int64_t *n) {
+    if (!n) return fail(SBWTGPU_ERR_INVALID_ARG, "NULL argument");
+    *n = (int64_t)__atomic_load_n(&g_sbwt_stream_ops, __ATOMIC_RELAXED);
+    return SBWTGPU_OK;
+}
+
 int64_t sbwtgpu_search_workspace_bytes(int64_t total_bases) {
     if (total_bases < 0) total_bases = 0;
     const int64_t n_cap = ws_sort_capacity(total_bases);
@@ -978,6 +985,7 @@
     SbwtWorkHeader *ws = static_cast<SbwtWorkHeader *>(d_ws);
     hipError_t e = hipMemsetAsync(ws, 0, sizeof(SbwtWorkHeader), st);
     if (e != hipSuccess) return fail(SBWTGPU_ERR_HIP, "hipMemsetAsync: %s", hipGetErrorString(e));
+    sbwt_count_stream_ops(1);
     const uint4 *packed = reinterpret_cast<const uint4 *>(static_cast<char *>(d_ws) + sizeof(SbwtWorkHeader));
     if (g_poison && n_reads > 0) {
         int64_t ends[2] = {0, 0};
@@ -1056,6 +1064,7 @@
             hipStream_t st = static_cast<hipStream_t>(stream);
             SbwtWorkHeader *ws = static_cast<SbwtWorkHeader *>(d_ws);
             HIP_TRY(hipMemsetAsync(ws, 0, SBWT_WS_CLEAR_BYTES, st));
+            sbwt_count_stream_ops(1);
             if (g_poison) {
                 int64_t ends[2] = {0, 0};
                 HIP_TRY(hipMemcpyAsync(&ends[0], d_out_off, 8, hipMemcpyDeviceToHost, st));
@@ -1069,7 +1078,6 @@
             uint4 *packed = reinterpret_cast<uint4 *>(static_cast<char *>(d_ws) + sizeof(SbwtWorkHeader));
             unsigned *defer = reinterpret_cast<unsigned *>(static_cast<char *>(d_ws) + align256(ws_packed_bytes(total_bases)));
             const SbwtTickTab tt_of_call = ws_tick_tab(d_ws, total_bases);
-            HIP_TRY(hipMemsetAsync(tt_of_call.defer_bits, 0, (size_t)(total_bases / 256 + 64), st));
             SbwtTickTab tt_for_launch = tt_of_call;
             if (!(g_fused_table && g_fused_ragged && n_reads <= total_bases / 32)) { tt_for_launch.tick = nullptr; tt_for_launch.tick_read = nullptr; }
             hipEvent_t e0 = nullptr, e1 = nullptr;
```

Measured after the change: 257.6 billion, median of 5. Within noise of the previous version (+0.2%).
